# conanhujinming/flash_hash_join

Hardware: AMD Instinct MI355X
Metric: probe throughput (billion probes/sec), int64 keys, whole join (build + probe phases) per step (higher is better)
Workload: dtype int64

## Files before the change

### flash_hash_join_amd/csrc/fj_host.h

```cpp
#pragma once
#include "fj_internal.h"
#include "../../include/flashjoin.h"
#include "../../include/flashjoin_lab.h"

#include <algorithm>
#include <chrono>
#include <cstdarg>
#include <cstdio>
#include <cstdlib>
#include <cstring>
#include <condition_variable>
#include <functional>
#include <mutex>
#include <string>
#include <thread>
#include <vector>

struct StreamState;

namespace fjh {

int set_err(const char* fmt, ...);
fj_timings& last_timings();
#define HIPCHK(x)                                                                                          \
    do {                                                                                                   \
        hipError_t e_ = (x);                                                                               \
        if (e_ != hipSuccess) return fjh::set_err("%s:%d: %s failed: %s", __FILE__, __LINE__, #x, hipGetErrorString(e_)); \
    } while (0)

struct DeviceGuard {
    int prev = -1; bool changed = false; hipError_t err = hipSuccess;
    explicit DeviceGuard(int dev) {
        err = hipGetDevice(&prev);
        if (err == hipSuccess && prev != dev) { err = hipSetDevice(dev); changed = err == hipSuccess; }
    }
    ~DeviceGuard() { if (changed) (void)hipSetDevice(prev); }
    DeviceGuard(const DeviceGuard&) = delete;
    DeviceGuard& operator=(const DeviceGuard&) = delete;
};
#define FJ_ON_DEVICE(dev)                                                                                   \
    fjh::DeviceGuard dev_guard_(dev);                                                                            \
    if (dev_guard_.err != hipSuccess) return fjh::set_err("selecting HIP device %d failed: %s", (int)(dev), hipGetErrorString(dev_guard_.err))
#define FJ_ENTER(c)                                                                                         \
    if (!(c)) return fjh::set_err("%s: null context", __func__);                                             \
    std::lock_guard<std::recursive_mutex> ctx_lock_((c)->mu);                                                \
    FJ_ON_DEVICE((c)->device)

struct Scalars {
    unsigned long long total;
    unsigned long long expected;
    u64 empty_val;
    u32 err;
    u32 flags;
    u32 alloc[8];
    u32 seg_counter[8];
    unsigned long long bloom_survivors;
    unsigned long long sample_hits;
    u32 next_item;
    u32 next_emit_item;
    unsigned long long owner_counts[64], owner_cursors[64], owner_offsets[64];
    u32 pack_alloc, pack_seg, pack_err, rx_alloc;
    unsigned long long pack_used[64];
    unsigned long long pack_kept;
    u32 pack_xcd[8 * FJ_PF_COUNTERS];
    u32 bc_bounds[20];
};

enum Slot {
    W_POOL_K = 0, W_POOL_V, W_DIR, W_LIST, W_BCHUNKS, W_REL, W_BOFF, W_SEGOFF, W_TOFF, W_TILES, W_KINDS,
    W_SIDE_STRIDE = 2 * W_KINDS,
    W_PART_COUNT = 3 * W_SIDE_STRIDE, W_OUT_OFF, W_GT_KEYS, W_GT_VALS, W_GT_BLOOM, W_WG_COUNT,
    W_H_BK, W_H_BV, W_H_PK, W_H_OK, W_H_OV, W_ROWIDX, W_BKEYS, W_BBASE,
    W_PK_FI, W_PK_BKEYS, W_PK_OBASE,
    W_RX_REL, W_RX_LIST, W_RX_SEGOFF, W_RX_BCH, W_RX_BOFF, W_RX_TOFF, W_RX_TILES,
    W_SK_TILES_B, W_SK_TILES_P, W_SK_NT, W_PART_COUNT2, W_OUT_OFF2,
    W_MM_TILES,
    W_MM_PBITS,
    W_FULL_BITS,
    W_NSLOTS
};

struct Buf { void* p = nullptr; size_t bytes = 0; };

enum Ev { E_START = 0, E_BUILD, E_PPART, E_JOIN, E_EMIT0, E_EMIT1, E_SB0, E_SB1, E_BF0, E_BF1, E_H0, E_H1, E_H2, E_PK0, E_NEV = E_PK0 + 8 };

struct BcastSources { const void* base = nullptr; int n = 0; uint64_t off[FJ_WIDE_MAXSRC] = {}, nkeys[FJ_WIDE_MAXSRC] = {}; };

struct Pending {
    enum Kind { LDS, HBM_TABLE, MANY, BCAST };
    bool valid = false;
    Kind kind = LDS;
    FjLdsJoinArgs lds{};
    FjGtArgs gt{};
    u32 nitems = 0, gt_grid = 0;
    u64 count = 0;
    bool has_second = false; FjLdsJoinArgs lds2{}; u32 nitems2 = 0; u64 count_main = 0; std::vector<u32> flagged;
    bool dups_main = false; std::vector<u32> sk_parts; int sk_bits = 0, sk_plan_bits = 0, sk_npass = 0;
    int mm_outer = 0; FjMmOuterArgs mm{}; u64 mm_P = 0, mm_u = 0, mm_r = 0;
    FjMmSweepArgs mm_sweep{}; u64 mm_u_main = 0; u64* mm_tile_off = nullptr; u64* mm_sweep_off = nullptr;
    bool mm_trivial = false; const u64* mm_pk = nullptr;
    bool has_dups = false;
    const u64* bk = nullptr; const u64* bv = nullptr; size_t nb = 0; int top_bits = 64;
    BcastSources src; const u32* toff = nullptr; size_t nb_total = 0;
};

struct SingleOut { u64* keys = nullptr; u64* vals = nullptr; size_t cap = 0; bool done = false; };

struct Plan { int bits = 0, npass = 0; int fan_log[4] = {0, 0, 0, 0}; int bloom_level = 0; };

struct PassIter {
    int side = 0; bool has_vals = false; size_t n = 0; Plan plan; int used = 64; u32 parents = 1; u64 lbound = 0;
    u32 tile_chunks = 16; int i = 0;
    FjChunkSet prev{}; bool have_prev = false; const uint4* tiles = nullptr; const u32* ntiles = nullptr; const u32* toff = nullptr;
    FjChunkSet cs{}; u32 Gmax = 1, F = 1, appends = 1;
    size_t piece_rows = 0;
    int slot = 0, cs_base = 0;
    u32 item_tc_max = 0;
    bool want_items = false; u32 items_cap = 0; u32* part_count = nullptr; int part_count_slot = W_PART_COUNT;
    bool bloom_done = false; const FjChunkSet* bloom_build = nullptr;
    const u32* bloom_prebuilt = nullptr;
    unsigned long long* bloom_bucket_keys = nullptr;
    int save_level = 0; FjChunkSet saved{};
    u32* alloc_word = nullptr; u32* seg_word = nullptr; u32* err_word = nullptr;
    bool in_pk7 = false; u32 in_b0 = 0, in_top_shift = 0;
    bool vals_pos = false;
};

}

struct PackState {
    bool begun = false, deferred = false;
    u32 part_shift = 0;
    fjh::PassIter it;
    FjPackArgs args{};
    int nranks = 0;
};

struct StreamState {
    bool active = false;
    fjh::Plan plan; fjh::PassIter pit, bit; FjLdsJoinArgs ja{};
    int top_bits = 64, evc = 0;
    size_t np_bound = 0, np_seen = 0, nb_bound = 0, nb_seen = 0;
    u32 p_appends_left = 0, b_appends_left = 0;
    bool probe_done = false, build_done = false;
    const u64* flat_build = nullptr;
    const u64* flat_probe[64]; size_t flat_np[64]; u32 nflat = 0;
    std::vector<std::pair<const u64*, size_t>> bpieces, ppieces;
    bool shuffled = false; u32 b_lo = 0, nbk = 0, nbk_pad = 0;
    bool probe_prepared = true; u32 probe_appends = 0;
    bool with_vals = false;
};

struct BcastState {
    bool packed = false, probed = false;
    size_t nb_total = 0, nb = 0, np = 0;
    int pieces = 1, evc = 0;
    fjh::Plan plan; fjh::PassIter pit; FjLdsJoinArgs ja{};
    bool with_vals = false;
    fjh::BcastSources src;
};

struct fj_ctx {
    int device = 0;
    fjh::Buf bufs[fjh::W_NSLOTS];
    hipEvent_t ev[fjh::E_NEV];
    hipStream_t side = nullptr;
    fjh::Scalars* d_sc = nullptr;
    fjh::Scalars* h_sc = nullptr;
    fjh::Pending pend;
    StreamState st;
    PackState pk;
    BcastState bc;
    hipEvent_t pk_ev = nullptr;
    unsigned long long* pk_h = nullptr;
    size_t ws_bytes = 0;
    u32 num_cus = 256;
    u32 reserve_cus = 0;
    void* stage[3] = {nullptr, nullptr, nullptr};
    size_t stage_bytes = 0;
    bool plan_in_flight = false;
    bool slot_dirty[fjh::W_NSLOTS] = {};
    std::recursive_mutex mu;
};

namespace fjh {

#define FJ_HOOK_LOOPBACK 1
#define FJ_HOOK_INJECT_FAIL 2
#define FJ_HOOK_SPLIT_ALWAYS 4
#define FJ_HOOK_ONE_COMM 8
#define FJ_HOOK_RESERVE_ALWAYS 16
#define FJ_HOOK_EMIT_TAGGED 32
#define FJ_HOOK_EMIT_RETRY_7TH 64
struct Options {
    size_t radix_threshold = 0; int scalar_hbm_table = 0; u32 persistent_min_items = 8192; u32 plan_target_keys = FJ_PART_TARGET_KEYS;
    int bloom_variant = 0, bloom_auto = 1, bloom_auto_max_hit_bp = 2300, mat_single_pass = 1;
    int join_wide = 2;
    u32 lab_hooks = 0;
    u32 join_items_target = 2048;
    int mm_heavy_keys = 0;
    int mm_heavy_outer = 0;
    Options();
};
Options& options();

int get_buf(fj_ctx* c, int slot, size_t bytes, void** out);
int get_zeroed_buf(fj_ctx* c, int slot, size_t bytes, void** out, hipStream_t s);
int plan_npass(int bits);
void plan_passes(Plan& p, bool extra_first);
Plan make_plan(size_t nb, int top_bits, bool want_bloom = false, u64 target_override = 0);
void pass_init(PassIter& it, int side, bool has_vals, size_t n, const Plan& plan, int top_bits);
u32 pass_groups(u64 chunks, u64 rows, u32 tile_chunks, u32 F);
int pass_prepare(fj_ctx* c, PassIter& it, u32 appends, hipStream_t s);
int pass_launch(fj_ctx* c, PassIter& it, const u64* keys, const u64* vals, size_t n, hipStream_t s, int* ev_cursor);
bool bloom_stage_follows(const PassIter& it, int level);
void join_item_geometry(u64 nparts, size_t np, u64 chunk_bound, u32* tc, u64* max_items);
bool wide_join_planned(bool materialize, size_t nb, size_t np_eff, int bits);
int level_finish(fj_ctx* c, PassIter& it, bool final_level, hipStream_t s);
int pass_complete(fj_ctx* c, PassIter& it, hipStream_t s);
int bloom_stage(fj_ctx* c, PassIter& it, hipStream_t s);
int run_passes(fj_ctx* c, PassIter& it, const u64* keys, const u64* vals, hipStream_t s, FjChunkSet* out, int* ev_cursor);
int clear_plan_scalars(fj_ctx* c, hipStream_t s);
void begin_plan(fj_ctx* c);
void end_plan(fj_ctx* c);
void drop_pending(fj_ctx* c);
int begin_step(fj_ctx* c, const char* who);
int read_scalars(fj_ctx* c, hipStream_t s);
float ev_ms(fj_ctx* c, int a, int b);
void plan_timings(fj_ctx* c, const Plan& plan, u64 partitions, int evc, fj_timings* t);
int stamps_begin(unsigned long long** dbg, hipStream_t s);
int stamps_report(const char* label, const unsigned long long* dbg, u32 nitems, hipStream_t s);

int emit_pending(fj_ctx* c, u64* d_ok, u64* d_ov, size_t cap, hipStream_t s, fj_timings* t);
int radix_join_tail(fj_ctx* c, int materialize, FjLdsJoinArgs& ja, const Plan& plan, size_t np, const PassIter& pit, hipStream_t s,
                    fj_timings* t, int evc, u64* out_count, bool* lds_full, int top_bits, SingleOut* so = nullptr);

int join_outer(fj_ctx* c, int mode, bool use_radix, const u64* bk, const u64* bv, size_t nb, const u64* pk, size_t np, int top_bits,
               hipStream_t s, fj_timings* t, u64* out_count, u64* d_ok, u64* d_ov, bool rid = false);
int join_full(fj_ctx* c, bool use_radix, const u64* bk, const u64* bv, size_t nb, const u64* pk, size_t np, int top_bits,
              hipStream_t s, fj_timings* t, u64* out_counts, u64* d_ok, u64* d_ov, bool rid);

int stream_open(fj_ctx* c, size_t nb_bound, int build_appends, size_t np_bound, int probe_appends, hipStream_t s, int top_bits,
                size_t probe_piece_rows = 0);
int stream_append_build(fj_ctx* c, const u64* d_bk, size_t n, hipStream_t s);
int stream_flush_build(fj_ctx* c, StreamState& st, hipStream_t s);
int stream_abort(fj_ctx* c);

int bcast_emit_launch(fj_ctx* c, const Pending& pd, u64* d_ok, u64* d_ov, hipStream_t s);
void drop_bcast_result_in(fj_ctx* c, const void* p, size_t bytes);

fj_ctx*& host_ctx();

}
```

### flash_hash_join_amd/csrc/fj_internal.h

```cpp
#pragma once
#include "fj_common.h"

#define FJ_ERR_POOL 1u
#define FJ_ERR_LDS_FULL 2u
#define FJ_STAT_DUPS 4u
#define FJ_STAT_RETRY 8u
#define FJ_STAT_EMIT_RETRY 16u
#define FJ_ERR_VARIANT 32u
#define FJ_BLOOM_HDR_MAGIC 0xB100F000u
#define FJ_STAT_TOOBIG 64u
#define FJ_ERR_OUTCAP 128u
#define FJ_ITEM_RETRY 0xFFFFFFFFu
#define FJ_ITEM_TOOBIG 0xFFFFFFFEu

struct FjPartArgs {
    const u64* in_keys;
    const u64* in_vals;
    const u32* in_list;
    const u32* in_dir;
    const uint4* in_tiles;
    const u32* in_ntiles;
    u64 n_flat;
    u32 parent0;
    u64* out_keys;
    u64* out_vals;
    u32* out_dir;
    u64* out_rel;
    u32* seg_off;
    u32* bchunks;
    u32* alloc;
    u32* seg_counter;
    u32 cap_chunks;
    u32 max_segs;
    u32* err;
    u32 shift;
    u32 fan_log;
    u32 side;
    u32 slab;
    u32 run_log;
    u32 in_pk7, in_b0, in_top_shift;
    u32 vals_pos;
};

struct FjChunkSet {
    u64* keys;
    u64* vals;
    u64 n_flat;
    u32* dir;
    u64* rel;
    u32* seg_off;
    u32* alloc;
    u32 cap;
    u32 nb;
    u32 fan_mask;
    u32 max_segs;
    u32* bchunks;
    u32* boff;
    u32* list;
    u32 run_log;
};

u32 fj_partition_lds_bytes(u32 fan_log, bool vals, int line_log);
u32 fj_partition_tile_chunks(u32 fan_log, bool vals);
hipError_t fj_launch_partition(const FjPartArgs& a, bool vals, int line_log, u32 grid, hipStream_t s);
hipError_t fj_launch_group(const FjChunkSet& cs, u32 tc, u32* toff, uint4* tiles, u32 max_tiles, u32* zero_tail, hipStream_t s);
hipError_t fj_launch_scan_u32_to_u64(const u32* in, u64* out, u32 n, hipStream_t s);
hipError_t fj_launch_dir_rank(u32* dir, u32 n, u32 b_lo, u32 nbk, u32 fan, u64* rel, u32* seg_off, u32* bchunks, u32* nalloc, hipStream_t s);

struct FjBloomArgs {
    const u64* pkeys;
    const u32* plist;
    const uint4* tiles;
    u64* out_keys; u32* out_dir; u64* out_rel;
    u32 cap_chunks;
    u32 pnb;
    const u32* toff;
    const u64* bkeys; const u32* blist; const u32* bboff;
    u32* seg_off; u32* bchunks; u32* alloc; u32* seg_counter;
    u32 max_segs;
    u32* err;
    unsigned long long* survivors;
    const u32* prebuilt;
    unsigned long long* bucket_keys;
};
u32 fj_bloom_tile_chunks();
u32 fj_bloom_waves_per_group();
u32 fj_bloom_slab_chunks();
hipError_t fj_launch_bloom_filter(const FjBloomArgs& a, u32 grid, int variant, hipStream_t s);
hipError_t fj_launch_bloom_export(const FjChunkSet& build, u32* out, u32 grid, int variant, hipStream_t s);
hipError_t fj_launch_flatten(const FjChunkSet& cs, const unsigned long long* bucket_keys, unsigned long long* base, u64* out, hipStream_t s);

struct FjPackArgs {
    const u64* keys; const u64* vals;
    const u32* list; const u32* boff;
    u32 nb, fan_log, nranks, wire7;
    uint4* fi;
    u32* fb;
    u32* bkeys;
    u32* obase;
    unsigned long long* used;
    unsigned char* dst_k[64]; u64* dst_v[64]; u32* dst_d[64];
};
hipError_t fj_launch_pack_plan(const FjPackArgs& a, hipStream_t s);
#define FJ_PF_COUNTERS 4u
#ifndef FJ_PFILT_BYTES
#define FJ_PFILT_BYTES 4096u
#endif
hipError_t fj_launch_part_filter_export(const FjChunkSet& build, u64* out, u32 grid, hipStream_t s);
hipError_t fj_launch_part_filter_inplace(const FjChunkSet& cs, const u64* filters, u32 part_shift, unsigned long long* kept, u32* next_of_xcd , u32 grid, hipStream_t s);
hipError_t fj_launch_part_filter_sample(const u64* raw, u64 n, u64 stride, const u64* filters, u32 part_shift, unsigned long long* kept, hipStream_t s);
hipError_t fj_launch_pack_squeeze(const FjPackArgs& a, u32 grid, hipStream_t s);


hipError_t fj_set_max_lds_once(const void* fn, u32 bytes);

struct FjLdsJoinArgs {
    FjChunkSet build, probe;
    u32 nparts;
    u32 nsplit;
    const uint4* items;
    const u32* nitems_dev;
    u32 items_cap;
    u32* part_count;
    unsigned long long* total;
    u32* err;
    const u64* out_off;
    u64* out_keys;
    u64* out_vals;
    unsigned long long* out_cursor;
    u64 out_capacity;
    u32 retry_only;
    u32 mark_toobig;
    u32 want_dups;
    u32 dedup;
    const u64* orig_vals;
    u32 avg_build_keys;
    unsigned long long* dbg;
    u32 dbg_flags;
    u32 row_ids;
};
hipError_t fj_launch_lds_join(const FjLdsJoinArgs& a, bool materialize, hipStream_t s, u32* next_item = nullptr,
                              u32 persistent_min_items = 8192);
hipError_t fj_launch_emit_single(const FjLdsJoinArgs& a, hipStream_t s, u32* next_item);
#define FJ_WIDE_MAXSRC 16u
struct FjWideArgs {
    const u32* toff; u32 part_lo, part_hi;
    const unsigned char* base; u32 nsrc, bits, mid_bytes;
    u32 group_log;
    u32 max_units;
    u32 pmask;
    u64 offs_off[FJ_WIDE_MAXSRC], lo_off[FJ_WIDE_MAXSRC], mid_off[FJ_WIDE_MAXSRC];
};
hipError_t fj_launch_count_join_wide(const FjLdsJoinArgs& a, const FjWideArgs& w, bool dense, u32 grid, hipStream_t s);
static inline u32 fj_wide_pmask(int bits, int top_bits) { return bits <= 0 ? 0u : (bits >= 32 ? 0xFFFFFFFFu : ((1u << bits) - 1u) << (top_bits - 32 - bits)); }

hipError_t fj_launch_lds_join_retry(const FjLdsJoinArgs& a, hipStream_t s);
hipError_t fj_launch_lds_emit_retry(const FjLdsJoinArgs& a, hipStream_t s, bool only_marked = true);

hipError_t fj_launch_sample_hits(const FjChunkSet& build, const u64* pk, u64 np, u32 nsamples, u32 shift32, u32 pmask,
                                 unsigned long long* hits, hipStream_t s);

#define FJ_MM_INNER 0
#define FJ_MM_LEFT 1
#define FJ_MM_FULL 2
struct FjMmOuterArgs {
    u32* miss_count;
    unsigned long long* miss_total;
    const u64* miss_off;
    u64 miss_base;
    u64* bits;
    unsigned long long* marked;
    u64* pbits;
};
hipError_t fj_launch_mm_join(const FjLdsJoinArgs& a, bool materialize, hipStream_t s, int outer = FJ_MM_INNER, const FjMmOuterArgs* oa = nullptr);
#define FJ_MM_TILE_CHUNKS 16u
hipError_t fj_launch_mm_tile_join(const FjLdsJoinArgs& a, bool materialize, hipStream_t s, int outer = FJ_MM_INNER, const FjMmOuterArgs* oa = nullptr);
struct FjMmSweepArgs {
    FjChunkSet probe;
    const uint4* items; u32 nitems;
    const u64* pbits;
    u32* miss_count;
    unsigned long long* miss_total;
    const u64* miss_off;
    u64 miss_base;
    u64* out_keys; u64* out_vals;
    u32 row_ids;
};
hipError_t fj_launch_mm_miss_sweep(const FjMmSweepArgs& w, bool materialize, hipStream_t s);

struct FjGtArgs {
    u64* tkeys; u64* tvals; u32* bloom;
    u64 cap_mask;
    u32* flags;
    u64* empty_val;
    const u64* bk; const u64* bv; u64 nb;
    const u64* pk; u64 np;
    u32* wg_count;
    unsigned long long* total;
    const u64* out_off;
    u64* out_keys; u64* out_vals;
    u32 row_ids;
    u32* matched;
};
hipError_t fj_launch_gt_build(const FjGtArgs& a, hipStream_t s);
hipError_t fj_launch_gt_probe(const FjGtArgs& a, bool materialize, u32 grid, hipStream_t s);

hipError_t fj_launch_owner_hist(const u64* keys, u64 n, u32 nranks, unsigned long long* counts, hipStream_t s);
hipError_t fj_launch_owner_scatter(const u64* keys, const u64* vals, u64 n, u32 nranks,
                                   const unsigned long long* offsets, unsigned long long* cursors,
                                   u64* out_keys, u64* out_vals, hipStream_t s);

hipError_t fj_launch_iota(u64* out, u64 n, hipStream_t s);
hipError_t fj_launch_gen_build(u64* keys, u64* vals, u64 first, u64 n, hipStream_t s);
hipError_t fj_launch_gen_probe(u64* keys, u64 first, u64 n, u64 build_total, u64 seed, u32 hit_bp,
                               unsigned long long* expected_hits, hipStream_t s);

__host__ __device__ inline u32 fj_owner_of_w1(u32 w1, u32 nranks) { return ((w1 >> 16) * nranks) >> 16; }

#define FJ_OJ_LEFT 0
#define FJ_OJ_ANTI 1
#define FJ_OJ_LEFT_FIRST 2
struct FjOjCursor { u32 hit, miss; u64 hit_base, miss_base; };
__device__ __forceinline__ void fj_oj_reserve(FjOjCursor* cur, u32 nh, u32 nm, u32 lane, u32 tid, unsigned long long* ghit,
                                              unsigned long long* gmiss, u64& hpos, u64& mpos) {
    u32 wh = 0, wm = 0;
    if (lane == 0) { if (nh) wh = atomicAdd(&cur->hit, nh); if (nm) wm = atomicAdd(&cur->miss, nm); }
    wh = __shfl(wh, 0, 64); wm = __shfl(wm, 0, 64);
    __syncthreads();
    if (tid == 0) {
        const u32 H = cur->hit, M = cur->miss;
        cur->hit_base = H ? (u64)atomicAdd(ghit, (unsigned long long)H) : 0ull;
        cur->miss_base = M ? (u64)atomicAdd(gmiss, (unsigned long long)M) : 0ull;
        cur->hit = 0; cur->miss = 0;
    }
    __syncthreads();
    hpos = cur->hit_base + wh; mpos = cur->miss_base + wm;
}
hipError_t fj_launch_outer_join(const FjLdsJoinArgs& a, int mode, u64 np, unsigned long long* miss_cursor, hipStream_t s);
hipError_t fj_launch_gt_build_first(const FjGtArgs& a, bool vals, hipStream_t s);
hipError_t fj_launch_gt_outer_probe(const FjGtArgs& a, int mode, unsigned long long* miss_cursor, u64 out_capacity, hipStream_t s);

hipError_t fj_launch_outer_join_full(const FjLdsJoinArgs& a, int mode, u64 np, unsigned long long* miss_cursor, u64* bits, hipStream_t s);
hipError_t fj_launch_full_sweep(const FjChunkSet& build, const u64* bits, const u64* orig_vals, u32 row_ids, u64* out_keys, u64* out_vals,
                                u64 base, u64 out_capacity, unsigned long long* cursor, u32* err, hipStream_t s);
hipError_t fj_launch_gt_full_sweep(const FjGtArgs& a, u64 base, u64 out_capacity, unsigned long long* cursor, u32* err, hipStream_t s);
```

### flash_hash_join_amd/csrc/fj_joins.hip

```cpp
#include "fj_host.h"

namespace fjh {

static int skew_side(fj_ctx* c, PassIter& it, int side, bool vals, const FjChunkSet& in, const std::vector<u32>& off, u64 chunks, int S, int bits_left,
                     int slot, int tiles_slot, u32* d_nt, hipStream_t s);

int emit_pending(fj_ctx* c, u64* d_ok, u64* d_ov, size_t cap, hipStream_t s, fj_timings* t) {
    Pending& pd = c->pend;
    if (!pd.valid) return set_err("fj_emit_pairs: no counted materialising join is pending on this context");
    if (pd.count > cap) return set_err("fj_emit_pairs: output capacity %zu < %llu pairs", cap, (unsigned long long)pd.count);
    if (pd.count > 0 && (((uintptr_t)d_ok | (uintptr_t)d_ov) & 7)) return set_err("output buffers must be 8-byte aligned");
    HIPCHK(hipEventRecord(c->ev[E_EMIT0], s));
    if (pd.count > 0) {
        void* p;
        if (pd.kind == Pending::LDS) {
            if (pd.lds.row_ids) {
                pd.lds.dedup = 1; pd.lds.orig_vals = nullptr;
            } else if (pd.has_dups) {
                if (get_buf(c, W_ROWIDX, pd.nb * 8, &p)) return 1;
                u64* rowidx = (u64*)p;
                HIPCHK(fj_launch_iota(rowidx, pd.nb, s));
                HIPCHK(hipMemsetAsync(&c->d_sc->alloc[0], 0, sizeof(c->d_sc->alloc) + sizeof(c->d_sc->seg_counter), s));
                PassIter bit;
                pass_init(bit, 0, true, pd.nb, make_plan(pd.nb, pd.top_bits), pd.top_bits);
                begin_plan(c);
                if (run_passes(c, bit, pd.bk, rowidx, s, &pd.lds.build, nullptr)) return 1;
                end_plan(c);
                pd.lds.dedup = 1; pd.lds.orig_vals = pd.bv;
                if (pd.has_second) {
                    const u32 m = (u32)pd.sk_parts.size();
                    std::vector<u32> bo(2 * m);
                    for (u32 j = 0; j < m; ++j) HIPCHK(hipMemcpyAsync(&bo[2 * j], pd.lds.build.boff + pd.sk_parts[j], 8, hipMemcpyDeviceToHost, s));
                    HIPCHK(hipStreamSynchronize(s));
                    u64 bchunks = 0;
                    for (u32 j = 0; j < m; ++j) bchunks += bo[2 * j + 1] - bo[2 * j];
                    if (get_buf(c, W_SK_NT, 16, &p)) return 1;
                    PassIter bit2;
                    begin_plan(c);
                    if (skew_side(c, bit2, 0, true, pd.lds.build, bo, bchunks, pd.sk_bits, pd.top_bits - pd.sk_plan_bits, pd.sk_npass, W_SK_TILES_B, (u32*)p, s)) return 1;
                    end_plan(c);
                    pd.lds2.build = bit2.prev;
                }
            }
            if (pd.has_second)
                for (u32 idx : pd.flagged) HIPCHK(hipMemsetAsync(&pd.lds.part_count[idx], 0, 4, s));
            if (get_buf(c, W_OUT_OFF, ((size_t)pd.nitems + 1) * 8, &p)) return 1;
            HIPCHK(fj_launch_scan_u32_to_u64(pd.lds.part_count, (u64*)p, pd.nitems, s));
            pd.lds.out_off = (const u64*)p; pd.lds.out_keys = d_ok; pd.lds.out_vals = d_ov;
            pd.lds.dbg = nullptr;
#ifdef FJ_LAB
            if (getenv("FJ_EMIT_STAMPS") && stamps_begin(&pd.lds.dbg, s)) return 1;
#endif
            const bool resident = !(options().lab_hooks & FJ_HOOK_EMIT_TAGGED);
            if (resident) HIPCHK(hipMemsetAsync(&c->d_sc->next_emit_item, 0, sizeof(u32), s));
            HIPCHK(fj_launch_lds_join(pd.lds, true, s, resident ? &c->d_sc->next_emit_item : nullptr, 1u));
            if (pd.lds.dbg) { if (stamps_report("FJ_EMIT_STAMPS", pd.lds.dbg, pd.nitems, s)) return 1; pd.lds.dbg = nullptr; }
            if (pd.has_second) {
                if (get_buf(c, W_OUT_OFF2, ((size_t)pd.nitems2 + 1) * 8, &p)) return 1;
                HIPCHK(fj_launch_scan_u32_to_u64(pd.lds2.part_count, (u64*)p, pd.nitems2, s));
                pd.lds2.out_off = (const u64*)p; pd.lds2.out_keys = d_ok + pd.count_main; pd.lds2.out_vals = d_ov + pd.count_main;
                const bool rid = pd.lds2.row_ids != 0;
                pd.lds2.dedup = (pd.has_dups || rid) ? 1u : 0u; pd.lds2.orig_vals = (pd.has_dups && !rid) ? pd.bv : nullptr; pd.lds2.dbg = nullptr;
                HIPCHK(fj_launch_lds_emit_retry(pd.lds2, s, false));
            }
        } else if (pd.kind == Pending::MANY) {
            if (get_buf(c, W_OUT_OFF, ((size_t)pd.nitems + 1) * 8, &p)) return 1;
            HIPCHK(fj_launch_scan_u32_to_u64(pd.lds.part_count, (u64*)p, pd.nitems, s));
            pd.lds.out_off = (const u64*)p; pd.lds.out_keys = d_ok; pd.lds.out_vals = d_ov;
            if (pd.mm_outer == FJ_MM_INNER) {
                HIPCHK(fj_launch_mm_join(pd.lds, true, s));
                if (pd.has_second) {
                    if (get_buf(c, W_OUT_OFF2, ((size_t)pd.nitems2 + 1) * 8, &p)) return 1;
                    HIPCHK(fj_launch_scan_u32_to_u64(pd.lds2.part_count, (u64*)p, pd.nitems2, s));
                    pd.lds2.out_off = (const u64*)p; pd.lds2.out_keys = d_ok + pd.count_main; pd.lds2.out_vals = d_ov + pd.count_main;
                    HIPCHK(fj_launch_mm_tile_join(pd.lds2, true, s));
                }
            }
            else if (pd.mm_trivial) {
                const bool rid = pd.lds.row_ids != 0;
                if (pd.mm_u) {
                    if (rid) HIPCHK(fj_launch_iota(d_ok, pd.mm_u, s)); else HIPCHK(hipMemcpyAsync(d_ok, pd.mm_pk, pd.mm_u * 8, hipMemcpyDeviceToDevice, s));
                    HIPCHK(hipMemsetAsync(d_ov, rid ? 0xFF : 0, pd.mm_u * 8, s));
                } else if (rid) {
                    HIPCHK(hipMemsetAsync(d_ok, 0xFF, pd.mm_r * 8, s)); HIPCHK(fj_launch_iota(d_ov, pd.mm_r, s));
                } else {
                    HIPCHK(hipMemcpyAsync(d_ok, pd.bk, pd.mm_r * 8, hipMemcpyDeviceToDevice, s));
                    HIPCHK(hipMemcpyAsync(d_ov, pd.bv, pd.mm_r * 8, hipMemcpyDeviceToDevice, s));
                }
            } else {
                if (get_buf(c, W_OUT_OFF2, ((size_t)pd.nitems + 1) * 8, &p)) return 1;
                HIPCHK(fj_launch_scan_u32_to_u64(pd.mm.miss_count, (u64*)p, pd.nitems, s));
                pd.mm.miss_off = (const u64*)p; pd.mm.miss_base = pd.mm_P;
                HIPCHK(fj_launch_mm_join(pd.lds, true, s, pd.mm_outer, &pd.mm));
                if (pd.has_second) {
                    HIPCHK(fj_launch_scan_u32_to_u64(pd.lds2.part_count, pd.mm_tile_off, pd.nitems2, s));
                    pd.lds2.out_off = pd.mm_tile_off; pd.lds2.out_keys = d_ok + pd.count_main; pd.lds2.out_vals = d_ov + pd.count_main;
                    HIPCHK(fj_launch_mm_tile_join(pd.lds2, true, s));
                    HIPCHK(fj_launch_scan_u32_to_u64(pd.mm_sweep.miss_count, pd.mm_sweep_off, pd.mm_sweep.nitems, s));
                    pd.mm_sweep.miss_off = pd.mm_sweep_off; pd.mm_sweep.miss_base = pd.mm_P + pd.mm_u_main;
                    pd.mm_sweep.out_keys = d_ok; pd.mm_sweep.out_vals = d_ov;
                    HIPCHK(fj_launch_mm_miss_sweep(pd.mm_sweep, true, s));
                }
                if (pd.mm_r) {
                    HIPCHK(hipMemsetAsync(&c->d_sc->sample_hits, 0, sizeof(unsigned long long), s));
                    HIPCHK(fj_launch_full_sweep(pd.lds.build, pd.mm.bits, nullptr, pd.lds.row_ids, d_ok, d_ov, pd.mm_P + pd.mm_u, pd.count,
                                                &c->d_sc->sample_hits, &c->d_sc->err, s));
                }
            }
        } else if (pd.kind == Pending::HBM_TABLE) {
            if (get_buf(c, W_OUT_OFF, ((size_t)pd.gt_grid + 1) * 8, &p)) return 1;
            HIPCHK(fj_launch_scan_u32_to_u64(pd.gt.wg_count, (u64*)p, pd.gt_grid, s));
            pd.gt.out_off = (const u64*)p; pd.gt.out_keys = d_ok; pd.gt.out_vals = d_ov;
            HIPCHK(fj_launch_gt_probe(pd.gt, true, pd.gt_grid, s));
        } else {
            if (bcast_emit_launch(c, pd, d_ok, d_ov, s)) return 1;
        }
    }
    pd.valid = false;
    HIPCHK(hipEventRecord(c->ev[E_EMIT1], s));
    if (pd.count > 0) {
        if (read_scalars(c, s)) return 1;
        if (pd.kind == Pending::LDS && (c->h_sc->err & FJ_STAT_EMIT_RETRY)) {
            HIPCHK(fj_launch_lds_emit_retry(pd.lds, s));
            HIPCHK(hipEventRecord(c->ev[E_EMIT1], s));
            if (read_scalars(c, s)) return 1;
            if (t) t->lds_retries += 1;
        }
        if (c->h_sc->err & (FJ_ERR_LDS_FULL | FJ_ERR_POOL)) return set_err("fj_emit_pairs: the emitting pass could not place every partition in LDS (device error word 0x%x)", c->h_sc->err);
        if (pd.kind == Pending::BCAST && (c->h_sc->err & FJ_STAT_RETRY))
            return set_err("internal error: a partition the counting kernel accepted does not fit the pair writer's table (fj_emit_pairs)");
        if (pd.kind == Pending::MANY && pd.mm_r && !pd.mm_trivial && ((c->h_sc->err & FJ_ERR_OUTCAP) || c->h_sc->sample_hits != pd.mm_r))
            return set_err("internal error: the sweep appended %llu of %llu unmatched build rows (fj_emit_pairs)", c->h_sc->sample_hits, (unsigned long long)pd.mm_r);
    }
    HIPCHK(hipStreamSynchronize(s));
    if (t) { t->emit_ms = ev_ms(c, E_EMIT0, E_EMIT1); t->total_ms += t->emit_ms; t->probe_phase_ms += t->emit_ms; }
    return 0;
}

int join_global(fj_ctx* c, int bloom, int materialize, const u64* bk, const u64* bv, size_t nb, const u64* pk, size_t np,
                hipStream_t s, fj_timings* t, u64* out_count, bool rid = false) {
    if (rid) bloom = 0;
    u64 cap = 64;
    while (cap < 2 * (u64)nb) cap <<= 1;
    FjGtArgs a{};
    void* p;
    if (get_buf(c, W_GT_KEYS, cap * 8, &p)) return 1; a.tkeys = (u64*)p;
    if (get_buf(c, W_GT_VALS, cap * 8, &p)) return 1; a.tvals = (u64*)p;
    a.bloom = nullptr;
    if (bloom) { if (get_buf(c, W_GT_BLOOM, cap / 8 * 4, &p)) return 1; a.bloom = (u32*)p; }
    const u64 npairs = (np + 1) / 2;
    const u32 grid = (u32)std::min<u64>(2048, std::max<u64>(1, npairs / 256));
    if (get_buf(c, W_WG_COUNT, (size_t)grid * 4, &p)) return 1; a.wg_count = (u32*)p;
    a.cap_mask = cap - 1; a.flags = &c->d_sc->flags; a.empty_val = &c->d_sc->empty_val;
    a.bk = bk; a.bv = rid ? nullptr : bv; a.nb = nb; a.pk = pk; a.np = np; a.total = &c->d_sc->total;
    a.row_ids = rid ? 1u : 0u;

    HIPCHK(hipEventRecord(c->ev[E_START], s));
    HIPCHK(hipMemsetAsync(c->d_sc, 0, offsetof(Scalars, alloc), s));
    HIPCHK(hipMemsetAsync(a.tkeys, 0xFF, cap * 8, s));
    if (a.bloom) HIPCHK(hipMemsetAsync(a.bloom, 0, cap / 8 * 4, s));
    if (rid) {
        HIPCHK(hipMemsetAsync(&c->d_sc->empty_val, 0xFF, sizeof(u64), s));
        HIPCHK(hipMemsetAsync(a.tvals, 0xFF, cap * 8, s));
        HIPCHK(fj_launch_gt_build_first(a, true, s));
    } else
    HIPCHK(fj_launch_gt_build(a, s));
    HIPCHK(hipEventRecord(c->ev[E_BUILD], s));
    HIPCHK(hipEventRecord(c->ev[E_PPART], s));
    if (np > 0) HIPCHK(fj_launch_gt_probe(a, false, grid, s));
    else HIPCHK(hipMemsetAsync(a.wg_count, 0, (size_t)grid * 4, s));
    HIPCHK(hipEventRecord(c->ev[E_JOIN], s));
    if (read_scalars(c, s)) return 1;
    *out_count = c->h_sc->total;
    t->path = 1; t->passes = 0; t->radix_bits = 0; t->partitions = 1;
    t->build_phase_ms = ev_ms(c, E_START, E_BUILD);
    t->join_ms = ev_ms(c, E_PPART, E_JOIN);
    t->probe_phase_ms = t->join_ms;
    t->total_ms = ev_ms(c, E_START, E_JOIN);
    if (materialize) { c->pend.valid = true; c->pend.kind = Pending::HBM_TABLE; c->pend.gt = a; c->pend.gt_grid = grid; c->pend.count = *out_count; }
    return 0;
}

static int skew_side(fj_ctx* c, PassIter& it, int side, bool vals, const FjChunkSet& in, const std::vector<u32>& off, u64 chunks, int S, int bits_left,
                     int slot, int tiles_slot, u32* d_nt, hipStream_t s) {
    const u32 m = (u32)(off.size() / 2);
    Plan p2; p2.bits = S; p2.npass = 1; p2.fan_log[0] = S;
    const u32 tc = fj_partition_tile_chunks((u32)S, vals);
    std::vector<uint4> tiles;
    for (u32 j = 0; j < m; ++j)
        for (u32 pos = off[2 * j]; pos < off[2 * j + 1]; pos += tc) tiles.push_back(make_uint4(pos, std::min(tc, off[2 * j + 1] - pos), j, 0));
    const u32 nt = (u32)tiles.size();
    void* p;
    if (get_buf(c, tiles_slot, std::max<size_t>(1, tiles.size()) * sizeof(uint4), &p)) return 1;
    if (nt) HIPCHK(hipMemcpyAsync(p, tiles.data(), tiles.size() * sizeof(uint4), hipMemcpyHostToDevice, s));
    HIPCHK(hipMemcpyAsync(d_nt, &nt, 4, hipMemcpyHostToDevice, s));
    HIPCHK(hipStreamSynchronize(s));
    pass_init(it, side, vals, std::max<u64>(1, chunks * FJ_CHUNK), p2, bits_left);
    it.parents = m; it.lbound = chunks;
    it.slot = slot;
    it.have_prev = true; it.prev = in; it.tiles = (const uint4*)p; it.ntiles = d_nt;
    if (side) { it.want_items = true; it.part_count_slot = W_PART_COUNT2; }
    HIPCHK(hipMemsetAsync(&c->d_sc->alloc[side * 4], 0, 4, s));
    HIPCHK(hipMemsetAsync(&c->d_sc->seg_counter[side * 4], 0, 4, s));
    if (pass_prepare(c, it, 1, s) || pass_launch(c, it, nullptr, nullptr, 0, s, nullptr) || pass_complete(c, it, s)) return 1;
    return 0;
}

int skew_join(fj_ctx* c, const FjLdsJoinArgs& ja, const Plan& plan, int top_bits, u32 nitems, int probe_slot, int materialize, hipStream_t s, bool* ok,
              u32* nparts_redone, Pending* pend) {
    *ok = false;
    if (!ja.items || !ja.build.list || !ja.probe.list || nitems == 0) return 0;
    std::vector<u32> pc(nitems);
    std::vector<uint4> items(nitems);
    HIPCHK(hipMemcpyAsync(pc.data(), ja.part_count, (size_t)nitems * 4, hipMemcpyDeviceToHost, s));
    HIPCHK(hipMemcpyAsync(items.data(), ja.items, (size_t)nitems * sizeof(uint4), hipMemcpyDeviceToHost, s));
    HIPCHK(hipStreamSynchronize(s));
    std::vector<u32> parts, flagged;
    for (u32 i = 0; i < nitems; ++i) if (pc[i] == FJ_ITEM_TOOBIG) { parts.push_back(items[i].z); flagged.push_back(i); }
    std::sort(parts.begin(), parts.end());
    parts.erase(std::unique(parts.begin(), parts.end()), parts.end());
    const u32 m = (u32)parts.size();
    if (m == 0 || m > 64) return 0;
    u64 already = 0;
    {
        u32 nlive = nitems;
        HIPCHK(hipMemcpy(&nlive, ja.nitems_dev, 4, hipMemcpyDeviceToHost));
        if (nlive > nitems) nlive = nitems;
        for (u32 i = 0; i < nlive; ++i) {
            if (pc[i] == FJ_ITEM_TOOBIG || pc[i] == FJ_ITEM_RETRY || !std::binary_search(parts.begin(), parts.end(), items[i].z)) continue;
            already += pc[i];
            flagged.push_back(i);
            HIPCHK(hipMemsetAsync(&ja.part_count[i], 0, 4, s));
        }
    }
    std::vector<u32> bo(2 * m), po(2 * m);
    for (u32 j = 0; j < m; ++j) {
        HIPCHK(hipMemcpyAsync(&bo[2 * j], ja.build.boff + parts[j], 8, hipMemcpyDeviceToHost, s));
        HIPCHK(hipMemcpyAsync(&po[2 * j], ja.probe.boff + parts[j], 8, hipMemcpyDeviceToHost, s));
    }
    HIPCHK(hipStreamSynchronize(s));
    u64 bchunks = 0, pchunks = 0, bmax = 0;
    for (u32 j = 0; j < m; ++j) { const u64 nb_j = bo[2 * j + 1] - bo[2 * j]; bchunks += nb_j; bmax = std::max(bmax, nb_j); pchunks += po[2 * j + 1] - po[2 * j]; }
    int S = 1;
    while (S < FJ_MAX_FAN_LOG && ((bmax * FJ_CHUNK) >> S) > 2048) ++S;
    if (((bmax * FJ_CHUNK) >> S) > 6000 || top_bits - plan.bits - S < 32) return 0;
    if (S < 5) S = std::min(5, top_bits - plan.bits - 32);
    if (S < 1) return 0;
    void* p;
    if (get_buf(c, W_SK_NT, 16, &p)) return 1;
    u32* d_nt = (u32*)p;
    PassIter bit2, pit2;
    const u64 count_main = c->h_sc->total - already;
    if (already) {
        HIPCHK(hipMemcpyAsync(&c->d_sc->total, &count_main, 8, hipMemcpyHostToDevice, s));
        HIPCHK(hipStreamSynchronize(s));
    }
    const bool had_dups = (c->h_sc->err & FJ_STAT_DUPS) != 0;
    HIPCHK(hipMemsetAsync(&c->d_sc->err, 0, 4, s));
    if (skew_side(c, bit2, 0, materialize != 0, ja.build, bo, bchunks, S, top_bits - plan.bits, plan.npass, W_SK_TILES_B, d_nt, s)) return 1;
    if (skew_side(c, pit2, 1, ja.row_ids != 0, ja.probe, po, pchunks, S, top_bits - plan.bits, probe_slot, W_SK_TILES_P, d_nt + 1, s)) return 1;
    FjLdsJoinArgs j2 = ja;
    j2.build = bit2.prev; j2.probe = pit2.prev; j2.nparts = j2.probe.nb; j2.nsplit = 1;
    j2.items = pit2.tiles; j2.nitems_dev = pit2.ntiles; j2.items_cap = pit2.items_cap; j2.part_count = pit2.part_count;
    j2.retry_only = 0; j2.mark_toobig = 0; j2.want_dups = materialize ? 1u : 0u; j2.dbg = nullptr;
    HIPCHK(fj_launch_lds_join(j2, false, s, nullptr, 0xFFFFFFFFu));
    if (read_scalars(c, s)) return 1;
    if ((c->h_sc->err & FJ_STAT_RETRY) && !(c->h_sc->err & (FJ_ERR_POOL | FJ_ERR_LDS_FULL))) {
        HIPCHK(fj_launch_lds_join_retry(j2, s));
        if (read_scalars(c, s)) return 1;
    }
    if (c->h_sc->err & FJ_ERR_POOL) return set_err("internal error: chunk pool exhausted while re-partitioning a skewed partition");
    if (c->h_sc->err & FJ_ERR_LDS_FULL) return 0;
    if (materialize) {
        pend->has_second = true; pend->lds2 = j2; pend->nitems2 = pit2.items_cap; pend->count_main = count_main; pend->flagged = flagged;
        pend->sk_parts = parts; pend->sk_bits = S; pend->sk_plan_bits = plan.bits; pend->sk_npass = plan.npass;
        pend->dups_main = had_dups;
    }
    *ok = true; *nparts_redone = m;
    return 0;
}

int radix_join_tail(fj_ctx* c, int materialize, FjLdsJoinArgs& ja, const Plan& plan, size_t np, const PassIter& pit, hipStream_t s,
                    fj_timings* t, int evc, u64* out_count, bool* lds_full, int top_bits, SingleOut* so) {
    ja.nparts = ja.probe.list ? ja.probe.nb : 1u << plan.bits;
    const u64 pchunks = (np + FJ_CHUNK - 1) / FJ_CHUNK;
    void* p;
    u32 nitems;
    if (ja.probe.list) {
        ja.items = pit.tiles; ja.nitems_dev = pit.ntiles; ja.items_cap = pit.items_cap; ja.part_count = pit.part_count;
        ja.nsplit = 1;
        nitems = pit.items_cap;
    } else {
        u64 nsplit = 1;
        if (ja.nparts < 2048) {
            nsplit = (2048 + ja.nparts - 1) / ja.nparts;
            const u64 per_part = pchunks / ja.nparts;
            nsplit = std::min<u64>(nsplit, std::max<u64>(1, per_part / 32));
        }
        ja.nsplit = (u32)nsplit; ja.items = nullptr; ja.nitems_dev = nullptr; ja.items_cap = 0;
        nitems = ja.nparts * ja.nsplit;
        if (get_buf(c, W_PART_COUNT, (size_t)nitems * 4, &p)) return 1; ja.part_count = (u32*)p;
    }
    ja.total = &c->d_sc->total; ja.err = &c->d_sc->err;
    ja.want_dups = materialize ? 1u : 0u; ja.dedup = 0; ja.orig_vals = nullptr; ja.retry_only = 0;
    ja.dbg = nullptr;
    ja.dbg_flags = (options().lab_hooks & FJ_HOOK_EMIT_RETRY_7TH) ? 8u : 0u;
#ifdef FJ_LAB
    if (getenv("FJ_JOIN_ABLATE")) ja.dbg_flags = (u32)atoi(getenv("FJ_JOIN_ABLATE"));
#endif
    if (so && materialize && ja.probe.list && ja.build.list && ja.build.vals && ja.items && !ja.dbg_flags) {
        FjLdsJoinArgs js = ja;
        js.out_cursor = &c->d_sc->total; js.out_capacity = so->cap; js.out_keys = so->keys; js.out_vals = so->vals; js.out_off = nullptr;
        HIPCHK(hipMemsetAsync(&c->d_sc->next_emit_item, 0, sizeof(u32), s));
        HIPCHK(fj_launch_emit_single(js, s, &c->d_sc->next_emit_item));
        HIPCHK(hipEventRecord(c->ev[E_JOIN], s));
        if (read_scalars(c, s)) return 1;
        if (c->h_sc->err & FJ_ERR_POOL) return set_err("internal error: chunk pool exhausted during a partition pass");
        if (!(c->h_sc->err & (FJ_STAT_DUPS | FJ_STAT_EMIT_RETRY | FJ_ERR_LDS_FULL | FJ_ERR_OUTCAP))) {
            end_plan(c);
            plan_timings(c, plan, ja.nparts, evc, t);
            t->lds_retries = 0;
            *out_count = c->h_sc->total;
            so->done = true;
            return 0;
        }
        HIPCHK(hipMemsetAsync(&c->d_sc->total, 0, sizeof(unsigned long long), s));
        HIPCHK(hipMemsetAsync(&c->d_sc->err, 0, sizeof(u32), s));
    }
#ifdef FJ_LAB
    if (getenv("FJ_JOIN_STAMPS") && stamps_begin(&ja.dbg, s)) return 1;
#endif
    const bool wide = pit.item_tc_max == 32 && !materialize && !ja.dbg && !ja.dbg_flags && ja.probe.list && ja.build.list && ja.items;
    if (wide) {
        FjWideArgs wa{};
        wa.pmask = fj_wide_pmask(plan.bits, top_bits);
        wa.group_log = np / ((size_t)1 << plan.bits) > 7000 ? 3u : 0u;
        FjLdsJoinArgs jw = ja;
#ifdef FJ_LAB
        if (getenv("FJ_WIDE_STAMPS") && stamps_begin(&jw.dbg, s)) return 1;
#endif
        const u32 grid = std::min<u32>(nitems, c->num_cus);
        HIPCHK(fj_launch_count_join_wide(jw, wa, false, grid, s));
        if (jw.dbg) {
            std::vector<unsigned long long> h(4096 * 8);
            HIPCHK(hipStreamSynchronize(s));
            HIPCHK(hipMemcpy(h.data(), jw.dbg, h.size() * 8, hipMemcpyDeviceToHost));
            double acc[8] = {0, 0, 0, 0, 0, 0, 0, 0};
            for (u32 g = 0; g < grid && g < 4096; ++g) for (int i = 0; i < 8; ++i) acc[i] += (double)h[g * 8 + i] * 0.01;
            u32 nit = 0;
            HIPCHK(hipMemcpy(&nit, jw.nitems_dev, 4, hipMemcpyDeviceToHost));
            const double per = (double)std::min<u32>(grid, 4096) * ((double)nit / grid);
            fprintf(stderr, "[FJ_WIDE_STAMPS] us per item (thread 0): rotate+requests %.3f  claim_issue+zero %.3f  barB %.3f  probe %.3f  resolve+park %.3f  barA %.3f  stores %.3f\n",
                    acc[0] / per, acc[5] / per, acc[6] / per, acc[1] / per, acc[2] / per, acc[3] / per, acc[4] / per);
            for (int ph = 0; ph < 3; ++ph) {
                fprintf(stderr, "[FJ_WIDE_STAMPS] wave 0..15, %s:", ph == 0 ? "requests + claims issued + probe" : ph == 1 ? "claims resolved + park (to barrier A)" : "stores (barrier A to B)");
                for (int w = 0; w < 16; ++w) {
                    double sacc = 0;
                    for (u32 g = 0; g < grid && g < 256; ++g) sacc += (double)h[2048 * 8 + g * 64 + w * 4 + ph] * 0.01;
                    fprintf(stderr, " %.2f", sacc / ((double)std::min<u32>(grid, 256) * ((double)nit / grid)));
                }
                fprintf(stderr, "\n");
            }
        }
    } else
    HIPCHK(fj_launch_lds_join(ja, false, s, &c->d_sc->next_item, options().persistent_min_items));
    if (ja.dbg) { if (stamps_report("FJ_JOIN_STAMPS", ja.dbg, nitems, s)) return 1; ja.dbg = nullptr; }
    HIPCHK(hipEventRecord(c->ev[E_JOIN], s));
    if (read_scalars(c, s)) return 1;
    t->lds_retries = 0;
    if ((c->h_sc->err & FJ_STAT_RETRY) && !(c->h_sc->err & (FJ_ERR_POOL | FJ_ERR_LDS_FULL))) {
        ja.retry_only = 1; ja.mark_toobig = ja.items ? 1u : 0u;
        HIPCHK(fj_launch_lds_join_retry(ja, s));
        ja.retry_only = 0;
        HIPCHK(hipEventRecord(c->ev[E_JOIN], s));
        if (read_scalars(c, s)) return 1;
        t->lds_retries = 1;
        if ((c->h_sc->err & FJ_STAT_TOOBIG) && !(c->h_sc->err & (FJ_ERR_POOL | FJ_ERR_LDS_FULL))) {
            bool ok = false; u32 redone = 0;
            if (skew_join(c, ja, plan, top_bits, nitems, pit.slot, materialize, s, &ok, &redone, &c->pend)) return 1;
            HIPCHK(hipEventRecord(c->ev[E_JOIN], s));
            if (read_scalars(c, s)) return 1;
            if (ok) t->lds_retries = 1 + (int)redone;
            else c->h_sc->err |= FJ_ERR_LDS_FULL;
        }
    }
    if (c->h_sc->err & FJ_ERR_POOL) return set_err("internal error: chunk pool exhausted during a partition pass");
    end_plan(c);
    plan_timings(c, plan, ja.nparts, evc, t);
    if (c->h_sc->err & FJ_ERR_LDS_FULL) { *lds_full = true; return 0; }
    *out_count = c->h_sc->total;
    if (materialize) {
        c->pend.valid = true; c->pend.kind = Pending::LDS; c->pend.lds = ja; c->pend.nitems = nitems; c->pend.count = *out_count;
        c->pend.has_dups = (c->h_sc->err & FJ_STAT_DUPS) != 0 || c->pend.dups_main;
    }
    return 0;
}

int join_radix(fj_ctx* c, int materialize, int bloom, const u64* bk, const u64* bv, size_t nb, const u64* pk, size_t np, int top_bits,
               hipStream_t s, fj_timings* t, u64* out_count, bool* lds_full, SingleOut* so = nullptr, bool rid = false) {
    Plan plan = make_plan(nb, top_bits, bloom != 0);
    *lds_full = false;
    t->sampled_hit_bp = -1;
    if (bloom == 2 && (plan.bloom_level == 0 || np < 4 * nb || np < (1u << 24) || !options().bloom_auto)) {
        bloom = 0; plan = make_plan(nb, top_bits, false);
    }
    begin_plan(c);
    HIPCHK(hipEventRecord(c->ev[E_START], s));
    if (clear_plan_scalars(c, s)) return 1;
    FjLdsJoinArgs ja{};
    PassIter bit, pit;
    pass_init(bit, 0, materialize != 0, nb, plan, top_bits);
    bit.vals_pos = rid;
    int evc = 0;
    if (plan.bloom_level > 0) bit.save_level = plan.bloom_level;
    if (run_passes(c, bit, bk, (materialize && !rid) ? bv : nullptr, s, &ja.build, nullptr)) return 1;
    HIPCHK(hipEventRecord(c->ev[E_BUILD], s));
    Plan pplan = plan;
    if (bloom == 2) {
        const u32 nsamp = FJ_SAMPLE_KEYS;
        HIPCHK(fj_launch_sample_hits(ja.build, pk, np, nsamp, (u32)(top_bits - 32 - plan.bits), (1u << plan.bits) - 1u, &c->d_sc->sample_hits, s));
        HIPCHK(hipMemcpyAsync(&c->h_sc->sample_hits, &c->d_sc->sample_hits, sizeof(unsigned long long), hipMemcpyDeviceToHost, s));
        HIPCHK(hipStreamSynchronize(s));
        const u32 hit_bp = (u32)(c->h_sc->sample_hits * 10000ull / nsamp);
        t->sampled_hit_bp = (int)hit_bp;
        if (hit_bp > (u32)options().bloom_auto_max_hit_bp) { pplan = make_plan(nb, top_bits, false); plan.bloom_level = 0; plan.npass = pplan.npass; }
    }
    pass_init(pit, 1, rid, np, pplan, top_bits);
    pit.vals_pos = rid;
    pit.want_items = true;
    {
        size_t np_eff = np;
        if (plan.bloom_level > 0) np_eff = (size_t)((double)np * (t->sampled_hit_bp >= 0 ? std::min(10000, t->sampled_hit_bp + 1000) : 1500) / 10000.0);
        if (wide_join_planned(materialize != 0, nb, np_eff, plan.bits)) pit.item_tc_max = 32;
    }
    if (plan.bloom_level > 0) pit.bloom_build = &bit.saved;
    if (run_passes(c, pit, pk, nullptr, s, &ja.probe, &evc)) return 1;
    HIPCHK(hipEventRecord(c->ev[E_PPART], s));
    ja.avg_build_keys = (u32)std::min<u64>(0xFFFFFFFFu, (u64)nb >> plan.bits);
    ja.row_ids = rid ? 1u : 0u;
    if (radix_join_tail(c, materialize, ja, plan, np, pit, s, t, evc, out_count, lds_full, top_bits, so)) return 1;
    if (c->pend.valid) { c->pend.bk = bk; c->pend.bv = bv; c->pend.nb = nb; c->pend.top_bits = top_bits; }
    return 0;
}

static int mm_tile_join(fj_ctx* c, const FjLdsJoinArgs& ja, u32 nitems, int materialize, hipStream_t s, Pending* pend,
                        int outer = FJ_MM_INNER, const FjMmOuterArgs* oa = nullptr) {
    u32 nlive = 0;
    std::vector<u32> pc(nitems), boff((size_t)ja.build.nb + 1);
    std::vector<uint4> items(nitems);
    HIPCHK(hipMemcpyAsync(&nlive, ja.nitems_dev, 4, hipMemcpyDeviceToHost, s));
    HIPCHK(hipMemcpyAsync(pc.data(), ja.part_count, (size_t)nitems * 4, hipMemcpyDeviceToHost, s));
    HIPCHK(hipMemcpyAsync(items.data(), ja.items, (size_t)nitems * sizeof(uint4), hipMemcpyDeviceToHost, s));
    HIPCHK(hipMemcpyAsync(boff.data(), ja.build.boff, boff.size() * 4, hipMemcpyDeviceToHost, s));
    HIPCHK(hipStreamSynchronize(s));
    if (nlive > nitems) nlive = nitems;
    std::vector<uint4> tiles, big;
    for (u32 i = 0; i < nlive; ++i) {
        if (pc[i] != FJ_ITEM_TOOBIG) continue;
        pc[i] = 0;
        if (outer != FJ_MM_INNER) big.push_back(items[i]);
        const u32 part = items[i].z;
        if (part >= ja.build.nb) return set_err("internal error: work item %u of a many-to-many join names partition %u of %u", i, part, ja.build.nb);
        const u32 nbc = boff[part + 1] - boff[part];
        for (u32 c_lo = 0; c_lo < nbc; c_lo += FJ_MM_TILE_CHUNKS) tiles.push_back(make_uint4(items[i].x, items[i].y, part, c_lo));
    }
    if (tiles.empty()) return set_err("internal error: the many-to-many counting pass reported an oversized partition and marked no item");
    if (tiles.size() > (1u << 26)) return set_err("many-to-many join: %zu (probe item, build tile) work items for the partitions beyond 4096 build rows; not supported", tiles.size());
    const u32 n2 = (u32)tiles.size();
    void* p;
    FjLdsJoinArgs j2 = ja;
    FjMmOuterArgs o2{};
    FjMmSweepArgs sw{};
    u64* tile_off = nullptr; u64* sweep_off = nullptr;
    const u32 nbig = (u32)big.size();
    if (outer == FJ_MM_INNER) {
        if (get_buf(c, W_MM_TILES, (size_t)n2 * sizeof(uint4), &p)) return 1;
        HIPCHK(hipMemcpyAsync(p, tiles.data(), (size_t)n2 * sizeof(uint4), hipMemcpyHostToDevice, s));
        j2.items = (const uint4*)p; j2.nitems_dev = nullptr; j2.items_cap = n2; j2.mark_toobig = 0;
        if (get_buf(c, W_PART_COUNT2, (size_t)n2 * 4, &p)) return 1;
        j2.part_count = (u32*)p;
    } else {
        auto r16 = [](size_t b) { return (b + 15) & ~(size_t)15; };
        const size_t o_big = (size_t)n2 * sizeof(uint4), o_tc = o_big + (size_t)nbig * sizeof(uint4), o_sc = o_tc + r16((size_t)n2 * 4),
                     o_to = o_sc + r16((size_t)nbig * 4), o_so = o_to + r16(((size_t)n2 + 1) * 8), bytes = o_so + r16(((size_t)nbig + 1) * 8);
        if (get_buf(c, W_MM_TILES, bytes, &p)) return 1;
        unsigned char* base = (unsigned char*)p;
        HIPCHK(hipMemcpyAsync(base, tiles.data(), (size_t)n2 * sizeof(uint4), hipMemcpyHostToDevice, s));
        HIPCHK(hipMemcpyAsync(base + o_big, big.data(), (size_t)nbig * sizeof(uint4), hipMemcpyHostToDevice, s));
        j2.items = (const uint4*)base; j2.nitems_dev = nullptr; j2.items_cap = n2; j2.mark_toobig = 0;
        j2.part_count = (u32*)(base + o_tc);
        tile_off = (u64*)(base + o_to); sweep_off = (u64*)(base + o_so);
        const size_t pbit_bytes = (size_t)ja.probe.cap * (FJ_CHUNK / 8);
        if (get_buf(c, W_MM_PBITS, pbit_bytes, &p)) return 1;
        HIPCHK(hipMemsetAsync(p, 0, pbit_bytes, s));
        o2 = *oa; o2.pbits = (u64*)p;
        sw.probe = ja.probe; sw.items = (const uint4*)(base + o_big); sw.nitems = nbig; sw.pbits = o2.pbits;
        sw.miss_count = (u32*)(base + o_sc); sw.miss_total = oa->miss_total; sw.row_ids = ja.row_ids;
    }
    HIPCHK(hipMemcpyAsync(ja.part_count, pc.data(), (size_t)nlive * 4, hipMemcpyHostToDevice, s));
    HIPCHK(hipMemsetAsync(&c->d_sc->err, 0, 4, s));
    const u64 count_main = c->h_sc->total, u_main = c->h_sc->expected;
    HIPCHK(fj_launch_mm_tile_join(j2, false, s, outer, &o2));
    if (outer != FJ_MM_INNER) HIPCHK(fj_launch_mm_miss_sweep(sw, false, s));
    HIPCHK(hipEventRecord(c->ev[E_JOIN], s));
    if (read_scalars(c, s)) return 1;
    if (materialize) {
        pend->has_second = true; pend->lds2 = j2; pend->nitems2 = n2; pend->count_main = count_main;
        if (outer != FJ_MM_INNER) { pend->mm_sweep = sw; pend->mm_u_main = u_main; pend->mm_tile_off = tile_off; pend->mm_sweep_off = sweep_off; }
    }
    return 0;
}

int join_many(fj_ctx* c, int materialize, const u64* bk, const u64* bv, size_t nb, const u64* pk, size_t np, int top_bits,
              hipStream_t s, fj_timings* t, u64* out_count, bool rid = false, int outer = FJ_MM_INNER) {
    const Plan plan = make_plan(nb, top_bits, false, 2048);
    begin_plan(c);
    HIPCHK(hipEventRecord(c->ev[E_START], s));
    if (clear_plan_scalars(c, s)) return 1;
    FjLdsJoinArgs ja{};
    PassIter bit, pit;
    pass_init(bit, 0, materialize != 0, nb, plan, top_bits);
    pass_init(pit, 1, rid, np, plan, top_bits);
    bit.vals_pos = pit.vals_pos = rid;
    pit.want_items = true;
    int evc = 0;
    ja.row_ids = rid ? 1u : 0u;
    if (run_passes(c, bit, bk, (materialize && !rid) ? bv : nullptr, s, &ja.build, nullptr)) return 1;
    HIPCHK(hipEventRecord(c->ev[E_BUILD], s));
    if (run_passes(c, pit, pk, nullptr, s, &ja.probe, &evc)) return 1;
    HIPCHK(hipEventRecord(c->ev[E_PPART], s));
    ja.nparts = 1u << plan.bits;
    u32 nitems;
    void* p;
    if (ja.probe.list) {
        ja.items = pit.tiles; ja.nitems_dev = pit.ntiles; ja.items_cap = pit.items_cap; ja.part_count = pit.part_count; ja.nsplit = 1;
        nitems = pit.items_cap;
    } else {
        const u64 pchunks = (np + FJ_CHUNK - 1) / FJ_CHUNK;
        ja.nsplit = (u32)std::min<u64>(2048, std::max<u64>(1, pchunks / 32)); ja.items = nullptr; ja.nitems_dev = nullptr; ja.items_cap = 0;
        nitems = ja.nparts * ja.nsplit;
        if (get_buf(c, W_PART_COUNT, (size_t)nitems * 4, &p)) return 1; ja.part_count = (u32*)p;
    }
    ja.total = &c->d_sc->total; ja.err = &c->d_sc->err;
    FjMmOuterArgs oa{};
    if (outer != FJ_MM_INNER) {
        if (get_buf(c, W_PART_COUNT2, (size_t)nitems * 4, &p)) return 1;
        oa.miss_count = (u32*)p; oa.miss_total = &c->d_sc->expected;
        HIPCHK(hipMemsetAsync(oa.miss_count, 0, (size_t)nitems * 4, s));
        if (outer == FJ_MM_FULL) {
            const size_t bit_bytes = (ja.build.list ? (size_t)ja.build.cap : (nb + FJ_CHUNK - 1) / FJ_CHUNK) * (FJ_CHUNK / 8);
            if (get_buf(c, W_FULL_BITS, bit_bytes, &p)) return 1;
            oa.bits = (u64*)p; oa.marked = &c->d_sc->bloom_survivors;
            HIPCHK(hipMemsetAsync(oa.bits, 0, bit_bytes, s));
        }
    }
    ja.mark_toobig = ((outer == FJ_MM_INNER ? options().mm_heavy_keys : options().mm_heavy_outer) && ja.items && ja.build.list) ? 1u : 0u;
    HIPCHK(fj_launch_mm_join(ja, false, s, outer, &oa));
    HIPCHK(hipEventRecord(c->ev[E_JOIN], s));
    if (read_scalars(c, s)) return 1;
    bool tiled = false;
    if ((c->h_sc->err & FJ_STAT_TOOBIG) && !(c->h_sc->err & (FJ_ERR_POOL | FJ_ERR_LDS_FULL))) {
        if (mm_tile_join(c, ja, nitems, materialize, s, &c->pend, outer, &oa)) return 1;
        tiled = true;
    }
    if (c->h_sc->err & FJ_ERR_POOL) return set_err("internal error: chunk pool exhausted during a partition pass");
    end_plan(c);
    if (c->h_sc->err & FJ_ERR_LDS_FULL)
        return set_err("many-to-many join: a final partition holds more than 4096 build rows (a build key with thousands of duplicates?); not supported");
    *out_count = c->h_sc->total;
    plan_timings(c, plan, ja.nparts, evc, t);
    if (tiled) t->lds_retries = FJ_LDS_RETRIES_MM_TILED;
    if (materialize) { c->pend.valid = true; c->pend.kind = Pending::MANY; c->pend.lds = ja; c->pend.nitems = nitems; c->pend.count = *out_count; }
    if (outer != FJ_MM_INNER) {
        const u64 P = c->h_sc->total, u = c->h_sc->expected, marked = outer == FJ_MM_FULL ? c->h_sc->bloom_survivors : 0;
        if (u > np || marked > nb) { drop_pending(c); return set_err("internal error: all-copies outer join counted %llu of %zu probe rows unmatched and %llu of %zu build rows matched", (unsigned long long)u, np, (unsigned long long)marked, nb); }
        const u64 r = outer == FJ_MM_FULL ? nb - marked : 0;
        out_count[0] = P; out_count[1] = r; out_count[2] = u;
        c->pend.mm_outer = outer; c->pend.mm = oa; c->pend.mm_P = P; c->pend.mm_u = u; c->pend.mm_r = r; c->pend.count = P + u + r;
    }
    return 0;
}


}
using namespace fjh;

extern "C" {

int fj_join_device(fj_ctx* c, int algo, int bloom, int materialize,
                   const uint64_t* d_bk, const uint64_t* d_bv, size_t nb, const uint64_t* d_pk, size_t np,
                   void* stream, int hash_top_bits, uint64_t* out_count,
                   uint64_t* d_out_keys, uint64_t* d_out_vals, size_t out_capacity, fj_timings* timings) {
    const bool many = algo >= 0 && (algo & FJ_ALGO_MANY_TO_MANY) != 0;
    const bool left = algo >= 0 && (algo & FJ_ALGO_LEFT_OUTER) != 0, anti = algo >= 0 && (algo & FJ_ALGO_ANTI) != 0;
    const bool rid = algo >= 0 && (algo & FJ_ALGO_ROW_IDS) != 0;
    const bool full = algo >= 0 && (algo & FJ_ALGO_FULL_OUTER) != 0;
    const bool allc = algo >= 0 && (algo & FJ_ALGO_ALL_COPIES) != 0;
    const int algo_word = algo;
    if (many) algo &= ~FJ_ALGO_MANY_TO_MANY;
    if (rid) {
        algo &= ~FJ_ALGO_ROW_IDS;
        if (!materialize) return set_err("fj_join_device: FJ_ALGO_ROW_IDS needs materialize = 1 (it changes what the output rows hold)");
        if (!d_bv) d_bv = d_bk;
        bloom = 0;
    }
    if (allc) {
        algo &= ~(FJ_ALGO_ALL_COPIES | FJ_ALGO_LEFT_OUTER | FJ_ALGO_FULL_OUTER);
        if (anti) return set_err("fj_join_device: FJ_ALGO_ALL_COPIES cannot be combined with FJ_ALGO_ANTI (an anti join has no copies to keep)");
        if (many) return set_err("fj_join_device: FJ_ALGO_ALL_COPIES cannot be combined with FJ_ALGO_MANY_TO_MANY (that flag alone is the inner join that keeps every copy)");
        if (!left && !full) return set_err("fj_join_device: unknown algo %d (FJ_ALGO_ALL_COPIES modifies FJ_ALGO_LEFT_OUTER or FJ_ALGO_FULL_OUTER; FJ_ALGO_MANY_TO_MANY is the inner form)", algo_word);
        if (left && full) return set_err("fj_join_device: FJ_ALGO_FULL_OUTER cannot be combined with FJ_ALGO_LEFT_OUTER");
        if (!materialize) return set_err("fj_join_device: FJ_ALGO_ALL_COPIES needs materialize = 1 (there is no counting-only form)");
        if (!out_count) return set_err("fj_join_device: FJ_ALGO_ALL_COPIES needs out_count (three words: pairs, unmatched build rows, unmatched probe rows)");
        if (((uintptr_t)d_out_keys | (uintptr_t)d_out_vals) & 7) return set_err("fj_join_device: output buffers must be 8-byte aligned");
        if (nb && !d_bv) return set_err("fj_join_device: FJ_ALGO_ALL_COPIES needs d_build_vals (only FJ_ALGO_ROW_IDS reads no build value)");
    }
    if (full && !allc) {
        algo &= ~FJ_ALGO_FULL_OUTER;
        if (left || anti) return set_err("fj_join_device: FJ_ALGO_FULL_OUTER cannot be combined with FJ_ALGO_%s", left ? "LEFT_OUTER" : "ANTI");
        if (many) return set_err("fj_join_device: FJ_ALGO_FULL_OUTER cannot be combined with FJ_ALGO_MANY_TO_MANY");
        if (!materialize) return set_err("fj_join_device: FJ_ALGO_FULL_OUTER needs materialize = 1 (its match count is the counting join's)");
        if ((np || nb) && (!d_out_keys || !d_out_vals)) return set_err("fj_join_device: FJ_ALGO_FULL_OUTER needs output buffers (d_out_keys and d_out_vals)");
        if (out_capacity < np || out_capacity - np < nb) return set_err("fj_join_device: output capacity %zu < %zu probe rows + %zu build rows (FJ_ALGO_FULL_OUTER may write every row of both sides)", out_capacity, np, nb);
        if (((uintptr_t)d_out_keys | (uintptr_t)d_out_vals) & 7) return set_err("fj_join_device: output buffers must be 8-byte aligned");
        if (nb && !d_bv) return set_err("fj_join_device: FJ_ALGO_FULL_OUTER needs d_build_vals (only FJ_ALGO_ROW_IDS reads no build value)");
        if (!out_count) return set_err("fj_join_device: FJ_ALGO_FULL_OUTER needs out_count (two words: matched probe rows, unmatched build rows)");
    }
    if ((left || anti) && !allc) {
        algo &= ~(FJ_ALGO_LEFT_OUTER | FJ_ALGO_ANTI);
        if (left && anti) return set_err("fj_join_device: FJ_ALGO_LEFT_OUTER and FJ_ALGO_ANTI cannot be combined");
        if (many) return set_err("fj_join_device: FJ_ALGO_%s cannot be combined with FJ_ALGO_MANY_TO_MANY", left ? "LEFT_OUTER" : "ANTI");
        if (left && !materialize) return set_err("fj_join_device: FJ_ALGO_LEFT_OUTER needs materialize = 1 (its match count is the counting join's)");
        if (materialize) {
            if (np && (!d_out_keys || (left && !d_out_vals))) return set_err("fj_join_device: FJ_ALGO_%s needs output buffers (d_out_keys%s)", left ? "LEFT_OUTER" : "ANTI", left ? " and d_out_vals" : "");
            if (out_capacity < np) return set_err("fj_join_device: output capacity %zu < %zu probe rows (FJ_ALGO_%s writes every probe row)", out_capacity, np, left ? "LEFT_OUTER" : "ANTI");
            if (((uintptr_t)d_out_keys | (uintptr_t)(left ? d_out_vals : nullptr)) & 7) return set_err("fj_join_device: output buffers must be 8-byte aligned");
        }
        if (!left && !d_bv) d_bv = d_bk;
    }
    if (algo < 0 || algo > 2) return set_err("fj_join_device: unknown algo %d", algo);
    if (hash_top_bits != 64 && hash_top_bits != 48) return set_err("fj_join_device: hash_top_bits must be 64 or 48");
    if ((nb && (!d_bk || !d_bv)) || (np && !d_pk)) return set_err("fj_join_device: null input pointer");
    if (((uintptr_t)d_bk | (uintptr_t)d_bv | (uintptr_t)d_pk) & 15) return set_err("fj_join_device: input pointers must be 16-byte aligned");
    FJ_ENTER(c);
    if (begin_step(c, "fj_join_device")) return 1;
    hipStream_t s = (hipStream_t)stream;
    fj_timings t; memset(&t, 0, sizeof t);
    t.sampled_hit_bp = -1;
    u64 count = 0;
    const Options& opt = options();
    bool use_radix = algo == FJ_ALGO_RADIX || (algo == FJ_ALGO_ADAPTIVE && nb >= opt.radix_threshold) ||
                     (algo == FJ_ALGO_SCALAR && !opt.scalar_hbm_table);
    if (allc) {
        u64 c3[3] = {0, 0, 0};
        if (nb == 0 || np == 0) {
            if (clear_plan_scalars(c, s)) return 1;
            c3[1] = (np == 0 && full) ? nb : 0; c3[2] = nb == 0 ? np : 0;
            Pending& pd = c->pend;
            pd.valid = true; pd.kind = Pending::MANY; pd.mm_outer = full ? FJ_MM_FULL : FJ_MM_LEFT; pd.mm_trivial = true;
            pd.lds.row_ids = rid ? 1u : 0u; pd.bk = d_bk; pd.bv = d_bv; pd.mm_pk = d_pk;
            pd.mm_P = 0; pd.mm_u = c3[2]; pd.mm_r = c3[1]; pd.count = c3[1] + c3[2];
        } else if (join_many(c, 1, d_bk, d_bv, nb, d_pk, np, hash_top_bits, s, &t, c3, rid, full ? FJ_MM_FULL : FJ_MM_LEFT)) return 1;
        out_count[0] = c3[0]; out_count[1] = c3[1]; out_count[2] = c3[2];
        if (d_out_keys && d_out_vals && emit_pending(c, d_out_keys, d_out_vals, out_capacity, s, &t)) return 1;
        if (timings) *timings = t;
        last_timings() = t;
        return 0;
    }
    if (full) {
        u64 counts[2] = {0, 0};
        if (join_full(c, use_radix, d_bk, d_bv, nb, d_pk, np, hash_top_bits, s, &t, counts, (u64*)d_out_keys, (u64*)d_out_vals, rid)) return 1;
        out_count[0] = counts[0]; out_count[1] = counts[1];
        if (timings) *timings = t;
        last_timings() = t;
        return 0;
    }
    if ((left || anti) && materialize) {
        if (join_outer(c, left ? FJ_OJ_LEFT : FJ_OJ_ANTI, use_radix, d_bk, d_bv, nb, d_pk, np, hash_top_bits, s, &t, &count,
                       (u64*)d_out_keys, (u64*)d_out_vals, rid)) return 1;
        if (out_count) *out_count = count;
        if (timings) *timings = t;
        last_timings() = t;
        return 0;
    }
    if (nb == 0 || np == 0) {
        count = 0;
    } else if (many) {
        if (join_many(c, materialize, d_bk, d_bv, nb, d_pk, np, hash_top_bits, s, &t, &count, rid)) return 1;
    } else if (use_radix) {
        bool lds_full = false;
        const int bloom_mode = rid ? 0 : algo == FJ_ALGO_ADAPTIVE ? (options().bloom_auto ? 2 : (bloom ? 1 : 0)) : (bloom ? 1 : 0);
        SingleOut so;
        so.keys = (u64*)d_out_keys; so.vals = (u64*)d_out_vals; so.cap = out_capacity;
        const bool try_single = materialize && d_out_keys && d_out_vals && out_capacity >= np && options().mat_single_pass &&
                                !(((uintptr_t)d_out_keys | (uintptr_t)d_out_vals) & 7);
        if (join_radix(c, materialize, bloom_mode, d_bk, d_bv, nb, d_pk, np, hash_top_bits, s, &t, &count, &lds_full, try_single ? &so : nullptr, rid)) return 1;
        if (lds_full) {
            fj_timings t2; memset(&t2, 0, sizeof t2);
            if (join_global(c, bloom, materialize, d_bk, d_bv, nb, d_pk, np, s, &t2, &count, rid)) return 1;
            t2.total_ms += t.total_ms; t2.fell_back = 1; t2.sampled_hit_bp = t.sampled_hit_bp; t = t2;
        }
    } else {
        if (join_global(c, bloom, materialize, d_bk, d_bv, nb, d_pk, np, s, &t, &count, rid)) return 1;
    }
    if (anti) count = np - count;
    if (out_count) *out_count = count;
    if (materialize && d_out_keys && d_out_vals && c->pend.valid) {
        if (emit_pending(c, d_out_keys, d_out_vals, out_capacity, s, &t)) return 1;
    }
    if (timings) *timings = t;
    last_timings() = t;
    return 0;
}

int fj_emit_pairs(fj_ctx* c, uint64_t* d_out_keys, uint64_t* d_out_vals, size_t out_capacity, void* stream, fj_timings* timings) {
    FJ_ENTER(c);
    fj_timings t = last_timings();
    if (emit_pending(c, d_out_keys, d_out_vals, out_capacity, (hipStream_t)stream, &t)) return 1;
    if (timings) *timings = t;
    last_timings() = t;
    return 0;
}

int fj_owner_split(fj_ctx* c, const uint64_t* d_keys, const uint64_t* d_vals, size_t n, int nranks,
                   uint64_t* d_out_keys, uint64_t* d_out_vals, uint64_t* h_counts, void* stream) {
    if (nranks < 1 || nranks > 64) return set_err("fj_owner_split: nranks must be 1..64");
    FJ_ENTER(c);
    hipStream_t s = (hipStream_t)stream;
    HIPCHK(hipMemsetAsync(c->d_sc->owner_counts, 0, sizeof(unsigned long long) * 128, s));
    HIPCHK(fj_launch_owner_hist(d_keys, n, (u32)nranks, c->d_sc->owner_counts, s));
    HIPCHK(hipMemcpyAsync(c->h_sc->owner_counts, c->d_sc->owner_counts, sizeof(unsigned long long) * 64, hipMemcpyDeviceToHost, s));
    HIPCHK(hipStreamSynchronize(s));
    unsigned long long run = 0;
    for (int r = 0; r < nranks; ++r) { c->h_sc->owner_offsets[r] = run; run += c->h_sc->owner_counts[r]; h_counts[r] = c->h_sc->owner_counts[r]; }
    if (run != n) return set_err("fj_owner_split: histogram covers %llu of %zu rows", run, n);
    HIPCHK(hipMemcpyAsync(c->d_sc->owner_offsets, c->h_sc->owner_offsets, sizeof(unsigned long long) * 64, hipMemcpyHostToDevice, s));
    HIPCHK(fj_launch_owner_scatter(d_keys, d_vals, n, (u32)nranks, c->d_sc->owner_offsets, c->d_sc->owner_cursors, d_out_keys, d_out_vals, s));
    HIPCHK(hipStreamSynchronize(s));
    return 0;
}

int fj_owner_hist(fj_ctx* c, const uint64_t* d_keys, size_t n, int nranks, uint64_t* h_counts, void* stream) {
    if (nranks < 1 || nranks > 64) return set_err("fj_owner_hist: nranks must be 1..64");
    FJ_ENTER(c);
    hipStream_t s = (hipStream_t)stream;
    HIPCHK(hipMemsetAsync(c->d_sc->owner_counts, 0, sizeof(unsigned long long) * 64, s));
    HIPCHK(fj_launch_owner_hist(d_keys, n, (u32)nranks, c->d_sc->owner_counts, s));
    HIPCHK(hipMemcpyAsync(c->h_sc->owner_counts, c->d_sc->owner_counts, sizeof(unsigned long long) * 64, hipMemcpyDeviceToHost, s));
    HIPCHK(hipStreamSynchronize(s));
    unsigned long long run = 0;
    for (int r = 0; r < nranks; ++r) { h_counts[r] = c->h_sc->owner_counts[r]; run += h_counts[r]; }
    if (run != n) return set_err("fj_owner_hist: histogram covers %llu of %zu rows", run, n);
    return 0;
}

int fj_owner_scatter(fj_ctx* c, const uint64_t* d_keys, const uint64_t* d_vals, size_t n, int nranks, const uint64_t* h_counts,
                     uint64_t* d_out_keys, uint64_t* d_out_vals, void* stream) {
    if (nranks < 1 || nranks > 64) return set_err("fj_owner_scatter: nranks must be 1..64");
    FJ_ENTER(c);
    hipStream_t s = (hipStream_t)stream;
    HIPCHK(hipStreamSynchronize(s));
    unsigned long long run = 0;
    for (int r = 0; r < nranks; ++r) { c->h_sc->owner_offsets[r] = run; run += h_counts[r]; }
    if (run != n) return set_err("fj_owner_scatter: counts cover %llu of %zu rows", run, n);
    HIPCHK(hipMemcpyAsync(c->d_sc->owner_offsets, c->h_sc->owner_offsets, sizeof(unsigned long long) * 64, hipMemcpyHostToDevice, s));
    HIPCHK(hipMemsetAsync(c->d_sc->owner_cursors, 0, sizeof(unsigned long long) * 64, s));
    HIPCHK(fj_launch_owner_scatter(d_keys, d_vals, n, (u32)nranks, c->d_sc->owner_offsets, c->d_sc->owner_cursors, d_out_keys, d_out_vals, s));
    return 0;
}

size_t fj_bloom_filter_words(void) { return ((size_t)1 << FJ_PREFILTER_BITS) * FJ_BLOOM_WORDS + 4; }

int fj_bloom_export(fj_ctx* c, const uint64_t* d_build_keys, size_t nb, int hash_top_bits, uint32_t* d_filters, void* stream) {
    if (hash_top_bits != 64 && hash_top_bits != 48) return set_err("fj_bloom_export: hash_top_bits must be 64 or 48");
    if (!d_filters || (nb && !d_build_keys) || ((uintptr_t)d_build_keys & 15) || ((uintptr_t)d_filters & 15)) return set_err("fj_bloom_export: null or misaligned pointer");
    FJ_ENTER(c);
    if (begin_step(c, "fj_bloom_export")) return 1;
    hipStream_t s = (hipStream_t)stream;
    const u32 nbuckets = 1u << FJ_PREFILTER_BITS;
    if (nb == 0) {
        HIPCHK(hipMemsetAsync(d_filters, 0, fj_bloom_filter_words() * 4, s));
        HIPCHK(hipMemsetD32Async((hipDeviceptr_t)(d_filters + (size_t)nbuckets * FJ_BLOOM_WORDS), (int)(FJ_BLOOM_HDR_MAGIC | (u32)options().bloom_variant), 1, s));
        return 0;
    }
    Plan plan; plan.bits = FJ_PREFILTER_BITS; plan_passes(plan, true);
    begin_plan(c);
    if (clear_plan_scalars(c, s)) return 1;
    PassIter bit;
    pass_init(bit, 0, false, nb, plan, hash_top_bits);
    FjChunkSet cs{};
    if (run_passes(c, bit, (const u64*)d_build_keys, nullptr, s, &cs, nullptr)) return 1;
    HIPCHK(fj_launch_bloom_export(cs, d_filters, c->num_cus, options().bloom_variant, s));
    if (read_scalars(c, s)) return 1;
    if (c->h_sc->err & FJ_ERR_POOL) return set_err("internal error: chunk pool exhausted during a partition pass");
    end_plan(c);
    return 0;
}

int fj_bloom_prefilter(fj_ctx* c, const uint64_t* d_probe_keys, size_t n, int hash_top_bits, const uint32_t* d_filters,
                       uint64_t* d_out_keys, size_t out_capacity, uint64_t* out_n, void* stream) {
    if (hash_top_bits != 64 && hash_top_bits != 48) return set_err("fj_bloom_prefilter: hash_top_bits must be 64 or 48");
    if (!d_filters || !out_n || (n && (!d_probe_keys || !d_out_keys)) || ((uintptr_t)d_probe_keys & 15) || ((uintptr_t)d_filters & 15) || ((uintptr_t)d_out_keys & 7))
        return set_err("fj_bloom_prefilter: null or misaligned pointer");
    if (out_capacity < n) return set_err("fj_bloom_prefilter: output capacity %zu < %zu input rows", out_capacity, n);
    FJ_ENTER(c);
    if (begin_step(c, "fj_bloom_prefilter")) return 1;
    *out_n = 0;
    if (n == 0) return 0;
    hipStream_t s = (hipStream_t)stream;
    Plan plan; plan.bits = FJ_PREFILTER_BITS; plan_passes(plan, true);
    plan.bloom_level = 1;
    begin_plan(c);
    if (clear_plan_scalars(c, s)) return 1;
    const u32 nbuckets = 1u << FJ_PREFILTER_BITS;
    void* p;
    if (get_buf(c, W_BKEYS, (size_t)nbuckets * 8, &p)) return 1; unsigned long long* bkeys = (unsigned long long*)p;
    if (get_buf(c, W_BBASE, ((size_t)nbuckets + 1) * 8, &p)) return 1; unsigned long long* bbase = (unsigned long long*)p;
    HIPCHK(hipMemsetAsync(bkeys, 0, (size_t)nbuckets * 8, s));
    static const FjChunkSet no_build{};
    PassIter pit;
    pass_init(pit, 1, false, n, plan, hash_top_bits);
    pit.bloom_build = &no_build; pit.bloom_prebuilt = (const u32*)d_filters; pit.bloom_bucket_keys = bkeys;
    FjChunkSet cs{};
    if (run_passes(c, pit, (const u64*)d_probe_keys, nullptr, s, &cs, nullptr)) return 1;
    if (bloom_stage(c, pit, s)) return 1;
    cs = pit.prev;
    HIPCHK(fj_launch_flatten(cs, bkeys, bbase, (u64*)d_out_keys, s));
    if (read_scalars(c, s)) return 1;
    HIPCHK(hipMemcpyAsync(&c->h_sc->expected, &bbase[nbuckets], sizeof(unsigned long long), hipMemcpyDeviceToHost, s));
    HIPCHK(hipStreamSynchronize(s));
    if (c->h_sc->err & FJ_ERR_POOL) return set_err("internal error: chunk pool exhausted during a partition pass");
    end_plan(c);
    if (c->h_sc->err & FJ_ERR_VARIANT)
        return set_err("fj_bloom_prefilter: these filters were not exported with bloom_variant %d (every rank must use the same FJ_BLOOM_VARIANT)", options().bloom_variant);
    if (c->h_sc->expected != c->h_sc->bloom_survivors) return set_err("internal error: prefilter flattened %llu of %llu survivors", c->h_sc->expected, c->h_sc->bloom_survivors);
    *out_n = c->h_sc->expected;
    return 0;
}
}
```

### flash_hash_join_amd/csrc/fj_partition.hip

```cpp
#include "fj_internal.h"
#include <cstdlib>
#include <mutex>
#include <vector>

namespace {

#ifndef FJ_LO_PAD
#define FJ_LO_PAD 1u
#endif
struct PartLds {
    u32 sorted_k, sorted_v, lo_k, lo_v, hist, toff, line_desc, t_chunk, t_cnt, wsum, misc, total;
};
__host__ __device__ inline PartLds part_lds_layout(u32 T, u32 F, u32 line, bool vals, u32 nwaves) {
    PartLds L;
    const u32 nsorted = T + 2;
    const u32 maxl = (T + (line - 1) * F) / line + 2;
    u32 o = 0;
    L.sorted_k = o; o += nsorted * 8;
    L.sorted_v = o; if (vals) o += nsorted * 8;
    L.lo_k = o; o += F * (line + FJ_LO_PAD) * 8;
    L.lo_v = o; if (vals) o += F * (line + FJ_LO_PAD) * 8;
    L.line_desc = o; o += maxl * 8;
    L.wsum = o; o += nwaves * 8;
    L.hist = o; o += (F + 4) * 4;
    L.toff = o; o += (F + 4) * 4;
    L.t_chunk = o; o += (T / FJ_CHUNK) * 4;
    L.t_cnt = o; o += (T / FJ_CHUNK) * 4;
    L.misc = o; o += 16 * 4;
    L.total = (o + 15) & ~15u;
    return L;
}

enum { M_SLAB_CUR = 0, M_SLAB_REM, M_NEW_BASE, M_NEED, M_NLINES, M_FLUSH, M_SEG, M_NEW_UNITS };

template <int NT, int KPT, int LINE_LOG, bool HAS_VALS, bool FLAT, bool PROBE_SIDE, int RLOG = FJ_RUN_LOG, bool PK7 = false, bool POS = false>
__global__ __launch_bounds__(NT, 4) void fj_partition_kernel(FjPartArgs a) {
    constexpr u32 T = NT * KPT, LINE = 1u << LINE_LOG, TC = T / FJ_CHUNK, NW = NT / 64, LOS = LINE + FJ_LO_PAD;
    static_assert(T % FJ_CHUNK == 0 && TC <= NT && LINE >= 4 && T + 64 < (1u << 17), "tile geometry");
    static_assert(!PK7 || (!FLAT && KPT % 4 == 0), "wire-format chunks come through chunk lists, four keys per load group");
    static_assert(!POS || (FLAT && HAS_VALS), "positions are made by the first pass over a flat input");
    constexpr bool RUNS = RLOG > 0;
    constexpr u32 RL = (u32)RLOG, RU = 1u << RL;
    const u32 F = 1u << a.fan_log, FM = F - 1;
    const u32 tid = threadIdx.x, lane = tid & 63, wave = tid >> 6;
    const u32 sh32 = a.shift - 32;

    extern __shared__ __attribute__((aligned(16))) unsigned char smem[];
    const PartLds Lo = part_lds_layout(T, F, LINE, HAS_VALS, NW);
    u64* tile_k = (u64*)(smem + Lo.sorted_k);
    u64* tile_v = (u64*)(smem + Lo.sorted_v);
    u64* lo_k = (u64*)(smem + Lo.lo_k);
    u64* lo_v = (u64*)(smem + Lo.lo_v);
    u64* line_desc = (u64*)(smem + Lo.line_desc);
    u64* wsum = (u64*)(smem + Lo.wsum);
    u32* hist = (u32*)(smem + Lo.hist);
    u32* toff = (u32*)(smem + Lo.toff);
    u32* t_chunk = (u32*)(smem + Lo.t_chunk);
    u32* t_cnt = (u32*)(smem + Lo.t_cnt);
    u32* misc = (u32*)(smem + Lo.misc);

    const u32 Lc = FLAT ? (u32)((a.n_flat + FJ_CHUNK - 1) >> FJ_CHUNK_LOG) : 0u;
    const u32 ntiles = FLAT ? (Lc + TC - 1) / TC : *a.in_ntiles;
    const u32 G = gridDim.x, g = blockIdx.x;
    const u32 t0 = (u32)(((u64)g * ntiles) / G);
    const u32 nmine = (u32)(((u64)(g + 1) * ntiles) / G) - t0;
    u32 t = 0;
    const u32 thi = nmine;
    const u32 cap = a.cap_chunks;
    if (t >= thi) return;

    auto get_desc = [&](u32 tt, u32& pos, u32& len, u32& parent) {
        const uint4 d = a.in_tiles[t0 + tt]; pos = d.x; len = d.y; parent = d.z;
    };
    auto meta_fetch = [&](u32 pos, u32 len, u32& id, u32& cnt) {
        id = 0; cnt = 0;
        if (tid < len) { const u32 e = a.in_list[pos + tid]; id = FJ_LIST_ID(e); cnt = FJ_LIST_CNT(e); }
    };
    const bool tiny = FLAT && a.n_flat < 2;
    const u64 last_pair = FLAT ? ((a.n_flat - 2) & ~1ull) : 0;
    struct Pk7Raw { uint4 lo; uint2 mid; u32 hi; };
    auto key_load7 = [&](u32 tt, Pk7Raw (&rr)[KPT / 4 ? KPT / 4 : 1], u64 (&vv)[KPT], u32& vmask) {
        (void)tt;
        vmask = 0;
#pragma unroll
        for (int i = 0; i < KPT / 4; ++i) {
            const u32 kidx = ((u32)i * NT + tid) * 4;
            const u32 j = kidx >> FJ_CHUNK_LOG, off = kidx & (FJ_CHUNK - 1);
            const u32 cnt = t_cnt[j];
            const unsigned char* base = reinterpret_cast<const unsigned char*>(a.in_keys) + (u64)t_chunk[j] * FJ_WIRE7_BYTES;
            rr[i].lo = *reinterpret_cast<const uint4*>(base + off * 4u);
            rr[i].mid = *reinterpret_cast<const uint2*>(base + FJ_WIRE7_MID + off * 2u);
            rr[i].hi = *reinterpret_cast<const u32*>(base + FJ_WIRE7_HI + off);
            if (HAS_VALS) {
                const u64x2 w0 = *reinterpret_cast<const u64x2*>(a.in_vals + (u64)t_chunk[j] * FJ_CHUNK + off);
                const u64x2 w1 = *reinterpret_cast<const u64x2*>(a.in_vals + (u64)t_chunk[j] * FJ_CHUNK + off + 2);
                vv[4 * i] = w0.x; vv[4 * i + 1] = w0.y; vv[4 * i + 2] = w1.x; vv[4 * i + 3] = w1.y;
            }
            const u32 nv = off < cnt ? (cnt - off < 4u ? cnt - off : 4u) : 0u;
            vmask |= ((1u << nv) - 1u) << (4 * i);
        }
    };
    auto key_load = [&](u32 tt, u64 (&kk)[KPT], u64 (&vv)[KPT], u32& vmask) {
        vmask = 0;
#pragma unroll
        for (int i = 0; i < KPT / 2; ++i) {
            u64 base; u32 nv;
            if (FLAT) {
                base = (u64)(t0 + tt) * T + ((u32)i * NT + tid) * 2;
                nv = base + 1 < a.n_flat ? 2u : (base < a.n_flat ? 1u : 0u);
                if (POS) { vv[2 * i] = base; vv[2 * i + 1] = base + 1; }
                if (base > last_pair) base = last_pair;
            } else {
                const u32 kidx = ((u32)i * NT + tid) * 2;
                const u32 j = kidx >> FJ_CHUNK_LOG, off = kidx & (FJ_CHUNK - 1);
                const u32 cnt = t_cnt[j];
                base = (u64)t_chunk[j] * FJ_CHUNK + off;
                nv = off + 1 < cnt ? 2u : (off < cnt ? 1u : 0u);
            }
            if (tiny) {
                kk[2 * i] = nv ? a.in_keys[0] : 0; kk[2 * i + 1] = 0;
                if (HAS_VALS) { vv[2 * i] = (nv && !POS) ? a.in_vals[0] : 0; vv[2 * i + 1] = 0; }
            } else {
                const u64x2 q = *reinterpret_cast<const u64x2*>(a.in_keys + base);
                kk[2 * i] = q.x; kk[2 * i + 1] = q.y;
                if (HAS_VALS && !POS) {
                    const u64x2 w = *reinterpret_cast<const u64x2*>(a.in_vals + base);
                    vv[2 * i] = w.x; vv[2 * i + 1] = w.y;
                }
            }
            vmask |= (nv == 2 ? 3u : (nv == 1 ? 1u : 0u)) << (2 * i);
        }
        if (FLAT && !tiny && (a.n_flat & 1ull)) {
#pragma unroll
            for (int i = 0; i < KPT / 2; ++i) {
                const u64 base = (u64)(t0 + tt) * T + ((u32)i * NT + tid) * 2;
                if (base + 1 == a.n_flat) { kk[2 * i] = a.in_keys[base]; if (HAS_VALS) vv[2 * i] = POS ? base : a.in_vals[base]; }
            }
        }
    };

    if (tid == 0) { misc[M_SLAB_CUR] = 0; misc[M_SLAB_REM] = 0; misc[M_NEW_BASE] = 0; misc[M_SEG] = 0; misc[M_NEW_UNITS] = 0; }
    u32 st_left = 0, st_fill = FJ_CHUNK, st_cur = FJ_DIR_INVALID, st_nch = 0;
    u32 pend_cnt = 0, pend_nf = 0, pend_tb = 0;

    auto carry = [&]() {
        if (tid < F) {
            const u32 b = tid, tot = st_left + pend_cnt;
            if (pend_nf == 0) {
                for (u32 j = 0; j < pend_cnt; ++j) {
                    lo_k[b * LOS + st_left + j] = tile_k[pend_tb + j];
                    if (HAS_VALS) lo_v[b * LOS + st_left + j] = tile_v[pend_tb + j];
                }
            } else {
                const u32 nl2 = tot - pend_nf, src = pend_tb + (pend_nf - st_left);
                for (u32 j = 0; j < nl2; ++j) {
                    lo_k[b * LOS + j] = tile_k[src + j];
                    if (HAS_VALS) lo_v[b * LOS + j] = tile_v[src + j];
                }
            }
            st_left = tot - pend_nf;
            pend_cnt = 0; pend_nf = 0;
        }
    };

    auto alloc_id = [&](u32 j, u32) -> u32 {
        const u32 rem = misc[M_SLAB_REM];
        return j < rem ? misc[M_SLAB_CUR] + (j << RL) : misc[M_NEW_BASE] + ((j - rem) << RL);
    };
    auto rot = [&](u32 b) -> u32 { return ((b * 2654435761u + blockIdx.x * 40503u) >> 13) & (RU - 1u); };
    auto run_left = [&](u32 c0, u32 b) -> u32 { return (RUNS && c0 != FJ_DIR_INVALID) ? (RU - 1u) - ((c0 - rot(b)) & (RU - 1u)) : 0u; };
    auto run_step = [&](u32 c0, u32 k) -> u32 { return (c0 & ~(RU - 1u)) | ((c0 + k) & (RU - 1u)); };
    auto chunk_id = [&](u32 kk, u32 c0, u32 ukb, u32 b) -> u32 {
        if constexpr (!RUNS) return alloc_id(ukb + kk - 1, b);
        const u32 rl = run_left(c0, b);
        if (kk <= rl) return run_step(c0, kk);
        const u32 q = kk - rl - 1u;
        return alloc_id(ukb + (q >> RL), b) + ((q + rot(b)) & (RU - 1u));
    };
    auto take_slabs = [&](u32 need) {
        const u32 su = a.slab >> RL, k = (need - misc[M_SLAB_REM] + su - 1) / su;
        const u32 nb = atomicAdd(a.alloc, k * a.slab);
        if (nb + k * a.slab > cap) atomicOr(a.err, FJ_ERR_POOL);
        misc[M_NEW_BASE] = nb; misc[M_NEW_UNITS] = k * su;
    };
    auto commit_units = [&](u32 need) {
        const u32 rem = misc[M_SLAB_REM];
        if (need <= rem) { misc[M_SLAB_CUR] += need << RL; misc[M_SLAB_REM] = rem - need; }
        else { const u32 used = need - rem; misc[M_SLAB_CUR] = misc[M_NEW_BASE] + (used << RL); misc[M_SLAB_REM] = misc[M_NEW_UNITS] - used; }
    };

    auto flush = [&](u32 parent) {
        if (tid == 0) misc[M_FLUSH] = 0;
        __syncthreads();
        u32 fresh = 0xFFFFFFFFu;
        if (tid < F && st_left > 0 && st_fill == FJ_CHUNK && !run_left(st_cur, tid)) fresh = atomicAdd(&misc[M_FLUSH], 1u);
        __syncthreads();
        if (tid == 0 && misc[M_FLUSH] > misc[M_SLAB_REM]) take_slabs(misc[M_FLUSH]);
        __syncthreads();
        if (tid < F) {
            const u32 b = tid, l = st_left, seg = misc[M_SEG];
            u32 f0 = st_fill, c = st_cur, n = st_nch;
            const u32 outb = parent * F + b;
            if (l > 0 && f0 == FJ_CHUNK) {
                if (fresh == 0xFFFFFFFFu) c = run_step(c, 1);
                else c = alloc_id(fresh, b) + rot(b);
                f0 = 0;
                if (c < cap) a.out_rel[c] = ((u64)seg << 32) | n;
                ++n;
            }
            if (c != FJ_DIR_INVALID && c < cap) {
                const u64 base = (u64)c * FJ_CHUNK + f0;
                for (u32 j = 0; j < l; ++j) {
                    a.out_keys[base + j] = lo_k[b * LOS + j];
                    if (HAS_VALS) a.out_vals[base + j] = lo_v[b * LOS + j];
                }
                a.out_dir[c] = (outb << FJ_DIR_CNT_BITS) | (f0 + l);
                if constexpr (RUNS) { for (u32 k = 1; k <= run_left(c, b); ++k) { const u32 id = run_step(c, k); if (id < cap) a.out_dir[id] = FJ_DIR_INVALID; } }
            }
            if (n > 0) {
                const u32 off = atomicAdd(&a.bchunks[outb], n);
                if (seg < a.max_segs) a.seg_off[(u64)seg * F + b] = off;
            }
            st_left = 0; st_fill = FJ_CHUNK; st_cur = FJ_DIR_INVALID; st_nch = 0;
        }
        __syncthreads();
        if (tid == 0) commit_units(misc[M_FLUSH]);
        __syncthreads();
    };

    u64 kn[KPT], vn[KPT];
    Pk7Raw rn[KPT / 4 ? KPT / 4 : 1];
    u32 validn = 0, par_next = a.parent0, par_n2 = a.parent0, mid = 0, mcnt = 0;
    u32 d3_pos = 0, d3_len = 0, d3_par = 0;
    if (FLAT) {
        key_load(t, kn, vn, validn);
    } else {
        u32 p, l;
        get_desc(t, p, l, par_next);
        meta_fetch(p, l, mid, mcnt);
        if (tid < TC) { t_chunk[tid] = mid; t_cnt[tid] = mcnt; }
        __syncthreads();
        if constexpr (PK7) key_load7(t, rn, vn, validn); else key_load(t, kn, vn, validn);
        mid = 0; mcnt = 0;
        if (t + 1 < thi) { get_desc(t + 1, p, l, par_n2); meta_fetch(p, l, mid, mcnt); }
        if (t + 2 < thi) get_desc(t + 2, d3_pos, d3_len, d3_par);
        __syncthreads();
        if (tid < TC) { t_chunk[tid] = mid; t_cnt[tid] = mcnt; }
    }
    __syncthreads();

    u32 cur_parent = 0xFFFFFFFFu;
    u32 hotb = 0xFFFFFFFFu;
    for (; t < thi; ++t) {
        u64 k[KPT], v[KPT];
#pragma unroll
        for (int i = 0; i < KPT; ++i) { k[i] = FLAT ? fj_key_mix(kn[i]) : kn[i]; if (HAS_VALS) v[i] = vn[i]; }
        const u32 valid = validn, parent = par_next;
        if constexpr (PK7) {
            const u64 top = (u64)((a.in_b0 + parent) >> a.in_top_shift) << 56;
#pragma unroll
            for (int i = 0; i < KPT / 4; ++i) {
                const u32 lo[4] = {rn[i].lo.x, rn[i].lo.y, rn[i].lo.z, rn[i].lo.w};
#pragma unroll
                for (int m = 0; m < 4; ++m) {
                    const u32 md = ((m & 2) ? rn[i].mid.y : rn[i].mid.x) >> ((m & 1) * 16) & 0xFFFFu;
                    const u32 hb = (rn[i].hi >> (8 * m)) & 0xFFu;
                    k[4 * i + m] = top | ((u64)((hb << 16) | md) << 32) | lo[m];
                }
            }
        }
        const u32 par_t1 = par_n2;
        if (!FLAT) {
            mid = 0; mcnt = 0;
            if (t + 2 < thi) { par_n2 = d3_par; meta_fetch(d3_pos, d3_len, mid, mcnt); }
            if (t + 3 < thi) get_desc(t + 3, d3_pos, d3_len, d3_par);
        }
        if (t + 1 < thi) { if constexpr (PK7) key_load7(t + 1, rn, vn, validn); else key_load(t + 1, kn, vn, validn); par_next = par_t1; }

        carry();
        if (parent != cur_parent) {
            if (cur_parent != 0xFFFFFFFFu) flush(cur_parent);
            if (tid == 0) {
                const u32 seg = atomicAdd(a.seg_counter, 1u);
                if (seg >= a.max_segs) atomicOr(a.err, FJ_ERR_POOL);
                misc[M_SEG] = seg;
            }
            cur_parent = parent;
        }
        for (u32 b = tid; b <= F; b += NT) hist[b] = 0;
        __syncthreads();

        u32 br[KPT];
        if (hotb == 0xFFFFFFFFu) {
#pragma unroll
            for (int i = 0; i < KPT; ++i) {
                const u32 b = (valid & (1u << i)) ? ((FJ_HW1(k[i]) >> sh32) & FM) : F;
                br[i] = (b << 16) | atomicAdd(&hist[b], 1u);
            }
            const u32 bl = br[KPT - 1] >> 16;
            const u32 cand = (u32)__builtin_amdgcn_readfirstlane((int)bl);
            if (__popcll(__ballot(bl == cand)) >= 8) hotb = cand;
        } else {
            u32 seen = 0;
#pragma unroll
            for (int i = 0; i < KPT; ++i) {
                const u32 b = (valid & (1u << i)) ? ((FJ_HW1(k[i]) >> sh32) & FM) : F;
                const u64 m = __ballot(b == hotb);
                const u32 n = (u32)__popcll(m);
                seen += n;
                u32 r;
                if (n >= 2) {
                    const int leader = __builtin_ctzll(m);
                    u32 base = 0;
                    if ((int)lane == leader) base = atomicAdd(&hist[hotb], n);
                    base = (u32)__builtin_amdgcn_readlane((int)base, leader);
                    if (b == hotb) r = base + (u32)__popcll(m & ((1ull << lane) - 1ull));
                    else r = atomicAdd(&hist[b], 1u);
                } else {
                    r = atomicAdd(&hist[b], 1u);
                }
                br[i] = (b << 16) | r;
            }
            if (seen < 8) hotb = 0xFFFFFFFFu;
        }
        __syncthreads();

        u32 cnt = 0, tot = 0, nf = 0, km = 0, kr = 0, kb = 0, l0 = 0;
        if (wave * 64 < F) {
            u64 x = 0;
            if (tid < F) {
                cnt = hist[tid];
                tot = st_left + cnt;
                nf = tot & ~(LINE - 1);
                km = nf ? ((st_fill + nf - 1) >> FJ_CHUNK_LOG) : 0;
                const u32 rl = run_left(st_cur, tid);
                kr = RUNS ? (km > rl ? (km - rl + RU - 1u) >> RL : 0u) : km;
                x = (u64)cnt | ((u64)(nf >> LINE_LOG) << 20) | ((u64)kr << 40);
            }
            u64 inc = x;
#pragma unroll
            for (int d = 1; d < 64; d <<= 1) {
                const u64 y = __shfl_up(inc, d, 64);
                if ((int)lane >= d) inc += y;
            }
            if (lane == 63) wsum[wave] = inc;
            kb = (u32)((inc - x) >> 40); l0 = (u32)(((inc - x) >> 20) & 0xFFFFFu);
            if (tid < F) toff[tid] = (u32)((inc - x) & 0xFFFFFu);
        }
        __syncthreads();
        if (wave * 64 < F) {
            u64 woff = 0;
            for (u32 w = 0; w < wave; ++w) woff += wsum[w];
            if (tid < F) {
                const u32 to = toff[tid] + (u32)(woff & 0xFFFFFu);
                toff[tid] = to;
                l0 += (u32)((woff >> 20) & 0xFFFFFu);
                kb += (u32)(woff >> 40);
                if (tid == F - 1) {
                    toff[F] = to + cnt;
                    const u32 need = kb + kr;
                    misc[M_NLINES] = l0 + (nf >> LINE_LOG);
                    misc[M_NEED] = need;
                    if (need > misc[M_SLAB_REM]) take_slabs(need);
                }
            }
        }
        __syncthreads();

#pragma unroll
        for (int i = 0; i < KPT; ++i) {
            const u32 d = toff[br[i] >> 16] + (br[i] & 0xFFFFu);
            tile_k[d] = k[i];
            if (HAS_VALS) tile_v[d] = v[i];
        }
        if (wave * 64 < F) {
            const bool own = tid < F;
            const u32 f0 = st_fill, c0 = st_cur, tb = own ? toff[tid] : 0u;
            const u32 nl = own ? (nf >> LINE_LOG) : 0u;
            auto put = [&](u32 pb, u32 pf0, u32 pc0, u32 pkb, u32 ptb, u32 pleft, u32 pl0, u32 j) {
                const u32 q = j << LINE_LOG, pq = pf0 + q, kk = pq >> FJ_CHUNK_LOG, off = pq & (FJ_CHUNK - 1);
                const u32 id = kk == 0 ? pc0 : chunk_id(kk, pc0, pkb, pb);
                const u32 dst = id < cap ? id * FJ_CHUNK + off : FJ_DIR_INVALID;
                const u32 lc = j == 0 ? pleft : 0u;
                const u32 sidx = ptb + q + 32u - pleft;
                line_desc[pl0 + j] = ((u64)dst << 32) | ((u64)pb << 22) | ((u64)lc << 17) | sidx;
            };
            const u32 avg2 = (2u * T / LINE) >> a.fan_log;
            const u32 own_lines = avg2 > 4u ? avg2 : 4u;
            for (u32 j = 0; j < nl && j < own_lines; ++j) put(tid, f0, c0, kb, tb, st_left, l0, j);
            u64 big = __ballot(nl > own_lines);
            while (big) {
                const int src = __builtin_ctzll(big);
                big &= big - 1;
                const u32 pf0 = (u32)__builtin_amdgcn_readlane((int)f0, src), pc0 = (u32)__builtin_amdgcn_readlane((int)c0, src);
                const u32 pkb = (u32)__builtin_amdgcn_readlane((int)kb, src), ptb = (u32)__builtin_amdgcn_readlane((int)tb, src);
                const u32 pleft = (u32)__builtin_amdgcn_readlane((int)st_left, src), pl0 = (u32)__builtin_amdgcn_readlane((int)l0, src);
                const u32 pnl = (u32)__builtin_amdgcn_readlane((int)nl, src);
                for (u32 j = own_lines + lane; j < pnl; j += 64) put(wave * 64 + (u32)src, pf0, pc0, pkb, ptb, pleft, pl0, j);
            }
        }
        if (tid < F) {
            const u32 b = tid, f0 = st_fill, c0 = st_cur, n0 = st_nch, tb = toff[b];
            const u32 outb = (parent * F + b) << FJ_DIR_CNT_BITS;
            const u64 segw = (u64)misc[M_SEG] << 32;
            for (u32 kk = 1; kk <= km; ++kk) {
                const u32 id = chunk_id(kk, c0, kb, b);
                if (id < cap) { a.out_dir[id] = outb | FJ_CHUNK; a.out_rel[id] = segw | (n0 + kk - 1); }
            }
            pend_cnt = cnt; pend_nf = nf; pend_tb = tb;
            st_cur = km ? chunk_id(km, c0, kb, b) : c0;
            st_fill = f0 + nf - (km << FJ_CHUNK_LOG);
            st_nch = n0 + km;
        }
        __syncthreads();

        if (!FLAT && tid < TC) { t_chunk[tid] = mid; t_cnt[tid] = mcnt; }
        const u32 nl = misc[M_NLINES];
        constexpr u32 WK = 2, WLPL = LINE / WK;
        for (u32 e = tid; e < nl * WLPL; e += NT) {
            const u32 l = e / WLPL, q = (e % WLPL) * WK;
            const u64 d = line_desc[l];
            const u32 dst = (u32)(d >> 32);
            if (dst != FJ_DIR_INVALID) {
                const u32 w = (u32)d, b = w >> 22, lc = (w >> 17) & 31u, sidx = (w & 0x1FFFFu) - 32u;
                u64 r[WK], rv[WK];
#pragma unroll
                for (int i = 0; i < (int)WK; ++i) {
                    const u32 vi = q + i;
                    const bool in_lo = vi < lc;
                    const u64* sk = in_lo ? (lo_k + b * LOS + vi) : (tile_k + (sidx + vi));
                    r[i] = *sk;
                    if (HAS_VALS) { const u64* sv = in_lo ? (lo_v + b * LOS + vi) : (tile_v + (sidx + vi)); rv[i] = *sv; }
                }
                u64x2 r0; r0.x = r[0]; r0.y = r[1];
                *reinterpret_cast<u64x2*>(a.out_keys + (u64)dst + q) = r0;
                if (HAS_VALS) { u64x2 w0; w0.x = rv[0]; w0.y = rv[1]; *reinterpret_cast<u64x2*>(a.out_vals + (u64)dst + q) = w0; }
            }
        }
        if (tid == 0) commit_units(misc[M_NEED]);
        __syncthreads();
    }
    carry();
    flush(cur_parent);
    for (u32 j = tid; j < (misc[M_SLAB_REM] << RL); j += NT) { const u32 id = misc[M_SLAB_CUR] + j; if (id < cap) a.out_dir[id] = FJ_DIR_INVALID; }
}

template <typename T, typename In, typename Out>
__device__ __forceinline__ T fj_block_scan(In value_at, Out put, u32 n) {
    __shared__ T wtot[4][16];
    const u32 tid = threadIdx.x, lane = tid & 63, wave = tid >> 6;
    T carry = 0;
    for (u32 base = 0; base < n; base += 16384) {
        T x[4][4], sum[4], inc[4];
#pragma unroll
        for (int j = 0; j < 4; ++j) {
            const u32 e0 = base + 4u * ((u32)j * 1024u + tid);
#pragma unroll
            for (int k = 0; k < 4; ++k) x[j][k] = e0 + k < n ? (T)value_at(e0 + k) : (T)0;
            sum[j] = x[j][0] + x[j][1] + x[j][2] + x[j][3];
            T v = sum[j];
#pragma unroll
            for (int d = 1; d < 64; d <<= 1) { const T y = __shfl_up(v, d, 64); if ((int)lane >= d) v += y; }
            inc[j] = v;
            if (lane == 63) wtot[j][wave] = v;
        }
        __syncthreads();
        T before = carry, total = carry;
#pragma unroll
        for (int j = 0; j < 4; ++j) {
            T mine = 0, all = 0;
            for (u32 w = 0; w < 16; ++w) { const T c = wtot[j][w]; all += c; if (w < wave) mine += c; }
            T run = total + mine + inc[j] - sum[j];
            const u32 e0 = base + 4u * ((u32)j * 1024u + tid);
#pragma unroll
            for (int k = 0; k < 4; ++k) { if (e0 + k < n) put(e0 + k, run); run += x[j][k]; }
            total += all;
        }
        (void)before;
        carry = total;
        __syncthreads();
    }
    return carry;
}

__global__ __launch_bounds__(1024) void fj_level_scan(u32* __restrict__ bchunks, u32* __restrict__ boff, u32 n, u32 tc,
                                                      u32* __restrict__ toff) {
    __shared__ u64 wtot[4][16];
    const u32 tid = threadIdx.x, lane = tid & 63, wave = tid >> 6;
    const float rtc = tc ? 1.0f / (float)tc : 0.f;
    auto tiles_of = [&](u32 c) -> u32 {
        if (!tc) return 0u;
        u32 q = (u32)((float)c * rtc);
        while (q * tc < c) ++q;
        while (q && (q - 1) * tc >= c) --q;
        return q;
    };
    u64 carry = 0;
    for (u32 base = 0; base < n; base += 16384) {
        uint4 x[4]; u64 sum[4], inc[4];
#pragma unroll
        for (int j = 0; j < 4; ++j) {
            const u32 e0 = base + 4u * ((u32)j * 1024u + tid);
            x[j] = make_uint4(0, 0, 0, 0);
            if (e0 < n) { x[j] = *reinterpret_cast<const uint4*>(bchunks + e0); *reinterpret_cast<uint4*>(bchunks + e0) = make_uint4(0, 0, 0, 0); }
            sum[j] = ((u64)x[j].x + x[j].y + x[j].z + x[j].w) | ((u64)(tiles_of(x[j].x) + tiles_of(x[j].y) + tiles_of(x[j].z) + tiles_of(x[j].w)) << 32);
            u64 v = sum[j];
#pragma unroll
            for (int d = 1; d < 64; d <<= 1) { const u64 y = __shfl_up(v, d, 64); if ((int)lane >= d) v += y; }
            inc[j] = v;
            if (lane == 63) wtot[j][wave] = v;
        }
        __syncthreads();
        u64 total = carry;
#pragma unroll
        for (int j = 0; j < 4; ++j) {
            u64 mine = 0, all = 0;
            for (u32 w = 0; w < 16; ++w) { const u64 c = wtot[j][w]; all += c; if (w < wave) mine += c; }
            u64 run = total + mine + inc[j] - sum[j];
            const u32 e0 = base + 4u * ((u32)j * 1024u + tid);
            if (e0 < n) {
                uint4 ob, ot;
                ob.x = (u32)run; ot.x = (u32)(run >> 32); run += (u64)x[j].x | ((u64)tiles_of(x[j].x) << 32);
                ob.y = (u32)run; ot.y = (u32)(run >> 32); run += (u64)x[j].y | ((u64)tiles_of(x[j].y) << 32);
                ob.z = (u32)run; ot.z = (u32)(run >> 32); run += (u64)x[j].z | ((u64)tiles_of(x[j].z) << 32);
                ob.w = (u32)run; ot.w = (u32)(run >> 32);
                *reinterpret_cast<uint4*>(boff + e0) = ob;
                if (tc) *reinterpret_cast<uint4*>(toff + e0) = ot;
            }
            total += all;
        }
        carry = total;
        __syncthreads();
    }
    if (tid == 0) { boff[n] = (u32)carry; if (tc) toff[n] = (u32)(carry >> 32); }
}

__global__ __launch_bounds__(1024) void fj_level_scan_wide(const u32* __restrict__ bchunks, u32* __restrict__ boff, u32 n, u32 tc,
                                                           u32* __restrict__ toff) {
    __shared__ u64 wtot[2][16];
    const u32 tid = threadIdx.x, lane = tid & 63, wave = tid >> 6, g = blockIdx.x;
    const u32 magic = tc > 1 ? (u32)((0x100000000ull + tc - 1) / tc) : 0u;
    auto tiles_of = [&](u32 c) -> u32 {
        if (tc <= 1) return tc ? c : 0u;
        const u32 q = __umulhi(c + tc - 1u, magic);
        return (q && (q - 1u) * tc >= c) ? q - 1u : q;
    };
    auto packed = [&](const uint4& x) -> u64 {
        return ((u64)x.x + x.y + x.z + x.w) | ((u64)(tiles_of(x.x) + tiles_of(x.y) + tiles_of(x.z) + tiles_of(x.w)) << 32);
    };
    const u32 e0 = g * 4096u + 4u * tid;
    uint4 x = make_uint4(0, 0, 0, 0);
    if (e0 < n) x = *reinterpret_cast<const uint4*>(bchunks + e0);
    u64 pre = 0;
#pragma unroll 4
    for (u32 j = 0; j < g; ++j) pre += packed(*reinterpret_cast<const uint4*>(bchunks + 4u * (j * 1024u + tid)));
    const u64 own = packed(x);
    u64 inc = own;
#pragma unroll
    for (int d = 1; d < 64; d <<= 1) {
        const u64 y = __shfl_up(inc, d, 64), z = __shfl_up(pre, d, 64);
        if ((int)lane >= d) { inc += y; pre += z; }
    }
    if (lane == 63) { wtot[0][wave] = inc; wtot[1][wave] = pre; }
    __syncthreads();
    u64 run = inc - own;
    for (u32 w = 0; w < 16; ++w) { run += wtot[1][w]; if (w < wave) run += wtot[0][w]; }
    if (e0 < n) {
        uint4 ob, ot;
        ob.x = (u32)run; ot.x = (u32)(run >> 32); run += (u64)x.x | ((u64)tiles_of(x.x) << 32);
        ob.y = (u32)run; ot.y = (u32)(run >> 32); run += (u64)x.y | ((u64)tiles_of(x.y) << 32);
        ob.z = (u32)run; ot.z = (u32)(run >> 32); run += (u64)x.z | ((u64)tiles_of(x.z) << 32);
        ob.w = (u32)run; ot.w = (u32)(run >> 32); run += (u64)x.w | ((u64)tiles_of(x.w) << 32);
        *reinterpret_cast<uint4*>(boff + e0) = ob;
        if (tc) *reinterpret_cast<uint4*>(toff + e0) = ot;
        if (e0 + 4u == n) { boff[n] = (u32)run; if (tc) toff[n] = (u32)(run >> 32); }
    }
}

template <bool BALANCE>
__device__ __forceinline__ void fj_tile_expand_one(const u32* __restrict__ boff, const u32* __restrict__ toff, u32 n, u32 tc,
                                                   uint4* __restrict__ tiles, u32 t) {
    u32 lo = 0, hi = n;
    while (hi - lo > 1) { const u32 mid = (lo + hi) >> 1; if (toff[mid] <= t) lo = mid; else hi = mid; }
    u32 step = tc;
    if (BALANCE) {
        const u32 k = toff[lo + 1] - toff[lo], c = boff[lo + 1] - boff[lo];
        if (k > 1 && k <= tc) step = (c + k - 1) / k;
    }
    const u32 pos = boff[lo] + (t - toff[lo]) * step;
    const u32 rem = boff[lo + 1] - pos;
    tiles[t] = make_uint4(pos, rem < step ? rem : step, lo, 0);
}

__global__ __launch_bounds__(1024) void fj_scan_u32_to_u64(const u32* __restrict__ in, u64* __restrict__ out, u32 n) {
    const u64 total = fj_block_scan<u64>([&](u32 i) { return in[i]; }, [&](u32 i, u64 v) { out[i] = v; }, n);
    if (threadIdx.x == 0) out[n] = total;
}

template <u32 RL>
__global__ __launch_bounds__(256) void fj_level_lists(const u32* __restrict__ dir, const u64* __restrict__ rel, const u32* __restrict__ nalloc,
                               u32 cap, const u32* __restrict__ boff, const u32* __restrict__ seg_off, u32 fan_mask,
                               u32 max_segs, u32* __restrict__ list,
                               u32 nb, u32 tc, const u32* __restrict__ toff, uint4* __restrict__ tiles, u32 max_tiles,
                               u32* __restrict__ zero_tail, u32* __restrict__ clr) {
    u32 n = *nalloc; if (n > cap) n = cap;
    const u32 stride = gridDim.x * blockDim.x, gtid = blockIdx.x * blockDim.x + threadIdx.x;
    if (clr) for (u32 i = gtid; i < nb / 4u; i += stride) reinterpret_cast<uint4*>(clr)[i] = make_uint4(0, 0, 0, 0);
    if (tc) {
        u32 total = toff[nb];
        if (total > max_tiles) total = max_tiles;
        for (u32 t = gtid; t < max_tiles; t += stride) {
            if (t < total) { if (zero_tail) fj_tile_expand_one<true>(boff, toff, nb, tc, tiles, t); else fj_tile_expand_one<false>(boff, toff, nb, tc, tiles, t); }
            else if (zero_tail) zero_tail[t] = 0;
        }
    }
    if constexpr (RL > 0) {
        constexpr u32 R = 1u << RL;
        const u32 nr = n >> RL;
        for (u32 i0 = gtid; i0 < nr; i0 += 2 * stride) {
            u32 ev[2][R]; u64 r[2][R];
#pragma unroll
            for (int u = 0; u < 2; ++u) {
                const u32 i = i0 + u * stride;
#pragma unroll
                for (u32 j = 0; j < R; ++j) { ev[u][j] = FJ_DIR_INVALID; r[u][j] = 0; }
                if (i < nr) {
                    if constexpr (RL == 2) {
                        const uint4 e = reinterpret_cast<const uint4*>(dir)[i];
                        ev[u][0] = e.x; ev[u][1] = e.y; ev[u][2] = e.z; ev[u][3] = e.w;
                    } else {
                        const uint2 e = reinterpret_cast<const uint2*>(dir)[i];
                        ev[u][0] = e.x; ev[u][1] = e.y;
                    }
#pragma unroll
                    for (u32 j = 0; j < R; j += 2) {
                        const ulonglong2 q = reinterpret_cast<const ulonglong2*>(rel)[((u64)i * R + j) >> 1];
                        r[u][j] = q.x; r[u][j + 1] = q.y;
                    }
                }
            }
            u32 base[2]; bool ok[2];
#pragma unroll
            for (int u = 0; u < 2; ++u) {
                u32 e0 = FJ_DIR_INVALID; u64 r0 = 0;
#pragma unroll
                for (int j = (int)R - 1; j >= 0; --j) if (ev[u][j] != FJ_DIR_INVALID) { e0 = ev[u][j]; r0 = r[u][j]; }
                const u32 b = e0 >> FJ_DIR_CNT_BITS, seg = (u32)(r0 >> 32);
                ok[u] = e0 != FJ_DIR_INVALID && seg < max_segs;
                base[u] = ok[u] ? boff[b] + seg_off[(u64)seg * (fan_mask + 1) + (b & fan_mask)] : 0;
            }
#pragma unroll
            for (int u = 0; u < 2; ++u) {
                if (!ok[u]) continue;
                const u32 id = R * (i0 + u * stride);
#pragma unroll
                for (u32 j = 0; j < R; ++j)
                    if (ev[u][j] != FJ_DIR_INVALID) list[base[u] + (u32)r[u][j]] = (((ev[u][j] & FJ_DIR_CNT_MASK) - 1u) << 24) | (id + j);
            }
        }
    } else {
        for (u32 i0 = gtid; i0 < n; i0 += 4 * stride) {
            u32 e[4]; u64 r[4];
#pragma unroll
            for (int u = 0; u < 4; ++u) {
                const u32 i = i0 + u * stride;
                e[u] = i < n ? dir[i] : FJ_DIR_INVALID;
                r[u] = i < n ? rel[i] : 0;
            }
            u32 pos[4]; bool ok[4];
#pragma unroll
            for (int u = 0; u < 4; ++u) {
                const u32 b = e[u] >> FJ_DIR_CNT_BITS, seg = (u32)(r[u] >> 32);
                ok[u] = e[u] != FJ_DIR_INVALID && seg < max_segs;
                pos[u] = ok[u] ? boff[b] + seg_off[(u64)seg * (fan_mask + 1) + (b & fan_mask)] + (u32)r[u] : 0;
            }
#pragma unroll
            for (int u = 0; u < 4; ++u)
                if (ok[u]) list[pos[u]] = (((e[u] & FJ_DIR_CNT_MASK) - 1u) << 24) | (i0 + u * stride);
        }
    }
}

template <bool FUSED>
__global__ __launch_bounds__(1024) void fj_level_lists_binned(const u32* __restrict__ dir, const u64* __restrict__ rel, const u32* __restrict__ nalloc,
                               u32 cap, u32* __restrict__ boff_g, const u32* __restrict__ seg_off, u32 fan_mask,
                               u32 max_segs, u32* __restrict__ list,
                               u32 nb, u32 tc, u32* __restrict__ toff_g, uint4* __restrict__ tiles, u32 max_tiles,
                               u32* __restrict__ zero_tail, u32* __restrict__ bchunks) {
    constexpr u32 NT = 1024, BLK = 4096, NBMAX = 512;
    __shared__ u32 hist[NBMAX + 1];
    __shared__ u32 wsum[NBMAX / 64];
    __shared__ uint2 ent[BLK];
    __shared__ u32 boff_s[FUSED ? NBMAX + 1 : 1], toff_s[FUSED ? NBMAX + 1 : 1];
    __shared__ u64 wtot[NBMAX / 64];
    __shared__ u32 s_last;
    const u32* boff = FUSED ? boff_s : boff_g;
    const u32* toff = FUSED ? toff_s : toff_g;
    u32 n = *nalloc; if (n > cap) n = cap;
    const u32 tid = threadIdx.x, lane = tid & 63, wave = tid >> 6;
    const u32 stride = gridDim.x * NT, gtid = blockIdx.x * NT + tid;
    if constexpr (FUSED) {
        const float rtc = tc ? 1.0f / (float)tc : 0.f;
        auto tiles_of = [&](u32 c) -> u32 {
            if (!tc) return 0u;
            u32 q = (u32)((float)c * rtc);
            while (q * tc < c) ++q;
            while (q && (q - 1) * tc >= c) --q;
            return q;
        };
        u64 mine = 0, v = 0;
        if (tid < NBMAX) {
            const u32 c = tid < nb ? bchunks[tid] : 0u;
            mine = (u64)c | ((u64)tiles_of(c) << 32);
            v = mine;
#pragma unroll
            for (int d = 1; d < 64; d <<= 1) { const u64 y = __shfl_up(v, d, 64); if ((int)lane >= d) v += y; }
            if (lane == 63) wtot[wave] = v;
        }
        __syncthreads();
        if (tid == 0) { __threadfence(); s_last = atomicAdd(&bchunks[nb], 1u) == gridDim.x - 1 ? 1u : 0u; }
        if (tid < NBMAX) {
            u64 woff = 0;
            for (u32 w = 0; w < wave; ++w) woff += wtot[w];
            const u64 ex = woff + v - mine;
            if (tid < nb) { boff_s[tid] = (u32)ex; toff_s[tid] = (u32)(ex >> 32); }
            if (tid == nb - 1) { boff_s[nb] = (u32)(ex + mine); toff_s[nb] = (u32)((ex + mine) >> 32); }
        }
        __syncthreads();
        if (s_last) { if (tid < nb) bchunks[tid] = 0; if (tid == 0) bchunks[nb] = 0; }
        if (blockIdx.x == 0 && tid <= nb) { boff_g[tid] = boff_s[tid]; if (tc) toff_g[tid] = toff_s[tid]; }
    }
    if (tc) {
        u32 total = toff[nb];
        if (total > max_tiles) total = max_tiles;
        for (u32 t = gtid; t < max_tiles; t += stride) {
            if (t < total) { if (zero_tail) fj_tile_expand_one<true>(boff, toff, nb, tc, tiles, t); else fj_tile_expand_one<false>(boff, toff, nb, tc, tiles, t); }
            else if (zero_tail) zero_tail[t] = 0;
        }
    }
    for (u32 base = blockIdx.x * BLK; base < n; base += gridDim.x * BLK) {
        if (tid < NBMAX) hist[tid] = 0;
        __syncthreads();
        u32 e[4]; u64 r[4];
#pragma unroll
        for (int u = 0; u < 4; ++u) {
            const u32 i = base + (u32)u * NT + tid;
            e[u] = i < n ? dir[i] : FJ_DIR_INVALID;
            r[u] = i < n ? rel[i] : 0;
        }
        u32 pos[4], slot[4], bk[4]; bool ok[4];
#pragma unroll
        for (int u = 0; u < 4; ++u) {
            const u32 b = e[u] >> FJ_DIR_CNT_BITS, seg = (u32)(r[u] >> 32);
            ok[u] = e[u] != FJ_DIR_INVALID && seg < max_segs && b < nb;
            bk[u] = ok[u] ? b : 0u;
            pos[u] = ok[u] ? boff[b] + seg_off[(u64)seg * (fan_mask + 1) + (b & fan_mask)] + (u32)r[u] : 0;
        }
#pragma unroll
        for (int u = 0; u < 4; ++u) slot[u] = ok[u] ? atomicAdd(&hist[bk[u]], 1u) : 0u;
        __syncthreads();
        u32 v = 0, inc = 0;
        if (tid < NBMAX) {
            v = hist[tid]; inc = v;
#pragma unroll
            for (int d = 1; d < 64; d <<= 1) { const u32 y = __shfl_up(inc, d, 64); if ((int)lane >= d) inc += y; }
            if (lane == 63) wsum[wave] = inc;
        }
        __syncthreads();
        if (tid < NBMAX) {
            u32 woff = 0;
            for (u32 w = 0; w < wave; ++w) woff += wsum[w];
            hist[tid] = woff + inc - v;
            if (tid == NBMAX - 1) hist[NBMAX] = woff + inc;
        }
        __syncthreads();
#pragma unroll
        for (int u = 0; u < 4; ++u)
            if (ok[u]) ent[hist[bk[u]] + slot[u]] = make_uint2(pos[u], (((e[u] & FJ_DIR_CNT_MASK) - 1u) << 24) | (base + (u32)u * NT + tid));
        __syncthreads();
        const u32 total = hist[NBMAX];
        for (u32 j = tid; j < total; j += NT) { const uint2 x = ent[j]; list[x.x] = x.y; }
        __syncthreads();
    }
}

__global__ __launch_bounds__(1024) void fj_dir_rank_kernel(u32* __restrict__ dir, u32 n, u32 b_lo, u32 nbk, u32 fan, u64* __restrict__ rel,
                                                           u32* __restrict__ seg_off, u32* __restrict__ bchunks, u32* __restrict__ nalloc) {
    __shared__ u32 h[1u << FJ_MAX_FAN_LOG];
    const u32 tid = threadIdx.x, base = blockIdx.x * 4096u;
    if (tid < (1u << FJ_MAX_FAN_LOG)) h[tid] = 0;
    __syncthreads();
    u32 bb[4], rr[4];
#pragma unroll
    for (int u = 0; u < 4; ++u) {
        const u32 i = base + (u32)u * 1024u + tid;
        bb[u] = FJ_DIR_INVALID; rr[u] = 0;
        if (i < n) {
            const u32 e = dir[i], b = (e >> FJ_DIR_CNT_BITS) - b_lo, cnt = e & FJ_DIR_CNT_MASK;
            const bool ok = e != FJ_DIR_INVALID && b < nbk && cnt >= 1u && cnt <= FJ_CHUNK;
            if (ok) bb[u] = b;
            dir[i] = ok ? ((b << FJ_DIR_CNT_BITS) | cnt) : FJ_DIR_INVALID;
        }
        const bool ok = bb[u] != FJ_DIR_INVALID;
        const u64 m = __ballot(ok);
        if (m) {
            const u32 b0 = (u32)__builtin_amdgcn_readlane((int)bb[u], __builtin_ctzll(m));
            if (__ballot(ok && bb[u] != b0) == 0) {
                u32 wb = 0;
                if ((threadIdx.x & 63u) == (u32)__builtin_ctzll(m)) wb = atomicAdd(&h[b0], (u32)__popcll(m));
                wb = (u32)__builtin_amdgcn_readlane((int)wb, __builtin_ctzll(m));
                if (ok) rr[u] = wb + (u32)__popcll(m & ((1ull << (threadIdx.x & 63u)) - 1ull));
            } else if (ok) rr[u] = atomicAdd(&h[bb[u]], 1u);
        }
    }
    __syncthreads();
    if (tid < nbk) { const u32 c = h[tid]; if (c) seg_off[(u64)blockIdx.x * fan + tid] = atomicAdd(&bchunks[tid], c); }
#pragma unroll
    for (int u = 0; u < 4; ++u) {
        const u32 i = base + (u32)u * 1024u + tid;
        if (bb[u] != FJ_DIR_INVALID) rel[i] = ((u64)blockIdx.x << 32) | rr[u];
    }
    if (blockIdx.x == 0 && tid == 0) *nalloc = n;
}

template <int NT, int KPT, int LINE_LOG, bool HAS_VALS, bool FLAT, bool PROBE_SIDE, int RLOG = FJ_RUN_LOG, bool PK7 = false, bool POS = false>
hipError_t launch_part0(const FjPartArgs& a, u32 grid, hipStream_t s) {
    const u32 F = 1u << a.fan_log;
    const PartLds L = part_lds_layout(NT * KPT, F, 1u << LINE_LOG, HAS_VALS, NT / 64);
    auto kern = fj_partition_kernel<NT, KPT, LINE_LOG, HAS_VALS, FLAT, PROBE_SIDE, RLOG, PK7, POS>;
    hipError_t e = fj_set_max_lds_once(reinterpret_cast<const void*>(kern), L.total);
    if (e != hipSuccess) return e;
    hipLaunchKernelGGL(kern, dim3(grid), dim3(NT), L.total, s, a);
    return hipGetLastError();
}

template <int NT, int KPT, int LINE_LOG, bool HAS_VALS, bool FLAT, bool PROBE_SIDE>
hipError_t launch_part1(const FjPartArgs& a, u32 grid, hipStream_t s) {
    if constexpr (FLAT && HAS_VALS) {
        if (a.vals_pos) {
            if (a.run_log == 0) return launch_part0<NT, KPT, LINE_LOG, HAS_VALS, FLAT, PROBE_SIDE, 0, false, true>(a, grid, s);
            if (a.run_log != FJ_RUN_LOG) return hipErrorInvalidValue;
            return launch_part0<NT, KPT, LINE_LOG, HAS_VALS, FLAT, PROBE_SIDE, FJ_RUN_LOG, false, true>(a, grid, s);
        }
    }
    if constexpr (FLAT) { if (a.run_log == 0) return launch_part0<NT, KPT, LINE_LOG, HAS_VALS, FLAT, PROBE_SIDE, 0>(a, grid, s); }
    if (a.run_log != FJ_RUN_LOG) return hipErrorInvalidValue;
    return launch_part0<NT, KPT, LINE_LOG, HAS_VALS, FLAT, PROBE_SIDE, FJ_RUN_LOG>(a, grid, s);
}

template <int NT, int KPT, int LINE_LOG, bool HAS_VALS, bool FLAT>
hipError_t launch_part(const FjPartArgs& a, u32 grid, hipStream_t s) {
    if constexpr (!HAS_VALS) {
        if (a.side == 0) return launch_part1<NT, KPT, LINE_LOG, HAS_VALS, FLAT, false>(a, grid, s);
    }
    return launch_part1<NT, KPT, LINE_LOG, HAS_VALS, FLAT, true>(a, grid, s);
}

template <int NT, int KPT, bool HAS_VALS>
hipError_t launch_part2(const FjPartArgs& a, int line_log, u32 grid, hipStream_t s) {
    const bool flat = a.in_list == nullptr;
    if (line_log == 3) return flat ? launch_part<NT, KPT, 3, HAS_VALS, true>(a, grid, s) : launch_part<NT, KPT, 3, HAS_VALS, false>(a, grid, s);
    return flat ? launch_part<NT, KPT, 4, HAS_VALS, true>(a, grid, s) : launch_part<NT, KPT, 4, HAS_VALS, false>(a, grid, s);
}

}

hipError_t fj_set_max_lds_once(const void* fn, u32 bytes) {
    struct Seen { const void* fn; int dev; u32 bytes; };
    static std::mutex mu;
    static std::vector<Seen> seen;
    int dev = 0;
    hipError_t e = hipGetDevice(&dev);
    if (e != hipSuccess) return e;
    std::lock_guard<std::mutex> lk(mu);
    for (Seen& x : seen)
        if (x.fn == fn && x.dev == dev) {
            if (x.bytes >= bytes) return hipSuccess;
            e = hipFuncSetAttribute(fn, hipFuncAttributeMaxDynamicSharedMemorySize, (int)bytes);
            if (e == hipSuccess) x.bytes = bytes;
            return e;
        }
    e = hipFuncSetAttribute(fn, hipFuncAttributeMaxDynamicSharedMemorySize, (int)bytes);
    if (e == hipSuccess) seen.push_back({fn, dev, bytes});
    return e;
}

u32 fj_partition_lds_bytes(u32 fan_log, bool vals, int line_log) {
    const u32 F = 1u << fan_log;
    if (vals) return part_lds_layout(1024 * 4, F, 1u << line_log, true, 16).total;
    return part_lds_layout(1024 * 8, F, 1u << line_log, false, 16).total;
}

u32 fj_partition_tile_chunks(u32 fan_log, bool vals) { (void)fan_log; return vals ? 16u : 32u; }


hipError_t fj_launch_partition(const FjPartArgs& a, bool vals, int line_log, u32 grid, hipStream_t s) {
    if (a.shift < 32) return hipErrorInvalidValue;
    if (a.fan_log > FJ_MAX_FAN_LOG || a.slab < (1u << FJ_RUN_LOG) || (a.slab & ((1u << FJ_RUN_LOG) - 1u))) return hipErrorInvalidValue;
    if (a.in_pk7) {
        if (!a.in_list || a.run_log != FJ_RUN_LOG) return hipErrorInvalidValue;
        if (vals) {
            if (a.fan_log == 9 && line_log != 3) return hipErrorInvalidValue;
            return line_log == 3 ? launch_part0<1024, 4, 3, true, false, true, FJ_RUN_LOG, true>(a, grid, s)
                                 : launch_part0<1024, 4, 4, true, false, true, FJ_RUN_LOG, true>(a, grid, s);
        }
        if (line_log != 4) return hipErrorInvalidValue;
        const u32 g = a.fan_log == 9 ? grid : (grid < 256 ? grid : 256);
        return a.side == 0 ? launch_part0<1024, 8, 4, false, false, false, FJ_RUN_LOG, true>(a, g, s)
                           : launch_part0<1024, 8, 4, false, false, true, FJ_RUN_LOG, true>(a, g, s);
    }
    if (a.fan_log == 9) {
        if (vals) return line_log == 3 ? launch_part2<1024, 4, true>(a, 3, grid, s) : hipErrorInvalidValue;
        return launch_part2<1024, 8, false>(a, line_log, grid, s);
    }
    if (vals) {
        return launch_part2<1024, 4, true>(a, line_log, grid, s);
    }
    return launch_part2<1024, 8, false>(a, line_log, grid < 256 ? grid : 256, s);
}

hipError_t fj_launch_group(const FjChunkSet& cs, u32 tc, u32* toff, uint4* tiles, u32 max_tiles, u32* zero_tail, hipStream_t s) {
    if (cs.nb & 3u) return hipErrorInvalidValue;
    static_assert(FJ_RUN_LOG == 1 || FJ_RUN_LOG == 2, "fj_level_lists reads a run's directory words with one 8-B or 16-B load");
    if (cs.run_log != 0 && cs.run_log != FJ_RUN_LOG) return hipErrorInvalidValue;
    if (cs.run_log == 0 && cs.nb <= 512 && cs.cap >= 4096) {
        const u32 blocks = (cs.cap + 4095u) / 4096u;
        if (blocks <= 512u) {
            hipLaunchKernelGGL(fj_level_lists_binned<true>, dim3(blocks), dim3(1024), 0, s, cs.dir, cs.rel, cs.alloc, cs.cap, cs.boff,
                               cs.seg_off, cs.fan_mask, cs.max_segs, cs.list, cs.nb, tc, toff, tiles, max_tiles, zero_tail, cs.bchunks);
        } else {
            hipLaunchKernelGGL(fj_level_scan, dim3(1), dim3(1024), 0, s, cs.bchunks, cs.boff, cs.nb, tc, toff);
            hipLaunchKernelGGL(fj_level_lists_binned<false>, dim3(blocks < 4096u ? blocks : 4096u), dim3(1024), 0, s, cs.dir, cs.rel, cs.alloc, cs.cap, cs.boff,
                               cs.seg_off, cs.fan_mask, cs.max_segs, cs.list, cs.nb, tc, toff, tiles, max_tiles, zero_tail, cs.bchunks);
        }
        return hipGetLastError();
    }
    const bool wide = cs.nb >= 8192u && cs.nb <= (1u << 19);
    if (wide) hipLaunchKernelGGL(fj_level_scan_wide, dim3((cs.nb + 4095u) / 4096u), dim3(1024), 0, s, cs.bchunks, cs.boff, cs.nb, tc, toff);
    else hipLaunchKernelGGL(fj_level_scan, dim3(1), dim3(1024), 0, s, cs.bchunks, cs.boff, cs.nb, tc, toff);
    auto kern = cs.run_log ? fj_level_lists<FJ_RUN_LOG> : fj_level_lists<0>;
    hipLaunchKernelGGL(kern, dim3(2048), dim3(256), 0, s, cs.dir, cs.rel, cs.alloc, cs.cap, cs.boff, cs.seg_off,
                       cs.fan_mask, cs.max_segs, cs.list, cs.nb, tc, toff, tiles, max_tiles, zero_tail, wide ? cs.bchunks : (u32*)nullptr);
    return hipGetLastError();
}

hipError_t fj_launch_dir_rank(u32* dir, u32 n, u32 b_lo, u32 nbk, u32 fan, u64* rel, u32* seg_off, u32* bchunks, u32* nalloc, hipStream_t s) {
    if (nbk > (1u << FJ_MAX_FAN_LOG) || fan < nbk || n == 0) return hipErrorInvalidValue;
    hipLaunchKernelGGL(fj_dir_rank_kernel, dim3((n + 4095u) / 4096u), dim3(1024), 0, s, dir, n, b_lo, nbk, fan, rel, seg_off, bchunks, nalloc);
    return hipGetLastError();
}

hipError_t fj_launch_scan_u32_to_u64(const u32* in, u64* out, u32 n, hipStream_t s) {
    hipLaunchKernelGGL(fj_scan_u32_to_u64, dim3(1), dim3(1024), 0, s, in, out, n);
    return hipGetLastError();
}
```

### flash_hash_join_amd/csrc/fj_plan.hip

```cpp
#include "fj_host.h"

namespace fjh {

namespace { thread_local std::string g_err; thread_local fj_timings g_last; }

int set_err(const char* fmt, ...) {
    char buf[1024];
    va_list ap; va_start(ap, fmt); vsnprintf(buf, sizeof buf, fmt, ap); va_end(ap);
    g_err = buf;
    return 1;
}
fj_timings& last_timings() { return g_last; }

Options& options() { static Options o; return o; }
static int set_option_value(Options& o, const char* name, long long value);
Options::Options() {
    static const char* const legacy[] = {"FJ_RADIX_THRESHOLD", "FJ_SCALAR_HBM_TABLE", "FJ_BLOOM_AUTO", "FJ_BLOOM_AUTO_MAX_HIT_BP", "FJ_BLOOM_VARIANT", "FJ_PLAN_TARGET_KEYS",
                                         "FJ_MAT_SINGLE_PASS", "FJ_PERSISTENT_MIN_ITEMS", "FJ_JOIN_ITEMS_TARGET", "FJ_JOIN_WIDE", "FJ_DIST_LOOPBACK", "FJ_DIST_INJECT_FAIL",
                                         "FJ_DIST_RESERVE_ALWAYS", "FJ_DIST_SPLIT_ALWAYS", "FJ_DIST_ONE_COMM", "FJ_EMIT_TAGGED"};
    for (const char* name : legacy)
        if (getenv(name)) fprintf(stderr, "flash_hash_join_amd: the environment variable %s is no longer read (use FJ_OPTIONS=\"name=value,...\" or fj_set_option; see include/flashjoin.h)\n", name);
    const char* e = getenv("FJ_OPTIONS");
    if (!e) return;
    std::string str(e);
    size_t pos = 0;
    while (pos < str.size()) {
        size_t end = str.find(',', pos);
        if (end == std::string::npos) end = str.size();
        const std::string item = str.substr(pos, end - pos);
        pos = end + 1;
        if (item.empty()) continue;
        const size_t eq = item.find('=');
        char* tail = nullptr;
        const long long value = eq == std::string::npos ? 0 : strtoll(item.c_str() + eq + 1, &tail, 10);
        if (eq == std::string::npos || eq == 0 || tail == item.c_str() + eq + 1 || *tail != '\0')
            fprintf(stderr, "flash_hash_join_amd: FJ_OPTIONS: ignoring '%s' (want name=integer)\n", item.c_str());
        else if (set_option_value(*this, item.substr(0, eq).c_str(), value))
            fprintf(stderr, "flash_hash_join_amd: FJ_OPTIONS: ignoring '%s' (%s)\n", item.c_str(), fj_last_error());
    }
}

int get_buf(fj_ctx* c, int slot, size_t bytes, void** out) {
    Buf& b = c->bufs[slot];
    if (bytes == 0) bytes = 16;
    if (b.bytes < bytes) {
        if (b.p) { HIPCHK(hipFree(b.p)); c->ws_bytes -= b.bytes; b.p = nullptr; b.bytes = 0; }
        size_t want = (bytes + 255) & ~(size_t)255;
        hipError_t e = hipMalloc(&b.p, want);
        if (e != hipSuccess) return set_err("hipMalloc(%zu bytes) for workspace slot %d failed: %s", want, slot, hipGetErrorString(e));
        b.bytes = want; c->ws_bytes += want;
    }
    *out = b.p;
    return 0;
}


int get_zeroed_buf(fj_ctx* c, int slot, size_t bytes, void** out, hipStream_t s) {
    const size_t before = c->bufs[slot].bytes;
    if (get_buf(c, slot, bytes, out)) return 1;
    if (c->bufs[slot].bytes != before || c->slot_dirty[slot]) {
        HIPCHK(hipMemsetAsync(*out, 0, c->bufs[slot].bytes, s));
        c->slot_dirty[slot] = false;
    }
    return 0;
}

int plan_npass(int bits) { return bits <= FJ_MAX_FAN_LOG ? (bits > 0 ? 1 : 0) : (bits <= 2 * FJ_MAX_FAN_LOG ? 2 : (bits + FJ_MAX_FAN_LOG - 1) / FJ_MAX_FAN_LOG); }

void plan_passes(Plan& p, bool extra_first) {
    p.npass = plan_npass(p.bits);
    for (int i = 0; i < p.npass; ++i) {
        const int rem = p.bits % p.npass;
        p.fan_log[i] = p.bits / p.npass + ((extra_first ? i < rem : i >= p.npass - rem) ? 1 : 0);
    }
}

Plan make_plan(size_t nb, int top_bits, bool want_bloom, u64 target_override) {
    Plan p;
    const u64 target = target_override ? std::min<u64>(target_override, options().plan_target_keys)
                                       : options().plan_target_keys;
    if (nb > target) {
        u64 parts = (nb + target - 1) / target;
        while ((1ull << p.bits) < parts) ++p.bits;
    }
    if (!target_override && target == FJ_PART_TARGET_KEYS && (nb >> p.bits) > FJ_PLAN_BUMP_KEYS && p.bits < top_bits - 32) {
        const int nb1 = p.bits == 0 ? 5 : p.bits + 1;
        if (p.bits == 0 || plan_npass(nb1) == plan_npass(p.bits)) p.bits = nb1;
    }
    if (p.bits > 0 && p.bits < 5) p.bits = 5;
    if (p.bits > top_bits - 32) p.bits = top_bits - 32;
    plan_passes(p, true);
    if (want_bloom && p.npass >= 2) {
        if (p.npass == 2)
            while (p.fan_log[0] < FJ_MAX_FAN_LOG && p.fan_log[1] > 4 && (nb >> p.fan_log[0]) > FJ_BLOOM_GOOD_KEYS) { ++p.fan_log[0]; --p.fan_log[1]; }
        int lvl_bits = 0;
        for (int i = 0; i + 1 < p.npass; ++i) lvl_bits += p.fan_log[i];
        if ((nb >> lvl_bits) <= FJ_BLOOM_MAX_KEYS) p.bloom_level = p.npass - 1;
    }
    return p;
}


void pass_init(PassIter& it, int side, bool has_vals, size_t n, const Plan& plan, int top_bits) {
    it = PassIter();
    it.side = side; it.has_vals = has_vals; it.n = n; it.plan = plan; it.used = top_bits;
    it.lbound = (n + FJ_CHUNK - 1) / FJ_CHUNK;
}

u32 pass_groups(u64 chunks, u64 rows, u32 tile_chunks, u32 F) {
    const u64 g64 = std::min<u64>(chunks / tile_chunks, rows / ((u64)F * 128));
    return (u32)std::min<u64>(512, std::max<u64>(1, g64));
}

int pass_prepare(fj_ctx* c, PassIter& it, u32 appends, hipStream_t s) {
    const int i = it.i;
    it.F = 1u << it.plan.fan_log[i];
    it.used -= it.plan.fan_log[i];
    it.appends = appends ? appends : 1;
    it.tile_chunks = fj_partition_tile_chunks((u32)it.plan.fan_log[i], it.has_vals);
    it.Gmax = pass_groups(it.lbound, it.n, it.tile_chunks, it.F);
    if (c->reserve_cus) it.Gmax = std::min<u32>(it.Gmax, c->reserve_cus < c->num_cus ? c->num_cus - c->reserve_cus : 1u);
    if (it.piece_rows && it.appends > 1 && !it.have_prev)
        it.Gmax = std::min(it.Gmax, pass_groups((it.piece_rows + FJ_CHUNK - 1) / FJ_CHUNK, it.piece_rows, it.tile_chunks, it.F));
    const u32 F = it.F, G = it.Gmax, parents = it.parents;
    const u64 nb_out = (u64)parents * F;
    const u64 cap64 = (it.n / FJ_CHUNK + 1 + (((u64)(G + parents) * F << FJ_RUN_LOG) + (u64)(G + 1) * fj_slab_for(it.appends)) * it.appends + 3) & ~3ull;
    if (cap64 >= (1ull << 24) || nb_out >= (1u << 22))
        return set_err("relation of %zu rows is too large for one GPU's chunk directory", it.n);
    FjChunkSet cs{};
    cs.cap = (u32)cap64; cs.nb = (u32)nb_out; cs.n_flat = 0; cs.fan_mask = F - 1; cs.max_segs = (G + parents + 2) * it.appends;
    cs.run_log = (!it.have_prev && it.i == 0 && F <= 256) ? 0u : (u32)FJ_RUN_LOG;
    const int base = it.side * W_SIDE_STRIDE + (it.slot & 1) * W_KINDS;
    it.cs_base = base;
    void* p;
    if (get_buf(c, base + W_POOL_K, cap64 * FJ_CHUNK * 8, &p)) return 1; cs.keys = (u64*)p;
    cs.vals = nullptr;
    if (it.has_vals) { if (get_buf(c, base + W_POOL_V, cap64 * FJ_CHUNK * 8, &p)) return 1; cs.vals = (u64*)p; }
    if (get_buf(c, base + W_DIR, cap64 * 4, &p)) return 1; cs.dir = (u32*)p;
    if (get_buf(c, base + W_REL, cap64 * 8, &p)) return 1; cs.rel = (u64*)p;
    if (get_buf(c, base + W_LIST, cap64 * 4, &p)) return 1; cs.list = (u32*)p;
    if (get_zeroed_buf(c, base + W_BCHUNKS, nb_out * 4 + 16, &p, s)) return 1; cs.bchunks = (u32*)p;
    if (get_buf(c, base + W_BOFF, (nb_out + 1) * 4, &p)) return 1; cs.boff = (u32*)p;
    if (get_buf(c, base + W_SEGOFF, (size_t)cs.max_segs * F * 4, &p)) return 1; cs.seg_off = (u32*)p;
    cs.alloc = it.alloc_word ? it.alloc_word : &c->d_sc->alloc[it.side * 4 + i];
    it.cs = cs;
    return 0;
}

int pass_launch(fj_ctx* c, PassIter& it, const u64* keys, const u64* vals, size_t n, hipStream_t s, int* ev_cursor) {
    const FjChunkSet& cs = it.cs;
    FjPartArgs a{};
    u32 G = it.Gmax;
    if (it.have_prev) {
        a.in_keys = it.prev.keys; a.in_vals = it.prev.vals; a.in_list = it.prev.list; a.in_dir = it.prev.dir;
        a.in_tiles = it.tiles; a.in_ntiles = it.ntiles; a.n_flat = 0;
    } else {
        a.in_keys = keys; a.in_vals = vals; a.in_list = nullptr; a.in_dir = nullptr; a.in_tiles = nullptr; a.in_ntiles = nullptr; a.n_flat = n;
        a.vals_pos = it.has_vals && it.vals_pos ? 1u : 0u;
        G = std::min(G, pass_groups((n + FJ_CHUNK - 1) / FJ_CHUNK, n, it.tile_chunks, it.F));
    }
    a.parent0 = 0;
    a.out_keys = cs.keys; a.out_vals = cs.vals; a.out_dir = cs.dir; a.out_rel = cs.rel; a.seg_off = cs.seg_off;
    a.bchunks = cs.bchunks; a.alloc = cs.alloc; a.seg_counter = it.seg_word ? it.seg_word : &c->d_sc->seg_counter[it.side * 4 + it.i];
    a.cap_chunks = cs.cap; a.max_segs = cs.max_segs;
    a.err = it.err_word ? it.err_word : &c->d_sc->err;
    if (it.have_prev && it.in_pk7) { a.in_pk7 = 1; a.in_b0 = it.in_b0; a.in_top_shift = it.in_top_shift; }
    a.shift = (u32)it.used; a.fan_log = (u32)it.plan.fan_log[it.i]; a.slab = fj_slab_for(it.appends); a.run_log = cs.run_log; a.side = (u32)it.side;
    const int line_log = (it.has_vals && it.F > 256) ? 3 : 4;
    if (ev_cursor) HIPCHK(hipEventRecord(c->ev[E_PK0 + 2 * (*ev_cursor)], s));
    HIPCHK(fj_launch_partition(a, it.has_vals, line_log, G, s));
    if (ev_cursor) { HIPCHK(hipEventRecord(c->ev[E_PK0 + 2 * (*ev_cursor) + 1], s)); ++*ev_cursor; }
    return 0;
}

bool bloom_stage_follows(const PassIter& it, int level) { return it.plan.bloom_level == level && it.bloom_build && !it.bloom_done; }

void join_item_geometry(u64 nparts, size_t np, u64 chunk_bound, u32* tc, u64* max_items) {
    const u64 pchunks = (np + FJ_CHUNK - 1) / FJ_CHUNK;
    const u64 bound = std::max<u64>(chunk_bound, pchunks);
    const u64 avg = std::max<u64>(1, bound / nparts);
    u64 want = 1;
    const u64 target_items = options().join_items_target;
    if (nparts < target_items) want = std::min<u64>((target_items + nparts - 1) / nparts, std::max<u64>(1, (pchunks / nparts) / 32));
    *tc = (u32)(want > 1 ? std::max<u64>(8, (avg * 9 / 8 + want - 1) / want) : std::max<u64>(512, 4 * avg));
    *max_items = bound / *tc + nparts + 1;
}

bool wide_join_planned(bool materialize, size_t nb, size_t np_eff, int bits) {
    if (materialize || bits <= 0 || options().join_wide == 0) return false;
    if (options().join_wide == 1) return true;
    return np_eff <= 3 * nb;
}

int level_finish(fj_ctx* c, PassIter& it, bool final_level, hipStream_t s) {
    const FjChunkSet& cs = it.cs;
    u32 tc = 0; u64 max_tiles = 0; u32* zero_tail = nullptr;
    if (bloom_stage_follows(it, it.i)) tc = fj_bloom_tile_chunks();
    else if (!final_level) tc = fj_partition_tile_chunks((u32)it.plan.fan_log[it.i], it.has_vals);
    else if (it.want_items) {
        join_item_geometry(cs.nb, it.n, it.lbound, &tc, &max_tiles);
        if (it.item_tc_max && tc > it.item_tc_max) { tc = it.item_tc_max; max_tiles = std::max<u64>(it.lbound, (it.n + FJ_CHUNK - 1) / FJ_CHUNK) / tc + cs.nb + 1; }
    }
    if (tc && !max_tiles) max_tiles = it.lbound / tc + cs.nb + 1;
    if (max_tiles >= (1ull << 31)) return set_err("internal error: tile table too large");
    u32* toff = nullptr; uint4* tiles = nullptr;
    void* p;
    if (tc) {
        if (get_buf(c, it.cs_base + W_TOFF, ((size_t)cs.nb + 1) * 4, &p)) return 1; toff = (u32*)p;
        if (get_buf(c, it.cs_base + W_TILES, max_tiles * sizeof(uint4), &p)) return 1; tiles = (uint4*)p;
        if (final_level) {
            if (get_buf(c, it.part_count_slot, (size_t)max_tiles * 4, &p)) return 1;
            it.part_count = zero_tail = (u32*)p; it.items_cap = (u32)max_tiles;
        }
    }
    HIPCHK(fj_launch_group(cs, tc, toff, tiles, (u32)max_tiles, zero_tail, s));
    it.tiles = tiles; it.ntiles = toff ? toff + cs.nb : nullptr; it.toff = toff;
    return 0;
}

int pass_complete(fj_ctx* c, PassIter& it, hipStream_t s) {
    const FjChunkSet& cs = it.cs;
    it.lbound = it.n / FJ_CHUNK + 1 + (u64)(it.Gmax + it.parents) * it.F * it.appends;
    ++it.i;
    if (level_finish(c, it, it.i == it.plan.npass, s)) return 1;
    it.prev = cs; it.have_prev = true;
    it.parents = cs.nb;
    ++it.slot;
    if (it.save_level == it.i) it.saved = cs;
    return 0;
}

int bloom_stage(fj_ctx* c, PassIter& it, hipStream_t s) {
    const FjChunkSet in = it.prev;
    const u32 G = c->num_cus;
    const u32 nw = fj_bloom_waves_per_group();
    const u64 max_segs = (u64)nw * ((u64)in.nb + G) + 16;
    const u64 cap64 = it.n / FJ_CHUNK + 1 + max_segs + (u64)fj_bloom_slab_chunks() * nw * G;
    if (cap64 >= (1ull << 24)) return set_err("relation of %zu rows is too large for one GPU's chunk directory", it.n);
    FjChunkSet cs{};
    cs.cap = (u32)cap64; cs.nb = in.nb; cs.n_flat = 0; cs.fan_mask = 0; cs.max_segs = (u32)max_segs;
    const int base = it.side * W_SIDE_STRIDE + (it.slot & 1) * W_KINDS;
    void* p;
    if (get_buf(c, base + W_POOL_K, cap64 * FJ_CHUNK * 8, &p)) return 1; cs.keys = (u64*)p;
    cs.vals = nullptr;
    if (get_buf(c, base + W_DIR, cap64 * 4, &p)) return 1; cs.dir = (u32*)p;
    if (get_buf(c, base + W_REL, cap64 * 8, &p)) return 1; cs.rel = (u64*)p;
    if (get_buf(c, base + W_LIST, cap64 * 4, &p)) return 1; cs.list = (u32*)p;
    if (get_zeroed_buf(c, base + W_BCHUNKS, (size_t)cs.nb * 4 + 16, &p, s)) return 1; cs.bchunks = (u32*)p;
    if (get_buf(c, base + W_BOFF, ((size_t)cs.nb + 1) * 4, &p)) return 1; cs.boff = (u32*)p;
    if (get_buf(c, base + W_SEGOFF, (size_t)cs.max_segs * 4, &p)) return 1; cs.seg_off = (u32*)p;
    cs.alloc = &c->d_sc->alloc[it.side * 4 + 3];
    FjBloomArgs a{};
    a.pkeys = in.keys; a.plist = in.list; a.pnb = in.nb; a.tiles = it.tiles; a.toff = it.toff;
    a.bkeys = it.bloom_build->keys; a.blist = it.bloom_build->list; a.bboff = it.bloom_build->boff;
    a.out_keys = cs.keys; a.out_dir = cs.dir; a.out_rel = cs.rel; a.seg_off = cs.seg_off; a.bchunks = cs.bchunks;
    a.alloc = cs.alloc; a.seg_counter = &c->d_sc->seg_counter[it.side * 4 + 3];
    a.cap_chunks = cs.cap; a.max_segs = cs.max_segs; a.err = &c->d_sc->err; a.survivors = &c->d_sc->bloom_survivors;
    a.prebuilt = it.bloom_prebuilt; a.bucket_keys = it.bloom_bucket_keys;
    HIPCHK(hipEventRecord(c->ev[E_BF0], s));
    HIPCHK(fj_launch_bloom_filter(a, G, options().bloom_variant, s));
    HIPCHK(hipEventRecord(c->ev[E_BF1], s));
    it.cs = cs; it.cs_base = base;
    it.lbound = it.n / FJ_CHUNK + 1 + max_segs;
    it.bloom_done = true;
    if (level_finish(c, it, it.i == it.plan.npass, s)) return 1;
    it.prev = cs;
    ++it.slot;
    return 0;
}

int run_passes(fj_ctx* c, PassIter& it, const u64* keys, const u64* vals, hipStream_t s, FjChunkSet* out, int* ev_cursor) {
    while (it.i < it.plan.npass) {
        if (bloom_stage_follows(it, it.i) && bloom_stage(c, it, s)) return 1;
        if (pass_prepare(c, it, 1, s)) return 1;
        if (pass_launch(c, it, keys, vals, it.n, s, ev_cursor)) return 1;
        if (pass_complete(c, it, s)) return 1;
    }
    if (!it.have_prev) {
        it.prev = FjChunkSet();
        it.prev.keys = const_cast<u64*>(keys); it.prev.vals = const_cast<u64*>(vals); it.prev.n_flat = it.n; it.prev.list = nullptr; it.prev.nb = 1;
    }
    *out = it.prev;
    return 0;
}

int clear_plan_scalars(fj_ctx* c, hipStream_t s) {
    HIPCHK(hipMemsetAsync(c->d_sc, 0, offsetof(Scalars, owner_counts), s));
    return 0;
}

void begin_plan(fj_ctx* c) {
    if (c->plan_in_flight) for (bool& d : c->slot_dirty) d = true;
    c->plan_in_flight = true;
}
void end_plan(fj_ctx* c) { c->plan_in_flight = false; }

void drop_pending(fj_ctx* c) { c->pend = Pending(); }

int begin_step(fj_ctx* c, const char* who) {
    if (who && c->st.active) return set_err("%s: a stream join is open on this context (fj_stream_finish it first)", who);
    drop_pending(c);
    return 0;
}

int read_scalars(fj_ctx* c, hipStream_t s) {
    HIPCHK(hipMemcpyAsync(c->h_sc, c->d_sc, sizeof(Scalars), hipMemcpyDeviceToHost, s));
    HIPCHK(hipStreamSynchronize(s));
    return 0;
}

float ev_ms(fj_ctx* c, int a, int b) { float ms = 0.f; (void)hipEventElapsedTime(&ms, c->ev[a], c->ev[b]); return ms; }

void plan_timings(fj_ctx* c, const Plan& plan, u64 partitions, int evc, fj_timings* t) {
    t->path = 0; t->passes = plan.npass; t->radix_bits = plan.bits; t->partitions = partitions;
    t->build_phase_ms = ev_ms(c, E_START, E_BUILD);
    t->join_ms = ev_ms(c, E_PPART, E_JOIN);
    t->probe_phase_ms = ev_ms(c, E_BUILD, E_JOIN);
    t->total_ms = ev_ms(c, E_START, E_JOIN);
    for (int i = 0; i < evc && i < 4; ++i) t->probe_part_kernel_ms[i] = ev_ms(c, E_PK0 + 2 * i, E_PK0 + 2 * i + 1);
    t->bloom_level = plan.bloom_level;
    if (plan.bloom_level > 0) { t->filter_ms = ev_ms(c, E_BF0, E_BF1); t->filter_survivors = c->h_sc->bloom_survivors; }
}

int stamps_begin(unsigned long long** dbg, hipStream_t s) {
    static unsigned long long* dbg_buf = nullptr;
    if (!dbg_buf) HIPCHK(hipMalloc((void**)&dbg_buf, 4096 * 8 * 8));
    HIPCHK(hipMemsetAsync(dbg_buf, 0, 4096 * 8 * 8, s));
    *dbg = dbg_buf;
    return 0;
}
int stamps_report(const char* label, const unsigned long long* dbg, u32 nitems, hipStream_t s) {
    std::vector<unsigned long long> h(4096 * 8);
    HIPCHK(hipStreamSynchronize(s));
    HIPCHK(hipMemcpy(h.data(), dbg, h.size() * 8, hipMemcpyDeviceToHost));
    double acc[6] = {0, 0, 0, 0, 0, 0}; int n = 0;
    unsigned long long tmin = ~0ull, tmax = 0;
    for (int i = 0; i < 4096 && i < (int)nitems; ++i) {
        const unsigned long long* r = &h[i * 8];
        if (!r[0] || !r[5]) continue;
        for (int j = 1; j <= 5; ++j) acc[j] += (double)(r[j] - r[j - 1]) * 0.01;
        if (r[0] < tmin) tmin = r[0];
        if (r[5] > tmax) tmax = r[5];
        ++n;
    }
    if (n == 0) n = 1;
    fprintf(stderr, "[%s] items=%d  meta+init=%.2f  build=%.2f  buildsync=%.2f  probe=%.2f  fin=%.2f us (means); first 4096 items span %.1f us\n",
            label, n, acc[1] / n, acc[2] / n, acc[3] / n, acc[4] / n, acc[5] / n, (double)(tmax - tmin) * 0.01);
    return 0;
}

static int set_option_value(Options& o, const char* name, long long value) {
    if (!strcmp(name, "radix_threshold")) { if (value < 0) return set_err("fj_set_option: radix_threshold must be >= 0"); o.radix_threshold = (size_t)value; return 0; }
    if (!strcmp(name, "scalar_hbm_table")) { o.scalar_hbm_table = value != 0; return 0; }
    if (!strcmp(name, "plan_target_keys")) { if (value < 16 || value > (long long)FJ_PART_TARGET_KEYS) return set_err("fj_set_option: plan_target_keys must be 16..%u", FJ_PART_TARGET_KEYS); o.plan_target_keys = (u32)value; return 0; }
    if (!strcmp(name, "bloom_auto")) { o.bloom_auto = value != 0; return 0; }
    if (!strcmp(name, "mat_single_pass")) { o.mat_single_pass = value != 0; return 0; }
    if (!strcmp(name, "bloom_auto_max_hit_bp")) { if (value < 0 || value > 10000) return set_err("fj_set_option: bloom_auto_max_hit_bp must be 0..10000"); o.bloom_auto_max_hit_bp = (int)value; return 0; }
    if (!strcmp(name, "bloom_variant")) { if (value < 0 || value > 2) return set_err("fj_set_option: bloom_variant must be 0..2"); o.bloom_variant = (int)value; return 0; }
    if (!strcmp(name, "join_wide")) { if (value < 0 || value > 2) return set_err("fj_set_option: join_wide must be 0..2"); o.join_wide = (int)value; return 0; }
    if (!strcmp(name, "persistent_min_items")) { if (value < 0) return set_err("fj_set_option: persistent_min_items must be >= 0"); o.persistent_min_items = (u32)std::min<long long>(value, 0xFFFFFFFFll); return 0; }
    if (!strcmp(name, "lab_hooks")) { if (value < 0 || value > 0xFFFF) return set_err("fj_set_option: lab_hooks is a mask of FJ_HOOK_* bits"); o.lab_hooks = (u32)value; return 0; }
    if (!strcmp(name, "join_items_target")) { if (value < 1 || value > (1 << 20)) return set_err("fj_set_option: join_items_target must be 1..1048576"); o.join_items_target = (u32)value; return 0; }
    if (!strcmp(name, "mm_heavy_keys")) { if (value < 0 || value > 1) return set_err("fj_set_option: mm_heavy_keys must be 0 or 1"); o.mm_heavy_keys = (int)value; return 0; }
    if (!strcmp(name, "mm_heavy_outer")) { if (value < 0 || value > 1) return set_err("fj_set_option: mm_heavy_outer must be 0 or 1"); o.mm_heavy_outer = (int)value; return 0; }
    return set_err("fj_set_option: unknown option '%s'", name);
}

}
using namespace fjh;

void fj_set_error_string(const char* msg) { fjh::g_err = msg ? msg : ""; }

extern "C" {

const char* fj_last_error(void) { return fjh::g_err.c_str(); }
const char* fj_version(void) { return "flash_hash_join_amd 0.6 (gfx950)"; }
int fj_abi_version(void) { return FJ_ABI_VERSION; }

int fj_set_option(const char* name, long long value) {
    if (!name) return set_err("fj_set_option: null name");
    return fjh::set_option_value(options(), name, value);
}

long long fj_get_option(const char* name) {
    const Options& o = options();
    if (name && !strcmp(name, "radix_threshold")) return (long long)o.radix_threshold;
    if (name && !strcmp(name, "scalar_hbm_table")) return o.scalar_hbm_table;
    if (name && !strcmp(name, "persistent_min_items")) return o.persistent_min_items;
    if (name && !strcmp(name, "join_wide")) return o.join_wide;
    if (name && !strcmp(name, "plan_target_keys")) return o.plan_target_keys;
    if (name && !strcmp(name, "bloom_variant")) return o.bloom_variant;
    if (name && !strcmp(name, "bloom_auto")) return o.bloom_auto;
    if (name && !strcmp(name, "mat_single_pass")) return o.mat_single_pass;
    if (name && !strcmp(name, "bloom_auto_max_hit_bp")) return o.bloom_auto_max_hit_bp;
    if (name && !strcmp(name, "lab_hooks")) return o.lab_hooks;
    if (name && !strcmp(name, "join_items_target")) return o.join_items_target;
    if (name && !strcmp(name, "mm_heavy_keys")) return o.mm_heavy_keys;
    if (name && !strcmp(name, "mm_heavy_outer")) return o.mm_heavy_outer;
    set_err("fj_get_option: unknown option '%s'", name ? name : "(null)");
    return -1;
}

uint64_t fj_key_mix64(uint64_t key) { return fj_key_mix(key); }
uint64_t fj_key_unmix64(uint64_t mixed) { return fj_key_unmix(mixed); }

int fj_device_count(void) {
    int n = 0;
    if (hipGetDeviceCount(&n) != hipSuccess) return 0;
    return n;
}

int fj_initialize(void) {
    int n = 0;
    hipError_t e = hipGetDeviceCount(&n);
    if (e != hipSuccess || n <= 0) return set_err("fj_initialize: no usable HIP device (%s)", e == hipSuccess ? "device count is 0" : hipGetErrorString(e));
    return 0;
}

fj_ctx* fj_ctx_create(int device) {
    int n = 0;
    hipError_t e = hipGetDeviceCount(&n);
    if (e != hipSuccess || device < 0 || device >= n) { set_err("fj_ctx_create: HIP device %d not available (%d devices)", device, n); return nullptr; }
    DeviceGuard guard(device);
    if (guard.err != hipSuccess) { set_err("fj_ctx_create: hipSetDevice(%d) failed", device); return nullptr; }
    fj_ctx* c = new fj_ctx();
    c->device = device;
    { int ncu = 0; if (hipDeviceGetAttribute(&ncu, hipDeviceAttributeMultiprocessorCount, device) == hipSuccess && ncu > 0) c->num_cus = (u32)ncu; }
    bool ok = hipMalloc((void**)&c->d_sc, sizeof(Scalars)) == hipSuccess &&
              hipHostMalloc((void**)&c->h_sc, sizeof(Scalars), hipHostMallocDefault) == hipSuccess &&
              hipMemset(c->d_sc, 0, sizeof(Scalars)) == hipSuccess;
    for (int i = 0; ok && i < E_NEV; ++i) ok = hipEventCreate(&c->ev[i]) == hipSuccess;
    ok = ok && hipStreamCreateWithFlags(&c->side, hipStreamNonBlocking) == hipSuccess;
    ok = ok && hipEventCreateWithFlags(&c->pk_ev, hipEventDisableTiming) == hipSuccess && hipHostMalloc((void**)&c->pk_h, 67 * 8, hipHostMallocDefault) == hipSuccess;
    if (!ok) { set_err("fj_ctx_create: allocating context scratch failed: %s", hipGetErrorString(hipGetLastError())); delete c; return nullptr; }
    return c;
}

void fj_ctx_destroy(fj_ctx* c) {
    if (!c) return;
    DeviceGuard guard(c->device);
    for (auto& b : c->bufs) if (b.p) (void)hipFree(b.p);
    for (int i = 0; i < E_NEV; ++i) (void)hipEventDestroy(c->ev[i]);
    if (c->side) (void)hipStreamDestroy(c->side);
    if (c->pk_ev) (void)hipEventDestroy(c->pk_ev);
    if (c->pk_h) (void)hipHostFree(c->pk_h);
    for (void* p : c->stage) if (p) (void)hipHostFree(p);
    if (c->d_sc) (void)hipFree(c->d_sc);
    if (c->h_sc) (void)hipHostFree(c->h_sc);
    delete c;
}

size_t fj_ctx_workspace_bytes(const fj_ctx* c) { return c ? c->ws_bytes : 0; }
void fj_ctx_reserve_cus(fj_ctx* c, unsigned n) { if (c) c->reserve_cus = n; }

int fj_ctx_trim(fj_ctx* c) {
    if (!c) c = host_ctx();
    if (!c) return 0;
    FJ_ENTER(c);
    if (begin_step(c, "fj_ctx_trim")) return 1;
    HIPCHK(hipDeviceSynchronize());
    for (auto& b : c->bufs) if (b.p) { HIPCHK(hipFree(b.p)); b.p = nullptr; b.bytes = 0; }
    c->ws_bytes = 0;
    return 0;
}
int fj_generate_build(fj_ctx* c, uint64_t* d_keys, uint64_t* d_vals, uint64_t first, size_t n, void* stream) {
    FJ_ENTER(c);
    HIPCHK(fj_launch_gen_build(d_keys, d_vals, first, n, (hipStream_t)stream));
    return 0;
}

int fj_generate_probe(fj_ctx* c, uint64_t* d_keys, uint64_t first, size_t n, uint64_t build_total, uint64_t seed,
                      uint32_t hit_bp, uint64_t* h_expected_hits, void* stream) {
    if (build_total == 0) return set_err("fj_generate_probe: build_total must be > 0");
    FJ_ENTER(c);
    hipStream_t s = (hipStream_t)stream;
    HIPCHK(hipMemsetAsync(&c->d_sc->expected, 0, sizeof(unsigned long long), s));
    HIPCHK(fj_launch_gen_probe(d_keys, first, n, build_total, seed, hit_bp, &c->d_sc->expected, s));
    HIPCHK(hipMemcpyAsync(&c->h_sc->expected, &c->d_sc->expected, sizeof(unsigned long long), hipMemcpyDeviceToHost, s));
    HIPCHK(hipStreamSynchronize(s));
    if (h_expected_hits) *h_expected_hits = c->h_sc->expected;
    return 0;
}

int fj_debug_partition(fj_ctx* c, const uint64_t* d_keys, const uint64_t* d_vals, size_t n, int total_bits,
                       int hash_top_bits, void* stream, uint64_t* h_out_keys, uint64_t* h_out_vals,
                       uint32_t* h_bucket_of, uint64_t* h_nvalid) {
    if (total_bits < 2 || total_bits > 24) return set_err("fj_debug_partition: total_bits must be 2..24");
    FJ_ENTER(c);
    if (begin_step(c, nullptr)) return 1;
    hipStream_t s = (hipStream_t)stream;
    Plan plan; plan.bits = total_bits;
    plan_passes(plan, true);
    begin_plan(c);
    if (clear_plan_scalars(c, s)) return 1;
    FjChunkSet cs{};
    PassIter dit;
    pass_init(dit, d_vals ? 0 : 1, d_vals != nullptr, n, plan, hash_top_bits);
    if (run_passes(c, dit, d_keys, d_vals, s, &cs, nullptr)) return 1;
    if (read_scalars(c, s)) return 1;
    if (c->h_sc->err) return set_err("fj_debug_partition: device error word 0x%x", c->h_sc->err);
    end_plan(c);
    std::vector<u32> dir(cs.cap), list(cs.cap), boff(cs.nb + 1);
    HIPCHK(hipMemcpy(dir.data(), cs.dir, (size_t)cs.cap * 4, hipMemcpyDeviceToHost));
    HIPCHK(hipMemcpy(list.data(), cs.list, (size_t)cs.cap * 4, hipMemcpyDeviceToHost));
    HIPCHK(hipMemcpy(boff.data(), cs.boff, (size_t)(cs.nb + 1) * 4, hipMemcpyDeviceToHost));
    std::vector<u64> ck(FJ_CHUNK), cv(FJ_CHUNK);
    u64 w = 0;
    for (u32 b = 0; b < cs.nb; ++b) {
        for (u32 i = boff[b]; i < boff[b + 1]; ++i) {
            const u32 id = FJ_LIST_ID(list[i]);
            if (id >= cs.cap) return set_err("fj_debug_partition: list entry %u out of range", id);
            const u32 e = dir[id], cnt = e & FJ_DIR_CNT_MASK;
            if ((e >> FJ_DIR_CNT_BITS) != b) return set_err("fj_debug_partition: chunk %u listed under bucket %u but tagged %u", id, b, e >> FJ_DIR_CNT_BITS);
            if (cnt == 0 || cnt > FJ_CHUNK || cnt != FJ_LIST_CNT(list[i])) return set_err("fj_debug_partition: chunk %u has count %u (list says %u)", id, cnt, FJ_LIST_CNT(list[i]));
            if (w + cnt > n) return set_err("fj_debug_partition: more than %zu rows in the chunk lists", n);
            HIPCHK(hipMemcpy(ck.data(), cs.keys + (size_t)id * FJ_CHUNK, cnt * 8, hipMemcpyDeviceToHost));
            for (u32 j = 0; j < cnt; ++j) h_out_keys[w + j] = fj_key_unmix(ck[j]);
            if (d_vals && h_out_vals) {
                HIPCHK(hipMemcpy(cv.data(), cs.vals + (size_t)id * FJ_CHUNK, cnt * 8, hipMemcpyDeviceToHost));
                memcpy(h_out_vals + w, cv.data(), cnt * 8);
            }
            for (u32 j = 0; j < cnt; ++j) h_bucket_of[w + j] = b;
            w += cnt;
        }
    }
    *h_nvalid = w;
    return 0;
}

int fj_device_malloc(void** p, size_t bytes) { HIPCHK(hipMalloc(p, bytes ? bytes : 16)); return 0; }
int fj_device_free(void* p) { if (p) HIPCHK(hipFree(p)); return 0; }
int fj_memcpy_h2d(void* d, const void* h, size_t bytes) { if (bytes) HIPCHK(hipMemcpy(d, h, bytes, hipMemcpyHostToDevice)); return 0; }
int fj_memcpy_d2h(void* h, const void* d, size_t bytes) { if (bytes) HIPCHK(hipMemcpy(h, d, bytes, hipMemcpyDeviceToHost)); return 0; }
int fj_memcpy_d2d(void* dst, const void* src, size_t bytes) { if (bytes) HIPCHK(hipMemcpy(dst, src, bytes, hipMemcpyDeviceToDevice)); return 0; }

void fj_free_host(void* p) { free(p); }
int fj_last_timings(fj_timings* out) { if (!out) return set_err("fj_last_timings: null"); *out = last_timings(); return 0; }

}
```

Before: 113.9.

## Merge build and probe partition passes into shared kernel launches per level

```diff
diff --git a/flash_hash_join_amd/csrc/fj_host.h b/flash_hash_join_amd/csrc/fj_host.h
--- a/flash_hash_join_amd/csrc/fj_host.h
+++ b/flash_hash_join_amd/csrc/fj_host.h
@@ -123,6 +123,7 @@
     int save_level = 0; FjChunkSet saved{};
     u32* alloc_word = nullptr; u32* seg_word = nullptr; u32* err_word = nullptr;
     bool in_pk7 = false; u32 in_b0 = 0, in_top_shift = 0;
+    double merged_build_share = -1.0;
     bool vals_pos = false;
 };
 
@@ -199,6 +200,7 @@
     u32 lab_hooks = 0;
     u32 join_items_target = 2048;
     int mm_heavy_keys = 0;
+    int merged_levels = 1;
     int mm_heavy_outer = 0;
     Options();
 };
@@ -220,6 +222,7 @@
 int pass_complete(fj_ctx* c, PassIter& it, hipStream_t s);
 int bloom_stage(fj_ctx* c, PassIter& it, hipStream_t s);
 int run_passes(fj_ctx* c, PassIter& it, const u64* keys, const u64* vals, hipStream_t s, FjChunkSet* out, int* ev_cursor);
+int run_passes_merged(fj_ctx* c, PassIter& bit, PassIter& pit, const u64* bk, const u64* pk, hipStream_t s, FjChunkSet* bout, FjChunkSet* pout, int* ev_cursor);
 int clear_plan_scalars(fj_ctx* c, hipStream_t s);
 void begin_plan(fj_ctx* c);
 void end_plan(fj_ctx* c);
@@ -227,7 +230,7 @@
 int begin_step(fj_ctx* c, const char* who);
 int read_scalars(fj_ctx* c, hipStream_t s);
 float ev_ms(fj_ctx* c, int a, int b);
-void plan_timings(fj_ctx* c, const Plan& plan, u64 partitions, int evc, fj_timings* t);
+void plan_timings(fj_ctx* c, const Plan& plan, u64 partitions, int evc, fj_timings* t, double build_share = -1.0);
 int stamps_begin(unsigned long long** dbg, hipStream_t s);
 int stamps_report(const char* label, const unsigned long long* dbg, u32 nitems, hipStream_t s);
 
diff --git a/flash_hash_join_amd/csrc/fj_internal.h b/flash_hash_join_amd/csrc/fj_internal.h
--- a/flash_hash_join_amd/csrc/fj_internal.h
+++ b/flash_hash_join_amd/csrc/fj_internal.h
@@ -42,6 +42,8 @@
     u32 vals_pos;
 };
 
+struct FjPartArgs2 { FjPartArgs b, p; u32 gb, gp; };
+
 struct FjChunkSet {
     u64* keys;
     u64* vals;
@@ -64,6 +66,9 @@
 u32 fj_partition_tile_chunks(u32 fan_log, bool vals);
 hipError_t fj_launch_partition(const FjPartArgs& a, bool vals, int line_log, u32 grid, hipStream_t s);
 hipError_t fj_launch_group(const FjChunkSet& cs, u32 tc, u32* toff, uint4* tiles, u32 max_tiles, u32* zero_tail, hipStream_t s);
+hipError_t fj_launch_partition2(const FjPartArgs& b, u32 gb, const FjPartArgs& p, u32 gp, hipStream_t s);
+struct FjGroupJob { FjChunkSet cs; u32 tc; u32* toff; uint4* tiles; u32 max_tiles; u32* zero_tail; };
+hipError_t fj_launch_group2(const FjGroupJob& b, const FjGroupJob& p, hipStream_t s);
 hipError_t fj_launch_scan_u32_to_u64(const u32* in, u64* out, u32 n, hipStream_t s);
 hipError_t fj_launch_dir_rank(u32* dir, u32 n, u32 b_lo, u32 nbk, u32 fan, u64* rel, u32* seg_off, u32* bchunks, u32* nalloc, hipStream_t s);
 
diff --git a/flash_hash_join_amd/csrc/fj_joins.hip b/flash_hash_join_amd/csrc/fj_joins.hip
--- a/flash_hash_join_amd/csrc/fj_joins.hip
+++ b/flash_hash_join_amd/csrc/fj_joins.hip
@@ -318,7 +318,7 @@
         if (c->h_sc->err & FJ_ERR_POOL) return set_err("internal error: chunk pool exhausted during a partition pass");
         if (!(c->h_sc->err & (FJ_STAT_DUPS | FJ_STAT_EMIT_RETRY | FJ_ERR_LDS_FULL | FJ_ERR_OUTCAP))) {
             end_plan(c);
-            plan_timings(c, plan, ja.nparts, evc, t);
+            plan_timings(c, plan, ja.nparts, evc, t, pit.merged_build_share);
             t->lds_retries = 0;
             *out_count = c->h_sc->total;
             so->done = true;
@@ -386,7 +386,7 @@
     }
     if (c->h_sc->err & FJ_ERR_POOL) return set_err("internal error: chunk pool exhausted during a partition pass");
     end_plan(c);
-    plan_timings(c, plan, ja.nparts, evc, t);
+    plan_timings(c, plan, ja.nparts, evc, t, pit.merged_build_share);
     if (c->h_sc->err & FJ_ERR_LDS_FULL) { *lds_full = true; return 0; }
     *out_count = c->h_sc->total;
     if (materialize) {
@@ -413,6 +413,18 @@
     bit.vals_pos = rid;
     int evc = 0;
     if (plan.bloom_level > 0) bit.save_level = plan.bloom_level;
+    const bool merged = options().merged_levels && !materialize && !rid && bloom != 2 && plan.bloom_level == 0 && plan.npass > 0 && nb > 0 && np > 0;
+    if (merged) {
+        pass_init(pit, 1, false, np, plan, top_bits);
+        pit.want_items = true;
+        if (wide_join_planned(false, nb, np, plan.bits)) pit.item_tc_max = 32;
+        pit.merged_build_share = (double)nb / ((double)nb + (double)np);
+        if (run_passes_merged(c, bit, pit, bk, pk, s, &ja.build, &ja.probe, &evc)) return 1;
+        HIPCHK(hipEventRecord(c->ev[E_PPART], s));
+        ja.avg_build_keys = (u32)std::min<u64>(0xFFFFFFFFu, (u64)nb >> plan.bits);
+        ja.row_ids = 0;
+        return radix_join_tail(c, materialize, ja, plan, np, pit, s, t, evc, out_count, lds_full, top_bits, so);
+    }
     if (run_passes(c, bit, bk, (materialize && !rid) ? bv : nullptr, s, &ja.build, nullptr)) return 1;
     HIPCHK(hipEventRecord(c->ev[E_BUILD], s));
     Plan pplan = plan;
diff --git a/flash_hash_join_amd/csrc/fj_partition.hip b/flash_hash_join_amd/csrc/fj_partition.hip
--- a/flash_hash_join_amd/csrc/fj_partition.hip
+++ b/flash_hash_join_amd/csrc/fj_partition.hip
@@ -33,8 +33,8 @@
 
 enum { M_SLAB_CUR = 0, M_SLAB_REM, M_NEW_BASE, M_NEED, M_NLINES, M_FLUSH, M_SEG, M_NEW_UNITS };
 
-template <int NT, int KPT, int LINE_LOG, bool HAS_VALS, bool FLAT, bool PROBE_SIDE, int RLOG = FJ_RUN_LOG, bool PK7 = false, bool POS = false>
-__global__ __launch_bounds__(NT, 4) void fj_partition_kernel(FjPartArgs a) {
+template <int NT, int KPT, int LINE_LOG, bool HAS_VALS, bool FLAT, int RLOG = FJ_RUN_LOG, bool PK7 = false, bool POS = false>
+__device__ __forceinline__ void fj_partition_body(const FjPartArgs& a, const u32 G, const u32 g) {
     constexpr u32 T = NT * KPT, LINE = 1u << LINE_LOG, TC = T / FJ_CHUNK, NW = NT / 64, LOS = LINE + FJ_LO_PAD;
     static_assert(T % FJ_CHUNK == 0 && TC <= NT && LINE >= 4 && T + 64 < (1u << 17), "tile geometry");
     static_assert(!PK7 || (!FLAT && KPT % 4 == 0), "wire-format chunks come through chunk lists, four keys per load group");
@@ -61,7 +61,6 @@
 
     const u32 Lc = FLAT ? (u32)((a.n_flat + FJ_CHUNK - 1) >> FJ_CHUNK_LOG) : 0u;
     const u32 ntiles = FLAT ? (Lc + TC - 1) / TC : *a.in_ntiles;
-    const u32 G = gridDim.x, g = blockIdx.x;
     const u32 t0 = (u32)(((u64)g * ntiles) / G);
     const u32 nmine = (u32)(((u64)(g + 1) * ntiles) / G) - t0;
     u32 t = 0;
@@ -167,7 +166,7 @@
         const u32 rem = misc[M_SLAB_REM];
         return j < rem ? misc[M_SLAB_CUR] + (j << RL) : misc[M_NEW_BASE] + ((j - rem) << RL);
     };
-    auto rot = [&](u32 b) -> u32 { return ((b * 2654435761u + blockIdx.x * 40503u) >> 13) & (RU - 1u); };
+    auto rot = [&](u32 b) -> u32 { return ((b * 2654435761u + g * 40503u) >> 13) & (RU - 1u); };
     auto run_left = [&](u32 c0, u32 b) -> u32 { return (RUNS && c0 != FJ_DIR_INVALID) ? (RU - 1u) - ((c0 - rot(b)) & (RU - 1u)) : 0u; };
     auto run_step = [&](u32 c0, u32 k) -> u32 { return (c0 & ~(RU - 1u)) | ((c0 + k) & (RU - 1u)); };
     auto chunk_id = [&](u32 kk, u32 c0, u32 ukb, u32 b) -> u32 {
@@ -445,6 +444,19 @@
     for (u32 j = tid; j < (misc[M_SLAB_REM] << RL); j += NT) { const u32 id = misc[M_SLAB_CUR] + j; if (id < cap) a.out_dir[id] = FJ_DIR_INVALID; }
 }
 
+template <int NT, int KPT, int LINE_LOG, bool HAS_VALS, bool FLAT, bool PROBE_SIDE, int RLOG = FJ_RUN_LOG, bool PK7 = false, bool POS = false>
+__global__ __launch_bounds__(NT, 4) void fj_partition_kernel(FjPartArgs a) {
+    fj_partition_body<NT, KPT, LINE_LOG, HAS_VALS, FLAT, RLOG, PK7, POS>(a, gridDim.x, blockIdx.x);
+}
+
+template <int NT, int KPT, int LINE_LOG, bool FLAT, int RLOG>
+__global__ __launch_bounds__(NT, 4) void fj_partition_both_kernel(FjPartArgs2 a) {
+    const u32 g = blockIdx.x;
+    if (g < a.gb) fj_partition_body<NT, KPT, LINE_LOG, false, FLAT, RLOG>(a.b, a.gb, g);
+    __syncthreads();
+    if (g < a.gp) fj_partition_body<NT, KPT, LINE_LOG, false, FLAT, RLOG>(a.p, a.gp, g);
+}
+
 template <typename T, typename In, typename Out>
 __device__ __forceinline__ T fj_block_scan(In value_at, Out put, u32 n) {
     __shared__ T wtot[4][16];
@@ -483,8 +495,8 @@
     return carry;
 }
 
-__global__ __launch_bounds__(1024) void fj_level_scan(u32* __restrict__ bchunks, u32* __restrict__ boff, u32 n, u32 tc,
-                                                      u32* __restrict__ toff) {
+__device__ __forceinline__ void fj_level_scan_body(u32* __restrict__ bchunks, u32* __restrict__ boff, u32 n, u32 tc,
+                                                   u32* __restrict__ toff) {
     __shared__ u64 wtot[4][16];
     const u32 tid = threadIdx.x, lane = tid & 63, wave = tid >> 6;
     const float rtc = tc ? 1.0f / (float)tc : 0.f;
@@ -535,10 +547,10 @@
     if (tid == 0) { boff[n] = (u32)carry; if (tc) toff[n] = (u32)(carry >> 32); }
 }
 
-__global__ __launch_bounds__(1024) void fj_level_scan_wide(const u32* __restrict__ bchunks, u32* __restrict__ boff, u32 n, u32 tc,
-                                                           u32* __restrict__ toff) {
+__device__ __forceinline__ void fj_level_scan_wide_body(const u32* __restrict__ bchunks, u32* __restrict__ boff, u32 n, u32 tc,
+                                                        u32* __restrict__ toff, const u32 g) {
     __shared__ u64 wtot[2][16];
-    const u32 tid = threadIdx.x, lane = tid & 63, wave = tid >> 6, g = blockIdx.x;
+    const u32 tid = threadIdx.x, lane = tid & 63, wave = tid >> 6;
     const u32 magic = tc > 1 ? (u32)((0x100000000ull + tc - 1) / tc) : 0u;
     auto tiles_of = [&](u32 c) -> u32 {
         if (tc <= 1) return tc ? c : 0u;
@@ -598,13 +610,13 @@
 }
 
 template <u32 RL>
-__global__ __launch_bounds__(256) void fj_level_lists(const u32* __restrict__ dir, const u64* __restrict__ rel, const u32* __restrict__ nalloc,
+__device__ __forceinline__ void fj_level_lists_body(const u32* __restrict__ dir, const u64* __restrict__ rel, const u32* __restrict__ nalloc,
                                u32 cap, const u32* __restrict__ boff, const u32* __restrict__ seg_off, u32 fan_mask,
                                u32 max_segs, u32* __restrict__ list,
                                u32 nb, u32 tc, const u32* __restrict__ toff, uint4* __restrict__ tiles, u32 max_tiles,
-                               u32* __restrict__ zero_tail, u32* __restrict__ clr) {
+                               u32* __restrict__ zero_tail, u32* __restrict__ clr, const u32 bid, const u32 nblk) {
     u32 n = *nalloc; if (n > cap) n = cap;
-    const u32 stride = gridDim.x * blockDim.x, gtid = blockIdx.x * blockDim.x + threadIdx.x;
+    const u32 stride = nblk * blockDim.x, gtid = bid * blockDim.x + threadIdx.x;
     if (clr) for (u32 i = gtid; i < nb / 4u; i += stride) reinterpret_cast<uint4*>(clr)[i] = make_uint4(0, 0, 0, 0);
     if (tc) {
         u32 total = toff[nb];
@@ -681,24 +693,30 @@
     }
 }
 
-template <bool FUSED>
-__global__ __launch_bounds__(1024) void fj_level_lists_binned(const u32* __restrict__ dir, const u64* __restrict__ rel, const u32* __restrict__ nalloc,
+template <bool WITH_SCAN>
+struct BinnedLds {
+    u32 hist[512 + 1];
+    u32 wsum[512 / 64];
+    uint2 ent[4096];
+    u32 boff_s[WITH_SCAN ? 512 + 1 : 1], toff_s[WITH_SCAN ? 512 + 1 : 1];
+    u64 wtot[512 / 64];
+    u32 s_last;
+};
+template <bool FUSED, typename Lds>
+__device__ __forceinline__ void fj_level_lists_binned_body(Lds& L, const u32* __restrict__ dir, const u64* __restrict__ rel, const u32* __restrict__ nalloc,
                                u32 cap, u32* __restrict__ boff_g, const u32* __restrict__ seg_off, u32 fan_mask,
                                u32 max_segs, u32* __restrict__ list,
                                u32 nb, u32 tc, u32* __restrict__ toff_g, uint4* __restrict__ tiles, u32 max_tiles,
-                               u32* __restrict__ zero_tail, u32* __restrict__ bchunks) {
+                               u32* __restrict__ zero_tail, u32* __restrict__ bchunks, const u32 bid, const u32 nblk) {
     constexpr u32 NT = 1024, BLK = 4096, NBMAX = 512;
-    __shared__ u32 hist[NBMAX + 1];
-    __shared__ u32 wsum[NBMAX / 64];
-    __shared__ uint2 ent[BLK];
-    __shared__ u32 boff_s[FUSED ? NBMAX + 1 : 1], toff_s[FUSED ? NBMAX + 1 : 1];
-    __shared__ u64 wtot[NBMAX / 64];
-    __shared__ u32 s_last;
+    u32* const hist = L.hist; u32* const wsum = L.wsum; uint2* const ent = L.ent;
+    u32* const boff_s = L.boff_s; u32* const toff_s = L.toff_s; u64* const wtot = L.wtot;
+    u32& s_last = L.s_last;
     const u32* boff = FUSED ? boff_s : boff_g;
     const u32* toff = FUSED ? toff_s : toff_g;
     u32 n = *nalloc; if (n > cap) n = cap;
     const u32 tid = threadIdx.x, lane = tid & 63, wave = tid >> 6;
-    const u32 stride = gridDim.x * NT, gtid = blockIdx.x * NT + tid;
+    const u32 stride = nblk * NT, gtid = bid * NT + tid;
     if constexpr (FUSED) {
         const float rtc = tc ? 1.0f / (float)tc : 0.f;
         auto tiles_of = [&](u32 c) -> u32 {
@@ -718,7 +736,7 @@
             if (lane == 63) wtot[wave] = v;
         }
         __syncthreads();
-        if (tid == 0) { __threadfence(); s_last = atomicAdd(&bchunks[nb], 1u) == gridDim.x - 1 ? 1u : 0u; }
+        if (tid == 0) { __threadfence(); s_last = atomicAdd(&bchunks[nb], 1u) == nblk - 1 ? 1u : 0u; }
         if (tid < NBMAX) {
             u64 woff = 0;
             for (u32 w = 0; w < wave; ++w) woff += wtot[w];
@@ -728,7 +746,7 @@
         }
         __syncthreads();
         if (s_last) { if (tid < nb) bchunks[tid] = 0; if (tid == 0) bchunks[nb] = 0; }
-        if (blockIdx.x == 0 && tid <= nb) { boff_g[tid] = boff_s[tid]; if (tc) toff_g[tid] = toff_s[tid]; }
+        if (bid == 0 && tid <= nb) { boff_g[tid] = boff_s[tid]; if (tc) toff_g[tid] = toff_s[tid]; }
     }
     if (tc) {
         u32 total = toff[nb];
@@ -738,7 +756,7 @@
             else if (zero_tail) zero_tail[t] = 0;
         }
     }
-    for (u32 base = blockIdx.x * BLK; base < n; base += gridDim.x * BLK) {
+    for (u32 base = bid * BLK; base < n; base += nblk * BLK) {
         if (tid < NBMAX) hist[tid] = 0;
         __syncthreads();
         u32 e[4]; u64 r[4];
@@ -782,6 +800,64 @@
         for (u32 j = tid; j < total; j += NT) { const uint2 x = ent[j]; list[x.x] = x.y; }
         __syncthreads();
     }
+}
+
+struct LevelArgs {
+    const u32* dir; const u64* rel; const u32* nalloc; u32 cap; u32* boff; const u32* seg_off; u32 fan_mask, max_segs; u32* list;
+    u32 nb, tc; u32* toff; uint4* tiles; u32 max_tiles; u32* zero_tail;
+    u32* bchunks;
+    u32* clr;
+    u32 nblocks;
+    u32 fused;
+};
+struct LevelArgs2 { LevelArgs r[2]; };
+
+__global__ __launch_bounds__(1024) void fj_level_scan(u32* __restrict__ bchunks, u32* __restrict__ boff, u32 n, u32 tc, u32* __restrict__ toff) {
+    fj_level_scan_body(bchunks, boff, n, tc, toff);
+}
+__global__ __launch_bounds__(1024) void fj_level_scan2(LevelArgs2 a) {
+    const LevelArgs& d = a.r[blockIdx.y];
+    fj_level_scan_body(d.bchunks, d.boff, d.nb, d.tc, d.toff);
+}
+__global__ __launch_bounds__(1024) void fj_level_scan_wide(const u32* __restrict__ bchunks, u32* __restrict__ boff, u32 n, u32 tc, u32* __restrict__ toff) {
+    fj_level_scan_wide_body(bchunks, boff, n, tc, toff, blockIdx.x);
+}
+__global__ __launch_bounds__(1024) void fj_level_scan_wide2(LevelArgs2 a) {
+    const LevelArgs& d = a.r[blockIdx.y];
+    fj_level_scan_wide_body(d.bchunks, d.boff, d.nb, d.tc, d.toff, blockIdx.x);
+}
+template <u32 RL>
+__global__ __launch_bounds__(256) void fj_level_lists(const u32* __restrict__ dir, const u64* __restrict__ rel, const u32* __restrict__ nalloc,
+                               u32 cap, const u32* __restrict__ boff, const u32* __restrict__ seg_off, u32 fan_mask,
+                               u32 max_segs, u32* __restrict__ list,
+                               u32 nb, u32 tc, const u32* __restrict__ toff, uint4* __restrict__ tiles, u32 max_tiles,
+                               u32* __restrict__ zero_tail, u32* __restrict__ clr) {
+    fj_level_lists_body<RL>(dir, rel, nalloc, cap, boff, seg_off, fan_mask, max_segs, list, nb, tc, toff, tiles, max_tiles, zero_tail, clr, blockIdx.x, gridDim.x);
+}
+template <u32 RL>
+__global__ __launch_bounds__(256) void fj_level_lists2(LevelArgs2 a) {
+    const LevelArgs& d = a.r[blockIdx.y];
+    fj_level_lists_body<RL>(d.dir, d.rel, d.nalloc, d.cap, d.boff, d.seg_off, d.fan_mask, d.max_segs, d.list, d.nb, d.tc, d.toff, d.tiles, d.max_tiles,
+                            d.zero_tail, d.clr, blockIdx.x, gridDim.x);
+}
+template <bool FUSED>
+__global__ __launch_bounds__(1024) void fj_level_lists_binned(const u32* __restrict__ dir, const u64* __restrict__ rel, const u32* __restrict__ nalloc,
+                               u32 cap, u32* __restrict__ boff_g, const u32* __restrict__ seg_off, u32 fan_mask,
+                               u32 max_segs, u32* __restrict__ list,
+                               u32 nb, u32 tc, u32* __restrict__ toff_g, uint4* __restrict__ tiles, u32 max_tiles,
+                               u32* __restrict__ zero_tail, u32* __restrict__ bchunks) {
+    __shared__ BinnedLds<FUSED> L;
+    fj_level_lists_binned_body<FUSED>(L, dir, rel, nalloc, cap, boff_g, seg_off, fan_mask, max_segs, list, nb, tc, toff_g, tiles, max_tiles, zero_tail, bchunks,
+                                      blockIdx.x, gridDim.x);
+}
+__global__ __launch_bounds__(1024) void fj_level_lists_binned2(LevelArgs2 a) {
+    __shared__ BinnedLds<true> L;
+    const LevelArgs& d = a.r[blockIdx.y];
+    if (blockIdx.x >= d.nblocks) return;
+    if (d.fused) fj_level_lists_binned_body<true>(L, d.dir, d.rel, d.nalloc, d.cap, d.boff, d.seg_off, d.fan_mask, d.max_segs, d.list, d.nb, d.tc, d.toff, d.tiles,
+                                                  d.max_tiles, d.zero_tail, d.bchunks, blockIdx.x, d.nblocks);
+    else fj_level_lists_binned_body<false>(L, d.dir, d.rel, d.nalloc, d.cap, d.boff, d.seg_off, d.fan_mask, d.max_segs, d.list, d.nb, d.tc, d.toff, d.tiles,
+                                           d.max_tiles, d.zero_tail, d.bchunks, blockIdx.x, d.nblocks);
 }
 
 __global__ __launch_bounds__(1024) void fj_dir_rank_kernel(u32* __restrict__ dir, u32 n, u32 b_lo, u32 nbk, u32 fan, u64* __restrict__ rel,
@@ -861,6 +937,16 @@
     const bool flat = a.in_list == nullptr;
     if (line_log == 3) return flat ? launch_part<NT, KPT, 3, HAS_VALS, true>(a, grid, s) : launch_part<NT, KPT, 3, HAS_VALS, false>(a, grid, s);
     return flat ? launch_part<NT, KPT, 4, HAS_VALS, true>(a, grid, s) : launch_part<NT, KPT, 4, HAS_VALS, false>(a, grid, s);
+}
+
+template <bool FLAT, int RLOG>
+hipError_t launch_part_both(const FjPartArgs2& a, hipStream_t s) {
+    const PartLds L = part_lds_layout(1024 * 8, 1u << a.p.fan_log, 16, false, 16);
+    auto kern = fj_partition_both_kernel<1024, 8, 4, FLAT, RLOG>;
+    hipError_t e = fj_set_max_lds_once(reinterpret_cast<const void*>(kern), L.total);
+    if (e != hipSuccess) return e;
+    hipLaunchKernelGGL(kern, dim3(a.gb > a.gp ? a.gb : a.gp), dim3(1024), L.total, s, a);
+    return hipGetLastError();
 }
 
 }
@@ -919,6 +1005,23 @@
     return launch_part2<1024, 8, false>(a, line_log, grid < 256 ? grid : 256, s);
 }
 
+hipError_t fj_launch_partition2(const FjPartArgs& b, u32 gb, const FjPartArgs& p, u32 gp, hipStream_t s) {
+    for (const FjPartArgs* a : {&b, &p}) {
+        if (a->shift < 32 || a->fan_log > FJ_MAX_FAN_LOG || a->slab < (1u << FJ_RUN_LOG) || (a->slab & ((1u << FJ_RUN_LOG) - 1u))) return hipErrorInvalidValue;
+        if (a->in_pk7 || a->vals_pos || a->in_vals || a->out_vals) return hipErrorInvalidValue;
+    }
+    const bool flat = b.in_list == nullptr;
+    if (flat != (p.in_list == nullptr) || b.fan_log != p.fan_log || b.run_log != p.run_log || gb == 0 || gp == 0) return hipErrorInvalidValue;
+    if (b.run_log != 0 && b.run_log != FJ_RUN_LOG) return hipErrorInvalidValue;
+    if (b.run_log == 0 && !flat) return hipErrorInvalidValue;
+    FjPartArgs2 a;
+    a.b = b; a.p = p;
+    a.gb = b.fan_log == 9 ? gb : (gb < 256 ? gb : 256);
+    a.gp = p.fan_log == 9 ? gp : (gp < 256 ? gp : 256);
+    if (flat) return b.run_log == 0 ? launch_part_both<true, 0>(a, s) : launch_part_both<true, FJ_RUN_LOG>(a, s);
+    return launch_part_both<false, FJ_RUN_LOG>(a, s);
+}
+
 hipError_t fj_launch_group(const FjChunkSet& cs, u32 tc, u32* toff, uint4* tiles, u32 max_tiles, u32* zero_tail, hipStream_t s) {
     if (cs.nb & 3u) return hipErrorInvalidValue;
     static_assert(FJ_RUN_LOG == 1 || FJ_RUN_LOG == 2, "fj_level_lists reads a run's directory words with one 8-B or 16-B load");
@@ -954,3 +1057,48 @@
     hipLaunchKernelGGL(fj_scan_u32_to_u64, dim3(1), dim3(1024), 0, s, in, out, n);
     return hipGetLastError();
 }
+
+hipError_t fj_launch_group2(const FjGroupJob& jb, const FjGroupJob& jp, hipStream_t s) {
+    const FjGroupJob* j[2] = {&jb, &jp};
+    bool binned[2];
+    for (int r = 0; r < 2; ++r) {
+        const FjChunkSet& cs = j[r]->cs;
+        if (cs.nb & 3u) return hipErrorInvalidValue;
+        if (cs.run_log != 0 && cs.run_log != FJ_RUN_LOG) return hipErrorInvalidValue;
+        binned[r] = cs.run_log == 0 && cs.nb <= 512 && cs.cap >= 4096;
+    }
+    if (binned[0] != binned[1] || jb.cs.nb != jp.cs.nb || jb.cs.run_log != jp.cs.run_log) {
+        hipError_t e = fj_launch_group(jb.cs, jb.tc, jb.toff, jb.tiles, jb.max_tiles, jb.zero_tail, s);
+        return e != hipSuccess ? e : fj_launch_group(jp.cs, jp.tc, jp.toff, jp.tiles, jp.max_tiles, jp.zero_tail, s);
+    }
+    LevelArgs2 a{};
+    for (int r = 0; r < 2; ++r) {
+        const FjChunkSet& cs = j[r]->cs;
+        LevelArgs& d = a.r[r];
+        d.dir = cs.dir; d.rel = cs.rel; d.nalloc = cs.alloc; d.cap = cs.cap; d.boff = cs.boff; d.seg_off = cs.seg_off; d.fan_mask = cs.fan_mask;
+        d.max_segs = cs.max_segs; d.list = cs.list; d.nb = cs.nb; d.tc = j[r]->tc; d.toff = j[r]->toff; d.tiles = j[r]->tiles;
+        d.max_tiles = j[r]->max_tiles; d.zero_tail = j[r]->zero_tail; d.bchunks = cs.bchunks; d.clr = nullptr; d.nblocks = 0; d.fused = 0;
+    }
+    if (binned[0]) {
+        u32 gx = 0;
+        for (int r = 0; r < 2; ++r) {
+            LevelArgs& d = a.r[r];
+            const u32 blocks = (d.cap + 4095u) / 4096u;
+            d.fused = blocks <= 512u ? 1u : 0u;
+            d.nblocks = blocks < 4096u ? blocks : 4096u;
+            if (!d.fused) hipLaunchKernelGGL(fj_level_scan, dim3(1), dim3(1024), 0, s, d.bchunks, d.boff, d.nb, d.tc, d.toff);
+            gx = d.nblocks > gx ? d.nblocks : gx;
+        }
+        hipLaunchKernelGGL(fj_level_lists_binned2, dim3(gx, 2), dim3(1024), 0, s, a);
+        return hipGetLastError();
+    }
+    const u32 nb = jb.cs.nb;
+    const bool wide = nb >= 8192u && nb <= (1u << 19);
+    if (wide) {
+        hipLaunchKernelGGL(fj_level_scan_wide2, dim3((nb + 4095u) / 4096u, 2), dim3(1024), 0, s, a);
+        a.r[0].clr = a.r[0].bchunks; a.r[1].clr = a.r[1].bchunks;
+    } else hipLaunchKernelGGL(fj_level_scan2, dim3(1, 2), dim3(1024), 0, s, a);
+    auto kern = jb.cs.run_log ? fj_level_lists2<FJ_RUN_LOG> : fj_level_lists2<0>;
+    hipLaunchKernelGGL(kern, dim3(2048, 2), dim3(256), 0, s, a);
+    return hipGetLastError();
+}
diff --git a/flash_hash_join_amd/csrc/fj_plan.hip b/flash_hash_join_amd/csrc/fj_plan.hip
--- a/flash_hash_join_amd/csrc/fj_plan.hip
+++ b/flash_hash_join_amd/csrc/fj_plan.hip
@@ -147,10 +147,10 @@
     return 0;
 }
 
-int pass_launch(fj_ctx* c, PassIter& it, const u64* keys, const u64* vals, size_t n, hipStream_t s, int* ev_cursor) {
+static void pass_args(fj_ctx* c, const PassIter& it, const u64* keys, const u64* vals, size_t n, FjPartArgs& a, u32& G) {
     const FjChunkSet& cs = it.cs;
-    FjPartArgs a{};
-    u32 G = it.Gmax;
+    a = FjPartArgs{};
+    G = it.Gmax;
     if (it.have_prev) {
         a.in_keys = it.prev.keys; a.in_vals = it.prev.vals; a.in_list = it.prev.list; a.in_dir = it.prev.dir;
         a.in_tiles = it.tiles; a.in_ntiles = it.ntiles; a.n_flat = 0;
@@ -166,10 +166,25 @@
     a.err = it.err_word ? it.err_word : &c->d_sc->err;
     if (it.have_prev && it.in_pk7) { a.in_pk7 = 1; a.in_b0 = it.in_b0; a.in_top_shift = it.in_top_shift; }
     a.shift = (u32)it.used; a.fan_log = (u32)it.plan.fan_log[it.i]; a.slab = fj_slab_for(it.appends); a.run_log = cs.run_log; a.side = (u32)it.side;
+}
+
+int pass_launch(fj_ctx* c, PassIter& it, const u64* keys, const u64* vals, size_t n, hipStream_t s, int* ev_cursor) {
+    FjPartArgs a; u32 G;
+    pass_args(c, it, keys, vals, n, a, G);
     const int line_log = (it.has_vals && it.F > 256) ? 3 : 4;
     if (ev_cursor) HIPCHK(hipEventRecord(c->ev[E_PK0 + 2 * (*ev_cursor)], s));
     HIPCHK(fj_launch_partition(a, it.has_vals, line_log, G, s));
     if (ev_cursor) { HIPCHK(hipEventRecord(c->ev[E_PK0 + 2 * (*ev_cursor) + 1], s)); ++*ev_cursor; }
+    return 0;
+}
+
+static int pass_launch2(fj_ctx* c, PassIter& bit, PassIter& pit, const u64* bk, const u64* pk, hipStream_t s, int* ev_cursor) {
+    FjPartArgs ab, ap; u32 Gb, Gp;
+    pass_args(c, bit, bk, nullptr, bit.n, ab, Gb);
+    pass_args(c, pit, pk, nullptr, pit.n, ap, Gp);
+    HIPCHK(hipEventRecord(c->ev[E_PK0 + 2 * (*ev_cursor)], s));
+    HIPCHK(fj_launch_partition2(ab, Gb, ap, Gp, s));
+    HIPCHK(hipEventRecord(c->ev[E_PK0 + 2 * (*ev_cursor) + 1], s)); ++*ev_cursor;
     return 0;
 }
 
@@ -192,7 +207,7 @@
     return np_eff <= 3 * nb;
 }
 
-int level_finish(fj_ctx* c, PassIter& it, bool final_level, hipStream_t s) {
+static int level_job(fj_ctx* c, PassIter& it, bool final_level, FjGroupJob* job) {
     const FjChunkSet& cs = it.cs;
     u32 tc = 0; u64 max_tiles = 0; u32* zero_tail = nullptr;
     if (bloom_stage_follows(it, it.i)) tc = fj_bloom_tile_chunks();
@@ -213,20 +228,48 @@
             it.part_count = zero_tail = (u32*)p; it.items_cap = (u32)max_tiles;
         }
     }
-    HIPCHK(fj_launch_group(cs, tc, toff, tiles, (u32)max_tiles, zero_tail, s));
+    *job = FjGroupJob{cs, tc, toff, tiles, (u32)max_tiles, zero_tail};
     it.tiles = tiles; it.ntiles = toff ? toff + cs.nb : nullptr; it.toff = toff;
     return 0;
 }
-
-int pass_complete(fj_ctx* c, PassIter& it, hipStream_t s) {
+int level_finish(fj_ctx* c, PassIter& it, bool final_level, hipStream_t s) {
+    FjGroupJob j;
+    if (level_job(c, it, final_level, &j)) return 1;
+    HIPCHK(fj_launch_group(j.cs, j.tc, j.toff, j.tiles, j.max_tiles, j.zero_tail, s));
+    return 0;
+}
+
+static void pass_advance(PassIter& it) {
     const FjChunkSet& cs = it.cs;
-    it.lbound = it.n / FJ_CHUNK + 1 + (u64)(it.Gmax + it.parents) * it.F * it.appends;
-    ++it.i;
-    if (level_finish(c, it, it.i == it.plan.npass, s)) return 1;
     it.prev = cs; it.have_prev = true;
     it.parents = cs.nb;
     ++it.slot;
     if (it.save_level == it.i) it.saved = cs;
+}
+
+int pass_complete(fj_ctx* c, PassIter& it, hipStream_t s) {
+    it.lbound = it.n / FJ_CHUNK + 1 + (u64)(it.Gmax + it.parents) * it.F * it.appends;
+    ++it.i;
+    if (level_finish(c, it, it.i == it.plan.npass, s)) return 1;
+    pass_advance(it);
+    return 0;
+}
+
+int run_passes_merged(fj_ctx* c, PassIter& bit, PassIter& pit, const u64* bk, const u64* pk, hipStream_t s, FjChunkSet* bout, FjChunkSet* pout,
+                      int* ev_cursor) {
+    while (bit.i < bit.plan.npass) {
+        if (pass_prepare(c, bit, 1, s) || pass_prepare(c, pit, 1, s)) return 1;
+        if (pass_launch2(c, bit, pit, bk, pk, s, ev_cursor)) return 1;
+        FjGroupJob jb, jp;
+        for (PassIter* it : {&bit, &pit}) {
+            it->lbound = it->n / FJ_CHUNK + 1 + (u64)(it->Gmax + it->parents) * it->F * it->appends;
+            ++it->i;
+        }
+        if (level_job(c, bit, bit.i == bit.plan.npass, &jb) || level_job(c, pit, pit.i == pit.plan.npass, &jp)) return 1;
+        HIPCHK(fj_launch_group2(jb, jp, s));
+        pass_advance(bit); pass_advance(pit);
+    }
+    *bout = bit.prev; *pout = pit.prev;
     return 0;
 }
 
@@ -311,12 +354,17 @@
 
 float ev_ms(fj_ctx* c, int a, int b) { float ms = 0.f; (void)hipEventElapsedTime(&ms, c->ev[a], c->ev[b]); return ms; }
 
-void plan_timings(fj_ctx* c, const Plan& plan, u64 partitions, int evc, fj_timings* t) {
+void plan_timings(fj_ctx* c, const Plan& plan, u64 partitions, int evc, fj_timings* t, double build_share) {
     t->path = 0; t->passes = plan.npass; t->radix_bits = plan.bits; t->partitions = partitions;
-    t->build_phase_ms = ev_ms(c, E_START, E_BUILD);
     t->join_ms = ev_ms(c, E_PPART, E_JOIN);
-    t->probe_phase_ms = ev_ms(c, E_BUILD, E_JOIN);
     t->total_ms = ev_ms(c, E_START, E_JOIN);
+    if (build_share >= 0) {
+        t->build_phase_ms = build_share * ev_ms(c, E_START, E_PPART);
+        t->probe_phase_ms = t->total_ms - t->build_phase_ms;
+    } else {
+        t->build_phase_ms = ev_ms(c, E_START, E_BUILD);
+        t->probe_phase_ms = ev_ms(c, E_BUILD, E_JOIN);
+    }
     for (int i = 0; i < evc && i < 4; ++i) t->probe_part_kernel_ms[i] = ev_ms(c, E_PK0 + 2 * i, E_PK0 + 2 * i + 1);
     t->bloom_level = plan.bloom_level;
     if (plan.bloom_level > 0) { t->filter_ms = ev_ms(c, E_BF0, E_BF1); t->filter_survivors = c->h_sc->bloom_survivors; }
@@ -363,6 +411,7 @@
     if (!strcmp(name, "join_items_target")) { if (value < 1 || value > (1 << 20)) return set_err("fj_set_option: join_items_target must be 1..1048576"); o.join_items_target = (u32)value; return 0; }
     if (!strcmp(name, "mm_heavy_keys")) { if (value < 0 || value > 1) return set_err("fj_set_option: mm_heavy_keys must be 0 or 1"); o.mm_heavy_keys = (int)value; return 0; }
     if (!strcmp(name, "mm_heavy_outer")) { if (value < 0 || value > 1) return set_err("fj_set_option: mm_heavy_outer must be 0 or 1"); o.mm_heavy_outer = (int)value; return 0; }
+    if (!strcmp(name, "merged_levels")) { if (value < 0 || value > 1) return set_err("fj_set_option: merged_levels must be 0 or 1"); o.merged_levels = (int)value; return 0; }
     return set_err("fj_set_option: unknown option '%s'", name);
 }
 
@@ -397,6 +446,7 @@
     if (name && !strcmp(name, "join_items_target")) return o.join_items_target;
     if (name && !strcmp(name, "mm_heavy_keys")) return o.mm_heavy_keys;
     if (name && !strcmp(name, "mm_heavy_outer")) return o.mm_heavy_outer;
+    if (name && !strcmp(name, "merged_levels")) return o.merged_levels;
     set_err("fj_get_option: unknown option '%s'", name ? name : "(null)");
     return -1;
 }
```

Result: no change. 114.9, median of 6 (+0.8%).
